# gligen/GLIGEN

Hardware: AMD Instinct MI355X
Metric: 512x512 images/sec @ 50 PLMS steps, box+text (CFG 7.5), UNet step ms (higher is better)
Workload: dtype bf16; 1 GPU; C2: box+text, 8 boxes (30 grounding tokens), 512x512, 50 PLMS steps, CFG 7.5, bf16 storage / fp32 accumulate; plms_steps=50, unet_evals_per_image=102, hipgraph=True, batches_in_flight=3

## Files before the change

gligen_amd/_lib.py:

```python
from __future__ import annotations

import ctypes as C
from pathlib import Path

_HERE = Path(__file__).resolve().parent
LIB_PATH = _HERE / "libgligen_amd.so"


class GligenAmdError(RuntimeError):
    pass


class UNetConfig(C.Structure):
    _fields_ = [
        ("in_channels", C.c_int), ("out_channels", C.c_int), ("model_channels", C.c_int),
        ("num_res_blocks", C.c_int), ("num_heads", C.c_int), ("context_dim", C.c_int),
        ("n_mult", C.c_int), ("channel_mult", C.c_int * 8),
        ("n_attn", C.c_int), ("attention_resolutions", C.c_int * 8),
        ("inpaint_mode", C.c_int), ("grounding_kind", C.c_int),
        ("gr_in_dim", C.c_int), ("gr_out_dim", C.c_int), ("max_persons", C.c_int), ("fuser_kind", C.c_int),
        ("extra_channels", C.c_int), ("tok_resize", C.c_int), ("tok_in_dim", C.c_int),
    ]


# ... 157 lines not shown
                                                C.POINTER(_P), C.POINTER(_P), _P, _P, _P]),
    "gl_op_class_conv_wgrad": (_I, [_P, _I, _P, _I, _I, _I, _I, _I, _P, _I, _P, _P, _P]),
}

TRAIN_INPUT_SYMBOLS = {
    "gl_train_step_inputs": (_I, [_P, C.POINTER(TrainStepInputsArgs), _P]),
}

TRAIN_FUSER_SYMBOLS = {
    "gl_op_block_train_fuser": (_I, [_P, _I, _P, C.POINTER(_P), _P, _P, _P, _P, _P, _P, _P, _P, C.POINTER(_P), _P]),
    "gl_op_grid_resize": (_I, [_P, _P, _I, _I, _I, _I, _P, _P]),
    "gl_op_grid_resize_backward": (_I, [_P, _P, _I, _I, _I, _I, _P, _P]),
}

_F = C.c_float
TRAIN_PRIM_SYMBOLS = {
    "gl_op_train_attention": (_I, [_P, _I, _I, _I, _I, _I] + [_P] * 9 + [_P]),
    "gl_op_train_linear": (_I, [_P, _I, _I, _I] + [_P] * 8 + [_P]),
    "gl_op_train_layernorm": (_I, [_P, _I, _I, _F, _P, _P, _P, _P, _I] + [_P] * 6 + [_P]),
    "gl_op_train_groupnorm": (_I, [_P, _I, _I, _I, _I, _F, _P, _P, _P, _P, _I] + [_P] * 4 + [_P]),
    "gl_op_train_geglu": (_I, [_P, _I, _I, _P, _P, _P, _P, _P]),
    "gl_op_train_dot": (_I, [_P, C.c_int64, _P, _P, _P, _F, _I, _P, _P]),
}

TRAINER_SYMBOLS = {
    "gl_op_adamw_ema_step": (_I, [_P, _P, _P, _P, _P, _P, C.c_int64, C.c_double, C.c_double, C.c_double, C.c_double, C.c_double, C.c_double, _I, _P]),
}

SAMPLER_SYMBOLS = {
    "gl_set_cfg_shared_prefix": (_I, [_I]),
}

class GemmPlanRecord(C.Structure):
    _fields_ = [("kernel", C.c_char * 96)] + [(n, C.c_int) for n in ("family", "M", "N", "K", "tm", "tn", "splits", "grid", "n_items", "box", "rm", "rz",
                                                                     "units_per_split", "xcd")]


class AttnProjLayout(C.Structure):
    _fields_ = [(n, C.c_int) for n in ("d", "dp", "dpv", "tq", "tk", "tq_pad", "tk_pad", "vt_perm32")]


GEMM_PLAN_SYMBOLS = {
    "gl_gemm_force_plan": (_I, [_I, _I, _I, _I]),
    "gl_gemm_force_knobs": (_I, [_I, _I, _I, _I, _I, _I]),
    "gl_gemm_force_clear": (_I, []),
    "gl_gemm_plan_log_clear": (_I, []),
    "gl_gemm_plan_log": (_I, [C.POINTER(GemmPlanRecord), _I, C.POINTER(_I), C.POINTER(_I)]),
    "gl_op_attention_project": (_I, [_P, _P, _P, _I, _I, _I, _I, _I, _I, _P, _P, _P, _P, _P, _P, C.POINTER(AttnProjLayout), _P]),
}

ATTENTION_CORE_SYMBOLS = {
    "gl_op_attention_core": (_I, [_P, _P, _P, _P, C.POINTER(AttnProjLayout), _I, _I, _I, _I, _P, _I, _I, _I, _P]),
}
ATTN_CORE_KERNELS = {"auto": 0, "attn_kernel": 1, "attn2_kernel_w4": 2, "attn2_kernel_w8": 3, "attn3_kernel": 4}
GL_ERR_UNSUPPORTED = 5

FUSER_KINDS = {"gatedSA": 0, "gatedSA2": 1, "gatedCA": 2}


def fuser_kind(fuser_type) -> int:
    try:
        return FUSER_KINDS[fuser_type or "gatedSA"]
    except KeyError:
        raise ValueError(f"fuser_type {fuser_type!r}: one of {sorted(FUSER_KINDS)}") from None


_lib = None


def load() -> C.CDLL:
    global _lib
    if _lib is not None:
        return _lib
    if not LIB_PATH.exists():
        raise GligenAmdError(
            f"{LIB_PATH} not found: build it with `python -m gligen_amd.build` "
            "(gligen_amd has no fallback path without its HIP library)")
    import torch
    lib = C.CDLL(str(LIB_PATH))
    for name, (res, args) in {**SYMBOLS, **IMAGE_SYMBOLS, **MAP_SYMBOLS, **TRAIN_MAP_SYMBOLS, **TRAIN_INPUT_SYMBOLS, **TRAIN_FUSER_SYMBOLS, **TRAIN_PRIM_SYMBOLS,
                              **TRAINER_SYMBOLS, **SAMPLER_SYMBOLS, **GEMM_PLAN_SYMBOLS, **ATTENTION_CORE_SYMBOLS}.items():
        fn = getattr(lib, name)
        fn.restype = res
        fn.argtypes = args
    _lib = lib
    return lib


def check(rc: int) -> None:
    if rc != 0:
        msg = load().gl_last_error()
        raise GligenAmdError(f"libgligen_amd error {rc}: {msg.decode() if msg else '?'}")
```

gligen_amd/csrc/capi.hip:

```cpp
#include "classmap.h"
#include "engine_impl.h"
#include "image.h"
#include "train.h"
#include "train_fusers.h"
#include "../../include/gligen_amd_train_maps.h"
#include "../../include/gligen_amd_train_inputs.h"
#include "../../include/gligen_amd_train_fusers.h"
#include "../../include/gligen_amd_train_prims.h"
#include "../../include/gligen_amd_trainer.h"
#include "../../include/gligen_amd_sampler.h"
#include "../../include/gligen_amd_gemm_plans.h"
#include "../../include/gligen_amd_attention_core.h"
#include "gemm_plan.h"

#include <cstdlib>

#include <cmath>

using namespace gl;

struct gl_ctx {
    std::shared_ptr<Engine> holder;
    Engine* eng;
    ImageStage image_stage;
};

#define GL_API_BEGIN try {
#define GL_API_END                                       \
    }                                                    \
    catch (const gl::GlError& e) {                       \
        return gl::set_error(e.code, "%s", e.what());    \
    }                                                    \
    catch (const std::exception& e) {                    \
        return gl::set_error(GL_ERR_STATE, "%s", e.what()); \
    }                                                    \
    return GL_OK;

struct DeviceGuard {
    int prev = -1;
    bool ok = true;
    explicit DeviceGuard(int dev) {
        if (hipGetDevice(&prev) != hipSuccess) prev = -1;
        if (prev != dev) ok = hipSetDevice(dev) == hipSuccess;
        else prev = -1;
    }
    ~DeviceGuard() {
        if (prev >= 0) (void)hipSetDevice(prev);
    }
};
#define NEED(ctx)                                                         \
    if (!(ctx) || !(ctx)->eng) return gl::set_error(GL_ERR_ARG, "null context"); \
    DeviceGuard device_guard_((ctx)->eng->device());                      \
    if (!device_guard_.ok) return gl::set_error(GL_ERR_HIP, "hipSetDevice(%d) failed", (ctx)->eng->device());

static inline hipStream_t S(gl_stream s) { return reinterpret_cast<hipStream_t>(s); }
#define HIPCK_API(expr)                                                                           \
    do {                                                                                          \
        hipError_t _e = (expr);                                                                   \
        if (_e != hipSuccess) throw GlError(GL_ERR_HIP, std::string(#expr) + ": " + hipGetErrorString(_e)); \
    } while (0)

extern "C" {

const char* gl_last_error(void) { return gl::last_error(); }

// ... 330 lines not shown
                    gl_stream s) {
    NEED(ctx);
    if (!x || !timesteps || !eps_out || !recs || !n_recs || max_recs <= 0) return gl::set_error(GL_ERR_ARG, "null pointer");
    GL_API_BEGIN
    ctx->eng->profile_begin();
    std::vector<Engine::ProfRec> out;
    try {
        ctx->eng->unet_forward(Beff, h, w, x, xB, timesteps, inpaint_extra, extraB, eps_out, S(s));
    } catch (...) {
        (void)ctx->eng->profile_end(S(s));
        throw;
    }
    out = ctx->eng->profile_end(S(s));
    int n = 0;
    for (const auto& r : out) {
        if (n >= max_recs) break;
        gl_prof_rec& d = recs[n++];
        snprintf(d.name, sizeof d.name, "%s", r.name.c_str());
        d.calls = r.calls; d.ms = r.ms; d.flops = r.flops; d.bytes = r.bytes;
    }
    *n_recs = n;
    GL_API_END
}

int gl_to_uint8(const float* img, uint8_t* out, int B, int C, int HW, gl_stream s) {
    if (!img || !out) return gl::set_error(GL_ERR_ARG, "null pointer");
    hipPointerAttribute_t at;
    if (hipPointerGetAttributes(&at, img) != hipSuccess) {
        (void)hipGetLastError();
        return gl::set_error(GL_ERR_ARG, "gl_to_uint8: img is not a device pointer");
    }
    DeviceGuard guard(at.device);
    if (!guard.ok) return gl::set_error(GL_ERR_HIP, "hipSetDevice(%d) failed", at.device);
    return to_uint8_launch(img, out, B, C, HW, S(s));
}

int gl_arena_high_water(gl_ctx* ctx, size_t* bytes) {
    NEED(ctx);
    *bytes = ctx->eng->arena().high_water();
    return GL_OK;
}

int gl_launch_count(gl_ctx* ctx, int64_t* n) {
    NEED(ctx);
    *n = ctx->eng->n_launches;
    return GL_OK;
}

int gl_set_ff_rows_policy(int mode) { return gl::ff_rows_policy_set(mode); }

int gl_ff_rows_policy_report(char* buf, size_t cap) { return gl::ff_rows_policy_report(buf, cap); }

int gl_set_cfg_shared_prefix(int on) { return gl::cfg_shared_prefix_set(on); }

int gl_gemm_force_plan(int tm, int tn, int splits, int grid_cap) {
    bool tile = tm == 0 && tn == 0;
    for (int c = 0; c < kGemmTiles; ++c) tile |= kGemmTm[c] == tm && kGemmTn[c] == tn;
    if (!tile || splits < 0 || splits > 32 || grid_cap < 0)
        return gl::set_error(GL_ERR_ARG, "gl_gemm_force_plan: tile %dx%d / %d splits / cap %d (tiles 4x5 4x4 2x5 2x4 2x2 or 0x0, splits 0..32, cap >= 0)", tm, tn, splits, grid_cap);
    gemm_force_cfg(tm, tn, tm ? splits : 0);
    gemm_force_grid(grid_cap);
    return GL_OK;
}
int gl_gemm_force_knobs(int halo_splits, int wide_splits, int wide_xcd, int xcd_boxes, int halo, int wide) {
    if (halo_splits < 0 || wide_splits < 0 || wide_xcd < -1 || wide_xcd > 1 || xcd_boxes < 0 || xcd_boxes > 1 || halo < 0 || wide < 0 || wide > 2)
        return gl::set_error(GL_ERR_ARG, "gl_gemm_force_knobs: halo_splits %d, wide_splits %d, wide_xcd %d, xcd_boxes %d, halo %d, wide %d", halo_splits, wide_splits, wide_xcd, xcd_boxes, halo, wide);
    gemm_force_knobs(halo_splits, wide_splits, wide_xcd, xcd_boxes, halo, wide);
    return GL_OK;
}
int gl_gemm_force_clear(void) { gemm_force_clear(); return GL_OK; }
int gl_gemm_plan_log_clear(void) { gemm_plan_log_clear(); return GL_OK; }
int gl_gemm_plan_log(gl_gemm_plan_record* out, int max, int* n_written, int* n_launches) {
    if (!out || !n_written || !n_launches || max < 0) return gl::set_error(GL_ERR_ARG, "gl_gemm_plan_log: null pointer or negative max");
    GemmLogEntry e[kGemmLogSize];
    const int n = gemm_plan_log(e, std::min(max, (int)kGemmLogSize), n_launches);
    for (int i = 0; i < n; ++i) {
        const GemmPlan& p = e[i].plan;
        gl_gemm_plan_record& r = out[i];
        r = gl_gemm_plan_record{};
        snprintf(r.kernel, sizeof r.kernel, "%s", p.name);
        r.family = p.family; r.M = e[i].M; r.N = e[i].N; r.K = e[i].K;
        r.tm = p.tm; r.tn = p.tn; r.splits = p.splits; r.grid = p.grid;
        if (p.family == GEMM_HALO) { r.n_items = p.halo.n_items; r.units_per_split = p.halo.chunks_per_split; }
        else if (p.family == GEMM_WIDE) { r.n_items = p.wide.n_items; r.units_per_split = p.wide.kt_per_split; r.xcd = p.wide.xcd; }
        else {
            r.n_items = p.work.n_items; r.units_per_split = p.work.kt_per_split;
            if (p.family != GEMM_GLDS) { r.box = p.work.box; r.rm = p.work.rm; r.rz = p.work.rz; }
        }
    }
    *n_written = n;
    return GL_OK;
}

int gl_box_calibrate(gl_ctx* ctx, gl_box_calibration* out, gl_stream s) {
    NEED(ctx);
    if (!out) return gl::set_error(GL_ERR_ARG, "gl_box_calibrate: null out pointer");
    GL_API_BEGIN
    Arena& ar = ctx->eng->arena();
    const size_t mk = ar.mark();
    const size_t bytes = size_t(1) << 30;
    void* scratch = ar.alloc(bytes);
    HIPCK_API(hipMemsetAsync(scratch, 1, bytes, S(s)));
    float v[3] = {0.f, 0.f, 0.f};
    int rc = box_calibrate_launch(scratch, bytes, v, S(s));
    ar.release(mk);
    if (rc != GL_OK) throw GlError(rc, gl::last_error());
// ... 592 lines not shown
        bf16* w4 = ar.get<bf16>((size_t)16 * Cout * Cin);
        const int rp = pack_upconv_phases_launch(w_oihw, w4, Cout, Cin, Cout, S(s));
        if (rp != GL_OK) throw GlError(rp, gl::last_error());
        c.w4 = w4;
        ctx->eng->conv3x3(TRef{(const bf16*)x0, C0, (const bf16*)x1, C1}, B, H, W, c, 1, 1, 1, nullptr, 0, nullptr, S(s), (bf16*)y);
        return GL_OK;
    }
    bf16* wp = ar.get<bf16>((size_t)Cout * 9 * Cin);
    int r = pack_conv_weight_launch(w_oihw, wp, Cout, Cin, 3, 3, Cout, S(s));
    if (r != GL_OK) throw GlError(r, gl::last_error());
    const int Hup = H << ups, Wup = W << ups;
    const int Ho = stride == 1 ? Hup : (pad_lo ? (Hup + 2 - 3) / 2 + 1 : (Hup + 1 - 3) / 2 + 1);
    const int Wo = stride == 1 ? Wup : (pad_lo ? (Wup + 2 - 3) / 2 + 1 : (Wup + 1 - 3) / 2 + 1);
    AOperand A{};
    A.p0 = (const bf16*)x0; A.C0 = C0; A.ld0 = C0; A.p1 = (const bf16*)x1; A.C1 = C1; A.ld1 = C1;
    A.mode = A_CONV3; A.Hin = H; A.Win = W; A.Ho = Ho; A.Wo = Wo; A.stride = stride; A.ups = ups; A.pad_lo = pad_lo;
    Epilogue E;
    epilogue_defaults(E);
    E.out = y; E.ldo = Cout; E.bias = bias; E.res = (const bf16*)res; E.ldres = Cout; E.rows_per_b = Ho * Wo;
    r = gemm_launch(A, wp, B * Ho * Wo, Cout, 9 * Cin, E, ctx->eng->splitk_ws(), ctx->eng->splitk_ws_bytes(), S(s));
    if (r != GL_OK) throw GlError(r, gl::last_error());
    GL_API_END
}

int gl_op_gn_silu_conv3x3(gl_ctx* ctx, const void* x0, int C0, const void* x1, int C1, int B, int H, int W, const float* gamma, const float* beta,
                          float eps, const float* w_oihw, const float* bias, int Cout, const float* bias2, const void* res, void* y, int mode,
                          int* used_prologue, gl_stream s) {
    NEED(ctx);
    if (!x0 || !gamma || !beta || !w_oihw || !y || !used_prologue) return gl::set_error(GL_ERR_ARG, "gl_op_gn_silu_conv3x3: null pointer");
    GL_API_BEGIN
    Engine& eng = *ctx->eng;
    Arena& ar = eng.arena();
    ar.reset();
    const int Cin = C0 + C1;
    bf16* wp = ar.get<bf16>((size_t)Cout * 9 * Cin);
    int r = pack_conv_weight_launch(w_oihw, wp, Cout, Cin, 3, 3, Cout, S(s));
    if (r != GL_OK) throw GlError(r, gl::last_error());
    NormW n;
    n.g = gamma; n.b = beta; n.C = Cin;
    ConvW c;
    c.w = wp; c.b = bias; c.Cin = Cin; c.Cout = Cout;
    const bool saved = eng.gn_prologue_;
    if (mode >= 0) eng.gn_prologue_ = mode != 0;
    const int64_t n0 = eng.n_prologue_convs;
    try {
        eng.gn_silu_conv3x3(TRef{(const bf16*)x0, C0, (const bf16*)x1, C1}, B, H, W, n, eps, c, bias2, Cout, (const bf16*)res, (bf16*)y, S(s));
    } catch (...) {
        eng.gn_prologue_ = saved;
        throw;
    }
    eng.gn_prologue_ = saved;
    *used_prologue = eng.n_prologue_convs > n0 ? 1 : 0;
    if (mode == 1 && !*used_prologue) throw GlError(GL_ERR_UNSUPPORTED, "gl_op_gn_silu_conv3x3: this shape has no GroupNorm prologue (conv_halo_kernel, H W % 256 == 0)");
    GL_API_END
}

int gl_op_groupnorm(gl_ctx* ctx, const void* x0, int C0, const void* x1, int C1, int B, int HW,
                    const float* gamma, const float* beta, float eps, int silu, void* y, gl_stream s) {
    NEED(ctx);
    GL_API_BEGIN
    Arena& ar = ctx->eng->arena();
    ar.reset();
    GNParams P{};
    P.x0 = (const bf16*)x0; P.C0 = C0; P.x1 = (const bf16*)x1; P.C1 = C1; P.B = B; P.HW = HW; P.eps = eps;
    P.gamma = gamma; P.beta = beta; P.y = (bf16*)y; P.silu = silu;
    P.partial = reinterpret_cast<float*>(ar.alloc(gn_partial_bytes(B, HW)));
    int r = groupnorm_launch(P, S(s));
    if (r != GL_OK) throw GlError(r, gl::last_error());
    GL_API_END
}

int gl_op_layernorm(gl_ctx* ctx, const void* x, const void* x2, int B, int N1, int N2, int Tpad, int C,
                    const float* gamma, const float* beta, float eps, void* y, gl_stream s) {
    NEED(ctx);
    GL_API_BEGIN
    LNParams P{};
    P.x = (const bf16*)x; P.x2 = (const bf16*)x2; P.B = B; P.N1 = N1; P.N2 = N2; P.Tpad = Tpad; P.C = C; P.eps = eps;
    P.gamma = gamma; P.beta = beta; P.y = (bf16*)y;
    int r = layernorm_launch(P, S(s));
    if (r != GL_OK) throw GlError(r, gl::last_error());
    GL_API_END
}

static void attention_project(Engine& eng, const void* xq, const void* xkv, int B, int Nq, int Nk, int C, int Ck, int H, const float* wq,
                              const float* wk, const float* wv, bf16* q, bf16* k, bf16* vt, int Tq_pad, int Tk_pad, int dp, int dpv, int vt_layout,
                              hipStream_t s) {
    Arena& ar = eng.arena();
    const int d = C / H, Tq = round_up(Nq, 64), Tk = round_up(Nk, 64);
    bf16* wqb = ar.get<bf16>((size_t)C * C);
    bf16* wkb = ar.get<bf16>((size_t)C * Ck);
    bf16* wvb = ar.get<bf16>((size_t)C * Ck);
    bf16* xqp = ar.get<bf16>((size_t)B * Tq * C);
    bf16* xkp = ar.get<bf16>((size_t)B * Tk * Ck);
    auto ck = [&](int rc) { if (rc != GL_OK) throw GlError(rc, gl::last_error()); };
    ck(cast_f32_bf16_launch(wq, wqb, (int64_t)C * C, s));
    ck(cast_f32_bf16_launch(wk, wkb, (int64_t)C * Ck, s));
    ck(cast_f32_bf16_launch(wv, wvb, (int64_t)C * Ck, s));
    ck(pad_rows_bf16_launch((const bf16*)xq, xqp, B, Nq, Tq, C, s));
    ck(pad_rows_bf16_launch((const bf16*)xkv, xkp, B, Nk, Tk, Ck, s));
    const bool fused = xq == xkv && C == Ck && Nq == Nk && gemm_supports_qkv() && (2 * C) % 128 == 0 &&
                       !(dev_env("GL_QKV_FUSED") && atoi(dev_env("GL_QKV_FUSED")) == 0);
    if (fused) {
        bf16* wqkv = ar.get<bf16>((size_t)3 * C * C);
        ck(cast_f32_bf16_launch(wq, wqkv, (int64_t)C * C, s));
        ck(cast_f32_bf16_launch(wk, wqkv + (size_t)C * C, (int64_t)C * C, s));
        ck(cast_f32_bf16_launch(wv, wqkv + (size_t)2 * C * C, (int64_t)C * C, s));
// ... 159 lines not shown
```

gligen_amd/csrc/engine.h:

```cpp
#pragma once
#include <array>
#include <map>
#include <memory>
#include <stdexcept>
#include <string>
#include <unordered_map>
#include <unordered_set>
#include <vector>

#include "arena.h"
#include "attention.h"
#include "clip.h"
#include "common.h"
#include "convnext.h"
#include "ffn.h"
#include "gemm.h"
#include "misc.h"
#include "norm.h"
#include "train.h"
#include "../../include/gligen_amd.h"

namespace gl {

struct RawTensor {
// ... 31 lines not shown
    const void* chain_stream = nullptr;
    bool chain_post = false;
    const void* chain_q_stream = nullptr;
    const float* chain_q_bias = nullptr;
};
struct RowStats { float2* p = nullptr; int nb = 0, ld = 0; };
struct STW {
    int C = 0, d = 0, idx = 0;
    NormW gn;
    LinW proj_in, proj_out;
    NormW ln1, ln2, ln3, fn1, fn2;
    SelfAttnW a1, fa;
    CrossAttnW a2;
    FFW ff, fff;
    LinW flin;
    CrossAttnW fca;
};

enum LayerKind { L_CONV_IN, L_RES, L_ST, L_DOWN, L_UP };
struct Layer {
    LayerKind kind;
    int idx;
};
struct UNetBlock { std::vector<Layer> layers; };

struct VaeAttnW { NormW gn; LinW q, k, v, proj; };

struct CnxBlock { const float* dw_w = nullptr; const float* dw_b = nullptr; NormW ln; LinW pw1, pw2; };
struct CnxNet {
    bool present = false;
    int resize = 0, in_dim = 0, tokens = 0;
    const float* inconv_w = nullptr; const float* inconv_b = nullptr;
    LinW stem; NormW stem_ln;
    NormW ds_ln[3]; LinW ds[3];
    std::vector<CnxBlock> blocks[4];
    int dims[4] = {0, 0, 0, 0};
    const float* pos = nullptr; const float* null_feat = nullptr;
    LinW mlp[3];
};

struct AttnBufs {
    bf16* q = nullptr;
    bf16* k = nullptr;
    bf16* vt = nullptr;
    int Tq_pad = 0, Tk_pad = 0;
};

struct TRef { const bf16* p0 = nullptr; int C0 = 0; const bf16* p1 = nullptr; int C1 = 0; int C() const { return C0 + C1; } };

int ff_rows_policy_set(int mode);
int ff_rows_policy_report(char* buf, size_t cap);
int cfg_shared_prefix_set(int on);
bool cfg_shared_prefix();
AttnParams attn_params(const bf16* q, const bf16* k, const bf16* vt, bf16* o, int H, int d, int Nq, int Nk, int Tq_pad, int Tk_pad, int vt_layout);

class Engine {
   public:
    explicit Engine(int device);
    ~Engine();
    static std::shared_ptr<Engine> fork(const std::shared_ptr<Engine>& parent, size_t arena_bytes);
    size_t weight_bytes() const { return persist_bytes_; }
    size_t arena_bytes() const { return arena_.committed(); }
    bool is_fork() const { return (bool)parent_; }

    void upload(const std::string& key, const void* src, int ndim, const int64_t* shape, bool is_device);
    void configure_unet(const gl_unet_config& c);
    void configure_vae(const gl_vae_config& c);
    void configure_clip_text(const gl_clip_text_config& c);
    void configure_clip_vision(const gl_clip_vision_config& c);
    void finalize();
    bool finalized() const { return finalized_; }

    void set_cond(int Beff, const float* context, int n_ctx, const gl_grounding& g, hipStream_t s);
    void set_fuser_scale(float v, hipStream_t s);
    void set_fuser_scales(const float* scales_host, int n, hipStream_t s);
    int n_fusers() const { return (int)unet_.st.size(); }
    void grounding_tokens(float* out, hipStream_t s);
    void spatial_tokens(int B, const float* image, int C, int H, int W, const float* mask, float* out, hipStream_t s);
    void spatial_tokens_classes(int B, const uint8_t* cls, int H, int W, const float* mask, float* out, hipStream_t s);
    int spatial_token_count() const { return unet_.cnx.tokens; }
    void restore_first_conv(const float* w, const float* b, hipStream_t s);
    void unet_forward(int Beff, int h, int w, const float* x, int xB, const int64_t* t, const float* extra,
                      int extraB, float* eps, hipStream_t s, const float* emb_row = nullptr);
    void vae_decode(int B, int h, int w, const float* z, float* out, hipStream_t s);
    void vae_encode(int B, int H, int W, const float* img, const float* noise, float* z, hipStream_t s);
    bool has_vae_encoder() const { return vae_.enc.present; }
    void clip_text_encode(const int32_t* ids, const int32_t* eos_index, int S, int T, float* last_hidden, float* pooled, hipStream_t s);
    void clip_vision_encode(const float* pixel_values, int S, float* last_hidden, float* pooled, float* image_embeds, hipStream_t s);
    int clip_vision_tokens() const { const int g = clipv_.cfg.patch ? clipv_.cfg.image_size / clipv_.cfg.patch : 0; return g * g + 1; }
    void sample_plms(const gl_plms_args& a, hipStream_t s);
    void sampler_timing(float* avg_ms, float* first_ms, int* n);

    Arena& arena() { return arena_; }
    float* splitk_ws() { return ws_; }
    size_t splitk_ws_bytes() const { return ws_bytes_; }
    void* persist(size_t bytes, bool zero);
    void init_workspace();
    AttnBufs& attn_bufs(int B, int H, int d, int Tq, int Tk, int dpv_layout = 0, int slot = 0);
    void attn_regime_counters(int enable, unsigned* out);
    unsigned* attn_counters() const { return attn_counting_ ? attn_ctr_ : nullptr; }

    bf16* gn_silu_conv3x3(const TRef& x, int B, int H, int W, const NormW& n, float eps, const ConvW& c, const float* bias2, int bias2_ld,
                          const bf16* res, bf16* out, hipStream_t s);
    bf16* conv3x3(const TRef& x, int B, int Hin, int Win, const ConvW& c, int stride, int ups, int pad_lo,
                  const float* bias2, int bias2_ld, const bf16* res, hipStream_t s, bf16* out = nullptr);
    static bool upconv_phase_form(int Cin, int Cout);
    bool gn_prologue_ = dev_env("GL_GN_PROLOGUE") && atoi(dev_env("GL_GN_PROLOGUE")) == 1;
    int64_t n_prologue_convs = 0;
    int device() const { return device_; }
    int64_t n_launches = 0;
    static constexpr int kTrainEvents = 64;
    hipEvent_t* train_events();
    bool train_events_recorded = false;
    TrainWeightCache* train_cache = nullptr;

    struct ProfRec { std::string name; int calls = 0; double ms = 0, flops = 0, bytes = 0; };
    void profile_begin();
    std::vector<ProfRec> profile_end(hipStream_t s);

   private:
    struct ProfEvt { std::string name; double flops, bytes; hipEvent_t e0, e1; };
    bool profiling_ = false;
    std::vector<ProfEvt> prof_;
    std::vector<hipEvent_t> prof_pool_;
    struct ProfScope {
        Engine* e; hipStream_t s; size_t idx;
        ProfScope(Engine* eng, hipStream_t st, const std::string& name, double flops, double bytes);
        ~ProfScope();
        void rename(const std::string& n) { if (e->profiling_) e->prof_[idx].name = n; }
    };
    friend struct ProfScope;
    const RawTensor& raw(const std::string& key) const;
    bool has(const std::string& key) const { return raw_.count(key) != 0; }
    const float* F(const std::string& key) const { return raw(key).p; }
    const float* FK(const std::string& key) { keep_raw_.insert(key); return raw(key).p; }
    std::unordered_set<std::string> keep_raw_;
    NormW norm(const std::string& prefix);
    LinW linear(const std::string& prefix, bool bias = true);
    ConvW conv3(const std::string& prefix, int Npad = 0, bool up2x = false);
    ConvW conv3_small(const std::string& prefix, int Cout);
    LinW conv1(const std::string& prefix);
    const bf16* cast_rows(const std::vector<std::string>& weight_keys);
    FFW ffw(const std::string& prefix, int C, const NormW* fold = nullptr, const std::string& pre_key = "", const std::string& post_key = "",
            const float* post_q_w = nullptr, const float* post_q_b = nullptr);
    struct FoldTmp { float* w = nullptr; float* b = nullptr; int N = 0, K = 0; };
    FoldTmp fold_ln(const std::string& weight_key, const float* bias, const NormW& n);
    std::vector<void*> fold_tmps_;
    ResW resw(const std::string& prefix, int Cin, int Cout, bool unet);

    void gemm(const AOperand& A, const bf16* W, int M, int N, int K, const Epilogue& E, hipStream_t s);
    bf16* linear_rows(const bf16* x, int M, const LinW& L, int act, const bf16* res, const float* gate, hipStream_t s, RowStats* stats = nullptr);
    bf16* layernorm_plain(const bf16* x, int B, int N, int C, bool pad64, hipStream_t s);
    bf16* groupnorm(const TRef& x, int B, int HW, const NormW& n, float eps, bool silu, hipStream_t s);
    bf16* layernorm(const bf16* x, int B, int N, int C, const NormW& n, bool pad64, hipStream_t s);
    bf16* conv3x3_small(const ConvW& c, Im2colParams P, int reps, hipStream_t s);
    void gn_silu_conv3x3_nchw(const bf16* x, int C, int B, int H, int W, const NormW& n, float eps, const ConvW& c, int n_real, float* out, hipStream_t s);
    bf16* resblock(const ResW& r, const TRef& x, int B, int H, int W, const float* embout, int emb_ld, float eps, hipStream_t s, bf16* out = nullptr);
    void replicate(const bf16* src, bf16* dst, size_t n, int reps, hipStream_t s);
    void attention(const bf16* q, const bf16* k, const bf16* vt, bf16* o, int B, int H, int d, int Nq, int Nk, int Tq_pad, int Tk_pad, int vt_layout,
                   hipStream_t s);
    void spatial_tokens_tail(int B, const float* img, const float* mask, float* out, hipStream_t s);

    Engine(const Engine&) = default;
    Engine& operator=(const Engine&) = delete;
    std::shared_ptr<Engine> parent_;
    size_t persist_bytes_ = 0;
    int device_;
    bool finalized_ = false;
    std::unordered_map<std::string, RawTensor> raw_;
    std::vector<void*> owned_;
    Arena arena_;
    float* ws_ = nullptr;
    size_t ws_bytes_ = 0;
    typedef std::array<int, 7> AttnKey;
    std::map<AttnKey, AttnBufs> attn_bufs_;
    unsigned* attn_ctr_ = nullptr;
    bool attn_counting_ = false;
    std::vector<hipEvent_t> train_events_;

    struct Unet {
        bool present = false;
        gl_unet_config cfg{};
        LinW te0, te2;
        LinW embcat;
        ConvW conv_in_small;
        std::vector<ResW> res;
        std::vector<STW> st;
        std::vector<ConvW> updown;
        std::vector<UNetBlock> in_blocks, out_blocks;
        UNetBlock mid_block;
        NormW out_norm;
        ConvW out_conv;
        const float* const* alpha_ptrs = nullptr;
        int gkind = 0;
        LinW pn[2][3];
        const float* pn_null_feat[2] = {nullptr, nullptr};
        const float* pn_null_pos = nullptr;
        const float* kp_table = nullptr;
        CnxNet cnx;
    } unet_;
    bool ln_fold_ = false;
    bool ff_rows_ = true;
    int ff_chain_ = 2;
    int qkv_rows_ = 1;
    bool fuser_hoist_ = true;
    void build_unet();
    float* gates_ = nullptr;
    float* fuser_scale_ = nullptr;
    bool fuser_off_ = false;
    struct Cond {
        int Beff = 0, Ng = 0, ctx_T = 0, ctx_Tpad = 0, obj_Tpad = 0;
        bf16* tokens = nullptr;
        int obj_stride = 0;
        std::vector<bf16*> objs;
        std::vector<bf16*> obj_k;
        std::vector<bf16*> obj_vt;
        std::vector<bf16*> ctx_k;
        std::vector<bf16*> ctx_vt;
        std::vector<void*> allocs;
    } cond_;
    void fuser_kv_fill(const STW& t, int B, int HW, hipStream_t s);
    void ensure_fuser_kv(const STW& t, int B, int HW, hipStream_t s);
    struct FuserKV { uint64_t epoch = 0; int B = 0, HW = 0; };
    std::vector<FuserKV> fuser_kv_;
    uint64_t cond_epoch_ = 0;

    bf16* transformer(const STW& t, const bf16* x, int B, int Bp, int H, int W, hipStream_t s);
    bf16* feedforward(const FFW& f, const bf16* ln, int M, const bf16* res, const float* gate, hipStream_t s, const RowStats* in_stats = nullptr,
                      RowStats* out_stats = nullptr, bool raw_rows = false, bool use_rows = false);
    bf16* fuser_ff_tail(const STW& t, const bf16* o, const bf16* t1, int B, int HW, bool rows, hipStream_t s, RowStats* st3, bool* q_done = nullptr);
    AttnBufs& to_q_heads(const LinW& q, const bf16* ln, int B, int Tp, int C, int d, int Tk_pad, const RowStats* st, const float* csum, hipStream_t s);
    void cross_q_gemm(const STW& t, const bf16* rows, const RowStats& st, int B, int HW, hipStream_t s);
    bf16* concat_layernorm(const STW& t, const bf16* x, int B, int HW, int Tf, hipStream_t s);
    void block_ff_tail(const STW& t, const bf16* o, const bf16* t3, const bf16* x, bf16* out, int B, int HW, bool rows, hipStream_t s);
    bf16* ff_behind(const FFW& f, const NormW& nw, const bf16* rows_in, RowStats& st_in, int B, int HW, const float* gate, bool rows, hipStream_t s,
                    RowStats* out_stats);
    bool can_fold(const RowStats& st, int M, int C, int Nc, int mode, int act, bool aligned);
    struct ChainQ { bf16* q; int DP, T, Tpad; };
    bf16* feedforward_chain(const FFW& f, const bf16* x, int M, const LinW& pre, const bf16* pre_res, const float* pre_gate, const float* gate,
                            const LinW* post, const bf16* post_res, bf16* out, hipStream_t s, RowStats* out_stats, const ChainQ* cq = nullptr);
    void self_attention(const SelfAttnW& a, const bf16* ln, int B, int T, int Nq, int Nk, int C, int d, bf16* o, hipStream_t s,
                        const RowStats* in_stats = nullptr, int Tbuf = 0, int slot = 0, bool projected = false);
    bool qkv_rows_ok(const SelfAttnW& a, int B, int T, int Nk, int C, int d) const;
    void qkv_project_gemm(const SelfAttnW& a, const bf16* ln, int B, int T, int Nk, int C, int d, hipStream_t s, const RowStats* in_stats, int Tbuf, int slot);
    void qkv_rows_project(const SelfAttnW& a, const bf16* x, int B, int T, int Nk, int C, int d, const LinW& pre, const bf16* pre_res, bf16* mid,
                          RowStats* mid_stats, int Tbuf, int slot, hipStream_t s, int Bin = 0);
    float* emb_rows(const int64_t* t_dev, int R, float* out, hipStream_t s);
    void emb_table_build(const int64_t* t_host, int R, hipStream_t s);
    float* emb_table_ = nullptr;
    float* emb_cur_ = nullptr;
    int64_t* emb_t_dev_ = nullptr;
    int emb_table_cap_ = 0;
    std::vector<int64_t> emb_t_cache_;

    bool ff_rows_for(const STW& t, int which, int B, int HW, hipStream_t s);
    bool qkv_rows_for(const STW& t, int which, int B, int HW, int Nk, hipStream_t s);
    template <class Run>
    bool timed_form(uint64_t key, int M, int C, int n_zero, const char* name, int form, hipStream_t s, Run&& run);

    void build_convnext(const std::string& PN);

    struct VaeLevel { std::vector<ResW> blocks; bool has_resample = false; ConvW resample; };
    struct VaeHalf {
        bool present = false;
        ConvW in_small;
        ResW mid1, mid2;
        VaeAttnW attn;
        std::vector<VaeLevel> levels;
        NormW norm_out;
        ConvW conv_out;
        const float* quant_w = nullptr;
        const float* quant_b = nullptr;
    };
    struct Vae { gl_vae_config cfg{}; VaeHalf dec, enc; } vae_;
    void build_vae();
    void build_vae_encoder();
    void build_vae_mid(VaeHalf& h, const std::string& prefix, int C);
    bf16* vae_attn(const VaeAttnW& a, const bf16* x, int B, int HW, hipStream_t s);

    struct ClipLayerW { NormW ln1, ln2; LinW qkv, out, fc1, fc2; };
// ... 53 lines not shown
```

gligen_amd/csrc/engine.hip:

```cpp
#include "engine_impl.h"

#include <algorithm>
#include <cmath>
#include <cstdarg>
#include <cstring>

namespace gl {

static thread_local char g_err[2048] = "";
int set_error(int code, const char* fmt, ...) {
    va_list ap;
    va_start(ap, fmt);
    vsnprintf(g_err, sizeof(g_err), fmt, ap);
    va_end(ap);
    return code;
}
const char* last_error() { return g_err; }

void Arena::init(size_t bytes) {
    off_ = hw_ = 0;
    HIPCK(hipGetDevice(&dev_));
    int vmm = 0;
    const char* sw = dev_env("GL_ARENA_VMM");
    if (!(sw && atoi(sw) == 0) && hipDeviceGetAttribute(&vmm, hipDeviceAttributeVirtualMemoryManagementSupported, dev_) == hipSuccess && vmm) {
// ... 455 lines not shown
        ProfScope ps(this, s, sym, 4.0 * B * H * (double)Nq * Nk * d, 0.0);
        CK(attn_launch(P, B, s));
        if (FILE* f = launch_log_file()) {
            fprintf(f, "%s|%d|%d|%d|2|%.0f\n", sym, Nq, Nk, d, 2.0 * B * H * d * (2.0 * Nq + 2.0 * Nk));
            fflush(f);
        }
    }
    ++n_launches;
}

void Engine::gemm(const AOperand& A, const bf16* W, int M, int N, int K, const Epilogue& E, hipStream_t s) {
    ProfScope ps(this, s, "gemm", 2.0 * M * N * K, 0.0);
    CK(gemm_launch(A, W, M, N, K, E, ws_, ws_bytes_, s));
    if (profiling_) {
        static const bool by_shape = dev_env("GL_PROF_SHAPES") != nullptr;
        std::string nm = gemm_last_kernel_name();
        if (by_shape) nm += fmt(" M%d N%d K%d", M, N, K);
        ps.rename(nm);
    }
    FILE* launch_log = launch_log_file();
    if (launch_log) {
        const double a_rows = A.mode != A_ROWS ? (double)(M / (A.Ho * A.Wo)) * A.Hin * A.Win : (double)M;
        const double out_b = E.mode == EPI_NCHW_F32 ? 4.0 * M * E.n_real : (E.act == ACT_GEGLU ? 1.0 : 2.0) * M * (double)N * (E.out_f32 ? 2 : 1);
        const double bytes = a_rows * (A.C0 + A.C1) * 2 + (double)N * K * 2 + out_b + (E.res ? 2.0 * M * N : 0.0);
        fprintf(launch_log, "%s|%d|%d|%d|%d|%.0f\n", gemm_last_kernel_name(), M, N, K, A.mode, bytes);
        fflush(launch_log);
    }
    {
        int tm, tn, sp;
        gemm_last_cfg(&tm, &tn, &sp);
        n_launches += sp > 1 ? 2 : 1;
    }
}

bf16* Engine::linear_rows(const bf16* x, int M, const LinW& L, int act, const bf16* res, const float* gate, hipStream_t s, RowStats* stats) {
    bf16* out = arena_.get<bf16>((size_t)M * L.N);
    Epilogue E = e_rows_res(out, L.N, L.b, res);
    E.act = act;
    E.gate = gate;
    if (stats) {
        *stats = RowStats{};
        if (ln_fold_ && L.N % 64 == 0) {
            stats->ld = L.N / 32;
            stats->p = arena_.get<float2>((size_t)M * stats->ld);
            E.stats_out = stats->p;
            E.stats_ld = stats->ld;
        }
    }
    gemm(a_rows(x, L.K), L.w, M, L.N, L.K, E, s);
    if (stats && stats->p) stats->nb = gemm_last_stats_nb();
    return out;
}

bf16* Engine::groupnorm(const TRef& x, int B, int HW, const NormW& n, float eps, bool silu, hipStream_t s) {
    const int C = x.C();
    if (n.C != C) throw GlError(GL_ERR_ARG, fmt("groupnorm: %d channels given to a norm with %d", C, n.C));
    bf16* y = arena_.get<bf16>((size_t)B * HW * C);
    GNParams P{};
    P.x0 = x.p0; P.C0 = x.C0; P.x1 = x.p1; P.C1 = x.C1;
    P.B = B; P.HW = HW; P.eps = eps; P.gamma = n.g; P.beta = n.b; P.y = y; P.silu = silu ? 1 : 0;
    P.partial = reinterpret_cast<float*>(arena_.alloc(gn_partial_bytes(B, HW)));
    ProfScope ps(this, s, HW <= 256 ? "gn_small_kernel" : "gn_stats_kernel + gn_apply_kernel", 0.0, 2.0 * B * HW * (double)C * 2);
    CK(groupnorm_launch(P, s));
    n_launches += HW <= 256 ? 1 : 2;
    return y;
}

bf16* Engine::gn_silu_conv3x3(const TRef& x, int B, int H, int W, const NormW& n, float eps, const ConvW& c, const float* bias2, int bias2_ld,
                              const bf16* res, bf16* out, hipStream_t s) {
    if (x.C() != c.Cin || n.C != c.Cin) throw GlError(GL_ERR_ARG, fmt("gn_silu_conv3x3: %d channels into a norm of %d and a conv of %d", x.C(), n.C, c.Cin));
    const int HW = H * W, M = B * HW;
    if (!out) out = arena_.get<bf16>((size_t)M * c.Cout);
    AOperand A = a_conv3(x, H, W, H, W, 1, 0, 1);
    Epilogue E = e_rows_res(out, c.Cout, c.b, res);
    E.bias2 = bias2; E.bias2_ld = bias2_ld; E.rows_per_b = HW;
    if (gn_prologue_ && gemm_gn_prologue_supported(A, M, c.Cout, 9 * c.Cin, E)) {
        GNParams P{};
        P.x0 = x.p0; P.C0 = x.C0; P.x1 = x.p1; P.C1 = x.C1;
        P.B = B; P.HW = HW; P.eps = eps; P.gamma = n.g; P.beta = n.b; P.silu = 1;
        P.partial = reinterpret_cast<float*>(arena_.alloc(gn_partial_bytes(B, HW)));
        P.coef = reinterpret_cast<float*>(arena_.alloc(gn_coef_bytes(B, c.Cin)));
        {
            const int nl = groupnorm_coef_launches(HW, x.C0, x.C1);
            ProfScope ps(this, s, nl == 1 ? "gn_small_coef_kernel" : "gn_stats_kernel + gn_coef_kernel", 0.0, 1.0 * B * HW * (double)c.Cin * 2);
            CK(groupnorm_coef_launch(P, s));
            n_launches += nl;
        }
        A.gn = P.coef;
        gemm(A, c.w, M, c.Cout, 9 * c.Cin, E, s);
        ++n_prologue_convs;
        return out;
    }
    bf16* a = groupnorm(x, B, HW, n, eps, true, s);
    A.p0 = a; A.C0 = c.Cin; A.ld0 = c.Cin; A.p1 = nullptr; A.C1 = 0; A.ld1 = 0;
    gemm(A, c.w, M, c.Cout, 9 * c.Cin, E, s);
    return out;
}

bf16* Engine::layernorm(const bf16* x, int B, int N, int C, const NormW& n, bool pad64, hipStream_t s) {
    const int Tp = pad64 ? round_up(N, 64) : N;
    bf16* y = arena_.get<bf16>((size_t)B * Tp * C);
    LNParams P{};
    P.x = x; P.x2 = nullptr; P.B = B; P.N1 = N; P.N2 = 0; P.Tpad = Tp; P.C = C; P.eps = 1e-5f;
    P.gamma = n.g; P.beta = n.b; P.y = y;
    ProfScope ps(this, s, "ln_kernel", 0.0, 2.0 * B * N * (double)C * 2);
    CK(layernorm_launch(P, s));
    ++n_launches;
    return y;
}

bf16* Engine::layernorm_plain(const bf16* x, int B, int N, int C, bool pad64, hipStream_t s) {
    NormW none;
    none.C = C;
    return layernorm(x, B, N, C, none, pad64, s);
}

bf16* Engine::conv3x3(const TRef& x, int B, int Hin, int Win, const ConvW& c, int stride, int ups, int pad_lo,
                      const float* bias2, int bias2_ld, const bf16* res, hipStream_t s, bf16* out) {
    if (x.C() != c.Cin) throw GlError(GL_ERR_ARG, fmt("conv3x3: input has %d channels, weight expects %d", x.C(), c.Cin));
    if (c.w4) {
        if (stride != 1 || ups != 1 || pad_lo != 1 || bias2 || res) throw GlError(GL_ERR_ARG, "conv3x3: phase-form weights serve the plain upsample conv only");
        const int Mi = 4 * Hin * Win;
        if (!out) out = arena_.get<bf16>((size_t)B * Mi * c.Cout);
        auto ok = [&](int b) { return gemm_upconv_phases_supported(a_conv2up(x, Hin, Win), b * Mi, c.Cout, 4 * c.Cin, e_rows(out, c.Cout, c.b)); };
        int Bc = B;
        while (Bc > 1 && !ok(Bc)) Bc = (Bc + 1) / 2;
        if (!ok(Bc)) throw GlError(GL_ERR_UNSUPPORTED, fmt("conv3x3: no phase form for a %d x %d x %d -> %d upsample conv", Hin, Win, c.Cin, c.Cout));
        for (int b0 = 0; b0 < B; b0 += Bc) {
            const size_t px = (size_t)b0 * Hin * Win;
            const TRef xb{x.p0 + px * x.C0, x.C0, x.p1 ? x.p1 + px * x.C1 : nullptr, x.C1};
            gemm(a_conv2up(xb, Hin, Win), c.w4, std::min(Bc, B - b0) * Mi, c.Cout, 4 * c.Cin, e_rows(out + (size_t)b0 * Mi * c.Cout, c.Cout, c.b), s);
        }
        return out;
    }
    const int Hup = Hin << ups, Wup = Win << ups;
    const int Ho = stride == 1 ? Hup : (pad_lo ? (Hup + 2 - 3) / 2 + 1 : (Hup + 1 - 3) / 2 + 1);
    const int Wo = stride == 1 ? Wup : (pad_lo ? (Wup + 2 - 3) / 2 + 1 : (Wup + 1 - 3) / 2 + 1);
    const int M = B * Ho * Wo;
    if (!out) out = arena_.get<bf16>((size_t)M * c.Cout);
    Epilogue E = e_rows_res(out, c.Cout, c.b, res);
    E.bias2 = bias2; E.bias2_ld = bias2_ld; E.rows_per_b = Ho * Wo;
    gemm(a_conv3(x, Hin, Win, Ho, Wo, stride, ups, pad_lo), c.w, M, c.Cout, 9 * c.Cin, E, s);
    return out;
}

void Engine::replicate(const bf16* src, bf16* dst, size_t n, int reps, hipStream_t s) {
    ProfScope ps(this, s, "replicate_kernel", 0.0, (1.0 + reps) * n * 2);
    CK(replicate_launch(src, dst, n * sizeof(bf16), reps, s));
    ++n_launches;
}

bf16* Engine::resblock(const ResW& r, const TRef& x, int B, int H, int W, const float* embout, int emb_ld, float eps, hipStream_t s, bf16* out) {
    const int HW = H * W, M = B * HW;
    if (!out) out = arena_.get<bf16>((size_t)M * r.Cout);
    const size_t mk = arena_.mark();
    bf16* h = gn_silu_conv3x3(x, B, H, W, r.n1, eps, r.c1, embout ? embout + r.emb_off : nullptr, emb_ld, nullptr, nullptr, s);
    const bf16* sk;
    if (r.has_skip) {
        bf16* skb = arena_.get<bf16>((size_t)M * r.Cout);
        AOperand A{};
        A.p0 = x.p0; A.C0 = x.C0; A.ld0 = x.C0; A.p1 = x.p1; A.C1 = x.C1; A.ld1 = x.C1; A.mode = A_ROWS;
        gemm(A, r.skip.w, M, r.Cout, r.Cin, e_rows(skb, r.Cout, r.skip.b), s);
        sk = skb;
    } else {
        if (x.p1) throw GlError(GL_ERR_STATE, "identity skip over a concatenated input");
        sk = x.p0;
    }
    gn_silu_conv3x3(TRef{h, r.Cout, nullptr, 0}, B, H, W, r.n2, eps, r.c2, nullptr, 0, sk, out, s);
    arena_.release(mk);
    return out;
}

bf16* Engine::conv3x3_small(const ConvW& c, Im2colParams P, int reps, hipStream_t s) {
    const size_t rows = (size_t)P.B * P.H * P.W;
    bf16* col = arena_.get<bf16>(reps * rows * c.Kpad);
    bf16* out = arena_.get<bf16>(reps * rows * c.Cout);
    P.Kpad = c.Kpad;
    for (int r = 0; r < reps; ++r) {
        P.out = col + r * rows * c.Kpad;
        CK(im2col_small_launch(P, s));
        ++n_launches;
    }
    gemm(a_rows(col, c.Kpad), c.w, (int)(reps * rows), c.Cout, c.Kpad, e_rows(out, c.Cout, c.b), s);
    return out;
}

void Engine::gn_silu_conv3x3_nchw(const bf16* x, int C, int B, int H, int W, const NormW& n, float eps, const ConvW& c, int n_real, float* out, hipStream_t s) {
    const int HW = H * W;
    bf16* a = groupnorm(TRef{x, C, nullptr, 0}, B, HW, n, eps, true, s);
    Epilogue E;
    epilogue_defaults(E);
    E.mode = EPI_NCHW_F32; E.out = out; E.bias = c.b; E.rows_per_b = HW; E.n_real = n_real;
    gemm(a_conv3(TRef{a, C, nullptr, 0}, H, W, H, W, 1, 0, 1), c.w, B * HW, c.Npad, 9 * C, E, s);
}

AttnBufs& Engine::attn_bufs(int B, int H, int d, int Tq, int Tk, int dpv_layout, int slot) {
    const int Tq_pad = round_up(Tq, 128), Tk_pad = round_up(Tk, 64);
    int dp, dpv;
    CK(attn_dims(d, &dp, &dpv));
    if (dpv_layout) dpv = dpv_layout;
    const AttnKey key{{B, H, d, Tq_pad, Tk_pad, dpv, slot}};
    auto it = attn_bufs_.find(key);
    if (it != attn_bufs_.end()) return it->second;
    AttnBufs b;
    b.Tq_pad = Tq_pad;
    b.Tk_pad = Tk_pad;
    b.q = reinterpret_cast<bf16*>(persist((size_t)B * H * Tq_pad * dp * sizeof(bf16), true));
    b.k = reinterpret_cast<bf16*>(persist((size_t)B * H * Tk_pad * dp * sizeof(bf16), true));
    b.vt = reinterpret_cast<bf16*>(persist((size_t)B * H * dpv * Tk_pad * sizeof(bf16), true));
    CK(attn_vt_ones_launch(b.vt, B * H, d, Tk_pad, 0, dpv));
    CK(attn_k_init_launch(b.k, B * H, d, Tk_pad, 0));
    HIPCK(hipStreamSynchronize(0));
    return attn_bufs_.emplace(key, b).first->second;
}

}
```

gligen_amd/csrc/engine_impl.h:

```cpp
#pragma once
#include "engine.h"

namespace gl {

#define CK(expr)                                              \
    do {                                                      \
        int _r = (expr);                                      \
        if (_r != GL_OK) throw GlError(_r, gl::last_error()); \
    } while (0)
#define HIPCK(expr)                                                                             \
    do {                                                                                        \
        hipError_t _e = (expr);                                                                 \
        if (_e != hipSuccess)                                                                   \
            throw GlError(GL_ERR_HIP, std::string(#expr) + " -> " + hipGetErrorString(_e));     \
    } while (0)

FILE* launch_log_file();

unsigned ff_rows_policy_epoch();

void cfg_shared_prefix_note(int what);

struct PlanAsBatch {
    explicit PlanAsBatch(int scale) { gemm_set_plan_batch_scale(scale); }
    ~PlanAsBatch() { gemm_set_plan_batch_scale(1); }
};

inline AOperand a_rows(const bf16* x, int K) {
    AOperand A;
    aoperand_rows(A, x, K, K);
    return A;
}
inline AOperand a_conv3(const TRef& x, int Hin, int Win, int Ho, int Wo, int stride, int ups, int pad_lo) {
    AOperand A{};
    A.p0 = x.p0; A.C0 = x.C0; A.ld0 = x.C0;
    A.p1 = x.p1; A.C1 = x.C1; A.ld1 = x.C1;
    A.mode = A_CONV3;
    A.Hin = Hin; A.Win = Win; A.Ho = Ho; A.Wo = Wo; A.stride = stride; A.ups = ups; A.pad_lo = pad_lo;
    return A;
}
inline AOperand a_conv2up(const TRef& x, int Hin, int Win) {
    AOperand A = a_conv3(x, Hin, Win, 2 * Hin, 2 * Win, 1, 0, 1);
    A.mode = A_CONV2UP;
    return A;
}
inline Epilogue e_rows(void* out, int ldo, const float* bias = nullptr) {
    Epilogue E;
    epilogue_defaults(E);
    E.out = out; E.ldo = ldo; E.bias = bias;
    return E;
}
inline Epilogue e_rows_res(void* out, int ldo, const float* bias, const bf16* res) {
    Epilogue E = e_rows(out, ldo, bias);
    E.res = res; E.ldres = ldo;
    return E;
}
inline Epilogue e_heads(int mode, bf16* q, bf16* k, int C, int H, int d, int DP, int T, int Tpad_q, int Tpad_k) {
    Epilogue E;
    epilogue_defaults(E);
    E.mode = mode;
    E.q = q; E.k = k; E.C = C; E.H = H; E.d = d; E.DP = DP; E.T = T; E.Tpad_q = Tpad_q; E.Tpad_k = Tpad_k;
    return E;
}
inline void e_fold_ln(Epilogue& E, const RowStats& st, const float* csum, int C) {
    E.ln_stats = st.p; E.ln_nb = st.nb; E.ln_ld = st.ld; E.ln_csum = csum;
    E.ln_inv_c = 1.f / (float)C; E.ln_eps = 1e-5f;
}

}
```

gligen_amd/csrc/engine_policy.hip:

```cpp
#include "engine_impl.h"
#include <algorithm>
#include <atomic>
#include <map>
#include <mutex>

namespace gl {

namespace ff_policy {
static std::mutex mu;
struct Entry { int rows; float us_rows, us_gemm; };
static std::map<uint64_t, Entry> table;
static std::atomic<int> mode{-1};
static std::atomic<unsigned> epoch{1};
static uint64_t key(int dev, int which, int form, int C, int M) {
    return ((uint64_t)dev << 56) | ((uint64_t)which << 52) | ((uint64_t)form << 48) | ((uint64_t)C << 32) | (uint64_t)(unsigned)M;
}
static bool static_rule(int M) { return M / 128 >= 224; }
static int current_mode() {
    static const bool env_once = [] {
        if (const char* e = dev_env("GL_FF_POLICY")) mode.store(atoi(e));
        return true;
    }();
    (void)env_once;
    return mode.load();
}
}

int ff_rows_policy_set(int mode) {
    if (mode < -1 || mode > 2) return set_error(GL_ERR_ARG, "ff_rows policy %d (expected -1 timed, 0 never, 1 wherever supported, 2 static rule)", mode);
    if (ff_policy::mode.exchange(mode) != mode) ff_policy::epoch.fetch_add(1);
    return GL_OK;
}
unsigned ff_rows_policy_epoch() { return ff_policy::epoch.load(); }

namespace cfg_prefix {
static std::atomic<int> on{-1};
static int current() {
    int v = on.load();
    if (v < 0) {
        const char* e = dev_env("GL_CFG_SHARED_PREFIX");
        const int want = (e && atoi(e) == 0) ? 0 : 1;
        int expect = -1;
        on.compare_exchange_strong(expect, want);
        v = on.load();
    }
    return v;
}
static std::atomic<long long> count[3];
}
bool cfg_shared_prefix() { return cfg_prefix::current() != 0; }
void cfg_shared_prefix_note(int what) { cfg_prefix::count[what].fetch_add(1); }
int cfg_shared_prefix_set(int on) {
    if (on != 0 && on != 1) return set_error(GL_ERR_ARG, "cfg shared prefix %d (expected 0 or 1)", on);
    if (cfg_prefix::current() != on) {
        cfg_prefix::on.store(on);
        ff_policy::epoch.fetch_add(1);
    }
    return GL_OK;
}
int ff_rows_policy_report(char* buf, size_t cap) {
    if (!buf || !cap) return set_error(GL_ERR_ARG, "ff_rows_policy_report: no buffer");
    std::lock_guard<std::mutex> lk(ff_policy::mu);
    size_t n = (size_t)snprintf(buf, cap, "mode=%d", ff_policy::mode.load());
    for (const auto& kv : ff_policy::table) {
        if (n + 96 + 128 >= cap) break;
        const uint64_t k = kv.first;
        n += (size_t)snprintf(buf + n, cap - n, ";dev%d %s form%d C%d M%d -> %s (rows %.1f us, gemm %.1f us)", (int)(k >> 56),
                              ((k >> 52) & 15) == 1 ? "fuser.ff" : ((k >> 52) & 15) == 2 ? "ff" : ((k >> 52) & 15) == 3 ? "proj_in+attn1.qkv" : "attn1.to_out+fuser.qkv", (int)((k >> 48) & 15), (int)((k >> 32) & 0xffff), (int)(k & 0xffffffffu),
                              kv.second.rows ? "rows" : "gemm", kv.second.us_rows, kv.second.us_gemm);
    }
    if (n + 128 < cap)
        snprintf(buf + n, cap - n, ";cfg_shared_prefix=%d evals=%lld rows_at_prefix=%lld rows_periodic=%lld", cfg_prefix::current(),
                 cfg_prefix::count[0].load(), cfg_prefix::count[1].load(), cfg_prefix::count[2].load());
    return GL_OK;
}

template <class Run>
bool Engine::timed_form(uint64_t key, int M, int C, int n_zero, const char* name, int form, hipStream_t s, Run&& run) {
    const int mode = ff_policy::current_mode();
    if (mode == 0) return false;
    if (mode == 1) return true;
    if (mode == 2) return ff_policy::static_rule(M);
    std::unique_lock<std::mutex> lk(ff_policy::mu);
    auto it = ff_policy::table.find(key);
    if (it != ff_policy::table.end()) return it->second.rows != 0;
    hipStreamCaptureStatus cap = hipStreamCaptureStatusNone;
    (void)hipStreamIsCapturing(s, &cap);
    if (cap != hipStreamCaptureStatusNone) {
        const bool rows = ff_policy::static_rule(M);
        ff_policy::table[key] = ff_policy::Entry{rows ? 1 : 0, 0.f, 0.f};
        return rows;
    }

    HIPCK(hipDeviceSynchronize());
    struct Restore {
        Engine* e; size_t mk; int64_t launches; bool prof;
        ~Restore() { e->arena_.release(mk); e->n_launches = launches; e->profiling_ = prof; }
    } restore{this, arena_.mark(), n_launches, profiling_};
    profiling_ = false;
    bf16* z[4];
    for (bf16*& p : z) p = arena_.get<bf16>((size_t)M * C);
    for (int i = 0; i < n_zero; ++i) HIPCK(hipMemsetAsync(z[i], 0, (size_t)M * C * sizeof(bf16), s));
    auto once = [&](bool rows) {
        const size_t m2 = arena_.mark();
        run(rows, z);
        arena_.release(m2);
    };
    hipEvent_t ev[2];
    HIPCK(hipEventCreate(&ev[0]));
    HIPCK(hipEventCreate(&ev[1]));
    struct EvGuard { hipEvent_t* e; ~EvGuard() { (void)hipEventDestroy(e[0]); (void)hipEventDestroy(e[1]); } } guard{ev};
    float best[2] = {1e30f, 1e30f};
    constexpr int REPS = 4, ROUNDS = 3;
    for (int form_i = 0; form_i < 2; ++form_i) once(form_i == 1);
    for (int r = 0; r < ROUNDS; ++r)
        for (int form_i = 0; form_i < 2; ++form_i) {
            HIPCK(hipEventRecord(ev[0], s));
            for (int i = 0; i < REPS; ++i) once(form_i == 1);
            HIPCK(hipEventRecord(ev[1], s));
            HIPCK(hipEventSynchronize(ev[1]));
            float ms = 0.f;
            HIPCK(hipEventElapsedTime(&ms, ev[0], ev[1]));
            best[form_i] = std::min(best[form_i], ms * 1e3f / REPS);
// ... 50 lines not shown
```

gligen_amd/csrc/engine_unet.hip:

```cpp
#include "engine_impl.h"
#include <algorithm>
#include <cmath>

namespace gl {

void Engine::configure_unet(const gl_unet_config& c) {
    if (c.n_mult < 1 || c.n_mult > 8 || c.n_attn < 0 || c.n_attn > 8) throw GlError(GL_ERR_ARG, "bad unet config");
    if (c.model_channels % 64 != 0) throw GlError(GL_ERR_UNSUPPORTED, "model_channels must be a multiple of 64");
    if (c.fuser_kind < 0 || c.fuser_kind > 2) throw GlError(GL_ERR_ARG, "fuser_kind: 0 gatedSA, 1 gatedSA2, 2 gatedCA");
    if (c.extra_channels < 0 || c.extra_channels > 64) throw GlError(GL_ERR_ARG, "extra_channels out of range");
    if (c.extra_channels && c.inpaint_mode) throw GlError(GL_ERR_UNSUPPORTED, "inpaint_mode with a grounding downsampler is undefined in the reference");
    unet_.cfg = c;
    unet_.present = true;
}

void Engine::build_unet() {
    const gl_unet_config& c = unet_.cfg;
    const int mc = c.model_channels;
    const std::string U = "unet/";
    auto in_attn = [&](int ds) {
        for (int i = 0; i < c.n_attn; ++i)
            if (c.attention_resolutions[i] == ds) return true;
        return false;
    };
// ... 464 lines not shown
    Epilogue E = e_rows(hbuf, 4 * C, f.b1);
    E.act = ACT_GEGLU; E.geglu16 = f.geglu16;
    if (in_stats) {
        if (!f.folded) throw GlError(GL_ERR_STATE, "feedforward: row statistics given to an unfolded projection");
        e_fold_ln(E, *in_stats, f.csum1, C);
    }
    gemm(a_rows(ln, C), f.w1, M, 8 * C, C, E, s);
    return linear_rows(hbuf, M, f.w2, ACT_NONE, res, gate, s, out_stats);
}

AttnBufs& Engine::to_q_heads(const LinW& q, const bf16* ln, int B, int Tp, int C, int d, int Tk_pad, const RowStats* st, const float* csum, hipStream_t s) {
    const int heads = C / d;
    int dp, dpv;
    CK(attn_dims(d, &dp, &dpv));
    AttnBufs& bufs = attn_bufs(B, heads, d, Tp, Tk_pad);
    Epilogue E = e_heads(EPI_QK_HEADS, bufs.q, nullptr, C, heads, d, dp, Tp, bufs.Tq_pad, 0);
    E.bias = q.b;
    if (st) e_fold_ln(E, *st, csum, C);
    gemm(a_rows(ln, C), q.w, B * Tp, C, C, E, s);
    return bufs;
}

void Engine::cross_q_gemm(const STW& t, const bf16* rows, const RowStats& st, int B, int HW, hipStream_t s) {
    const int C = t.C, M = B * HW;
    const int Tp = round_up(HW, 64);
    const bool f3 = t.a2.folded && can_fold(st, M, C, C, EPI_QK_HEADS, ACT_NONE, Tp == HW);
    const bf16* ln = f3 ? rows : (t.a2.folded ? layernorm_plain(rows, B, HW, C, true, s) : layernorm(rows, B, HW, C, t.ln2, true, s));
    to_q_heads(t.a2.q, ln, B, Tp, C, t.d, cond_.ctx_Tpad, f3 ? &st : nullptr, t.a2.q_csum, s);
}

void Engine::ensure_fuser_kv(const STW& t, int B, int HW, hipStream_t s) {
    if (fuser_kv_.size() < unet_.st.size()) fuser_kv_.resize(unet_.st.size());
    const FuserKV& kv = fuser_kv_[t.idx];
    if (kv.epoch == cond_epoch_ && kv.B == B && kv.HW == HW) return;
    hipStreamCaptureStatus cap = hipStreamCaptureStatusNone;
    (void)hipStreamIsCapturing(s, &cap);
    if (cap != hipStreamCaptureStatusNone) throw GlError(GL_ERR_STATE, "fuser keys of this prompt / shape were not projected before the graph capture");
    fuser_kv_fill(t, B, HW, s);
    n_launches += 2;
}

bf16* Engine::concat_layernorm(const STW& t, const bf16* x, int B, int HW, int Tf, hipStream_t s) {
    const int Ng = cond_.Ng, C = t.C;
    bf16* lnc = arena_.get<bf16>((size_t)B * Tf * C);
    LNParams P{};
    P.x = x; P.x2 = cond_.objs[t.idx]; P.B = B; P.N1 = HW; P.N2 = Ng; P.Tpad = Tf; P.C = C; P.eps = 1e-5f;
    P.gamma = t.fa.folded ? nullptr : t.fn1.g; P.beta = t.fa.folded ? nullptr : t.fn1.b; P.y = lnc;
    ProfScope ps(this, s, "ln_kernel", 0.0, 2.0 * B * (HW + Ng) * (double)C * 2);
    CK(layernorm_launch(P, s));
    ++n_launches;
    return lnc;
}

bf16* Engine::transformer(const STW& t, const bf16* x, int B, int Bp, int H, int W, hipStream_t s) {
    const int HW = H * W, M = B * HW, C = t.C, d = t.d, heads = C / d;
    bf16* out = arena_.get<bf16>((size_t)M * C);
    const size_t mk = arena_.mark();
    if (cond_.Beff != B) throw GlError(GL_ERR_STATE, fmt("unet_forward batch %d != batch %d of the conditioning set by gl_unet_set_cond", B, cond_.Beff));
    if (Bp <= 0 || B % Bp != 0) throw GlError(GL_ERR_STATE, fmt("transformer: prefix batch %d does not divide batch %d", Bp, B));
    const bool shared = Bp < B;
    const int Mp = Bp * HW;

    bf16* n = groupnorm(TRef{x, C, nullptr, 0}, Bp, HW, t.gn, 1e-6f, false, s);
    const int Tp = round_up(HW, 64);
    const bool aligned = Tp == HW;
    auto normed = [&](const bf16* rows, const NormW& nw, bool folded, bool fuse, bool pad64) -> const bf16* {
        if (fuse) return rows;
        return folded ? layernorm_plain(rows, Bp, HW, C, pad64, s) : layernorm(rows, Bp, HW, C, nw, pad64, s);
    };
    RowStats st0, st1, st2, st3;
    const bool r2 = !fuser_off_ && ff_rows_for(t, 1, B, HW, s), r4 = ff_rows_for(t, 2, B, HW, s);
    bf16* t0;
    const bf16* ln = nullptr;
    bf16* o = arena_.get<bf16>((size_t)M * C);
    bool rq1;
    {
    PlanAsBatch plan_as(B / Bp);
    rq1 = aligned && qkv_rows_for(t, 0, Bp, HW, HW, s);
    if (rq1) {
        t0 = arena_.get<bf16>((size_t)Mp * C);
        qkv_rows_project(t.a1, n, Bp, HW, HW, C, d, t.proj_in, nullptr, t0, nullptr, 0, 0, s);
        self_attention(t.a1, nullptr, Bp, Tp, HW, HW, C, d, o, s, nullptr, 0, 0, true);
        if (shared) cfg_shared_prefix_note(1);
    } else {
        t0 = linear_rows(n, Mp, t.proj_in, ACT_NONE, nullptr, nullptr, s, &st0);
        const bool f1 = t.a1.folded && can_fold(st0, Mp, C, 3 * C, EPI_QKV_HEADS, ACT_NONE, aligned);
        ln = normed(t0, t.ln1, t.a1.folded, f1, true);
        self_attention(t.a1, ln, Bp, Tp, HW, HW, C, d, o, s, f1 ? &st0 : nullptr);
    }
    }
    const int Ng = cond_.Ng;
    const bool rq2 = !fuser_off_ && unet_.cfg.fuser_kind == 0 && fuser_hoist_ && aligned && cond_.Ng > 0 && qkv_rows_for(t, 1, B, HW, HW + Ng, s);
    if (shared && !rq2) {
        replicate(o, o + (size_t)Mp * C, (size_t)Mp * C, B / Bp - 1, s);
        bf16* t0b = arena_.get<bf16>((size_t)M * C);
        replicate(t0, t0b, (size_t)Mp * C, B / Bp, s);
        t0 = t0b;
    }
    bf16* t1 = rq2 ? arena_.get<bf16>((size_t)M * C) : linear_rows(o, M, t.a1.out, ACT_NONE, t0, nullptr, s, &st1);

    bf16* t3;
    bool q_done = false;
    if (fuser_off_) {
        t3 = t1;
        st3 = st1;
    } else if (unet_.cfg.fuser_kind == 0) {
        const int Tf = round_up(HW + Ng, 64);
        if (rq2) {
            ensure_fuser_kv(t, B, HW, s);
            qkv_rows_project(t.fa, o, B, HW, HW + Ng, C, d, t.a1.out, t0, t1, nullptr, Tf, t.idx + 1, s, shared ? Bp : 0);
            if (shared) cfg_shared_prefix_note(2);
            self_attention(t.fa, nullptr, B, HW, HW, HW + Ng, C, d, o, s, nullptr, Tf, t.idx + 1, true);
        } else if (fuser_hoist_ && t.fa.fused && t.fa.folded && aligned) {
            ensure_fuser_kv(t, B, HW, s);
            const bool ff = can_fold(st1, M, C, 3 * C, EPI_QKV_HEADS, ACT_NONE, aligned);
            const bf16* rows = ff ? t1 : layernorm_plain(t1, B, HW, C, false, s);
// ... 214 lines not shown
    if ((int)emb_t_cache_.size() == R && std::equal(t_host, t_host + R, emb_t_cache_.begin())) return;
    if (R > emb_table_cap_) {
        const int cap = std::max(R, 64);
        emb_table_ = reinterpret_cast<float*>(persist((size_t)cap * unet_.embcat.N * sizeof(float), false));
        emb_t_dev_ = reinterpret_cast<int64_t*>(persist((size_t)cap * sizeof(int64_t), false));
        if (!emb_cur_) emb_cur_ = reinterpret_cast<float*>(persist((size_t)unet_.embcat.N * sizeof(float), true));
        emb_table_cap_ = cap;
    }
    HIPCK(hipMemcpyAsync(emb_t_dev_, t_host, (size_t)R * sizeof(int64_t), hipMemcpyHostToDevice, s));
    const size_t mk = arena_.mark();
    emb_rows(emb_t_dev_, R, emb_table_, s);
    arena_.release(mk);
    emb_t_cache_.assign(t_host, t_host + R);
}

void Engine::unet_forward(int Beff, int h, int w, const float* x, int xB, const int64_t* t, const float* extra,
                          int extraB, float* eps, hipStream_t s, const float* emb_row) {
    if (!unet_.present || !finalized_) throw GlError(GL_ERR_STATE, "unet not finalized");
    if (cond_.Beff != Beff) throw GlError(GL_ERR_STATE, fmt("unet_forward batch %d but conditioning was set for %d", Beff, cond_.Beff));
    const gl_unet_config& c = unet_.cfg;
    const int extra_C = c.inpaint_mode ? c.in_channels + 1 : c.extra_channels;
    if ((extra_C != 0) != (extra != nullptr))
        throw GlError(GL_ERR_ARG, "the extra first-conv input (inpainting_extra_input / downsampled grounding_extra_input) must be given iff the model has those channels");
    if (xB <= 0 || Beff % xB != 0) throw GlError(GL_ERR_ARG, "x batch must divide the effective batch");
    const int mc = c.model_channels;
    arena_.reset();

    const float* embout = emb_row;
    int emb_ld = 0;
    if (!emb_row) {
        embout = emb_rows(t, Beff, nullptr, s);
        emb_ld = unet_.embcat.N;
        ++n_launches;
    }
    CK(gates_launch(unet_.alpha_ptrs, fuser_scale_, gates_, 2 * (int)unet_.st.size(), s));
    ++n_launches;

    struct Act { bf16* p; int C, H, W; };
    std::vector<Act> hs;
    Act cur{nullptr, 0, h, w};

    int Bp = Beff;
    if (emb_row && Beff / xB > 1 && cfg_shared_prefix()) {
        bool has_st = false;
        for (const UNetBlock& b : unet_.in_blocks)
            for (const Layer& L : b.layers) has_st = has_st || L.kind == L_ST;
        if (has_st) {
            Bp = xB;
            cfg_shared_prefix_note(0);
        }
    }
    bool in_prefix = Bp < Beff;

    auto run_layer = [&](const Layer& L, const TRef& in, int Bl, bool full) {
        PlanAsBatch plan_as(L.kind == L_ST ? 1 : Beff / Bl);
        auto out_for = [&](int HWo, int Co) { return full ? arena_.get<bf16>((size_t)Beff * HWo * Co) : nullptr; };
        auto fill = [&](bf16* o, int HWo, int Co) {
            if (full) replicate(o, o + (size_t)Bl * HWo * Co, (size_t)Bl * HWo * Co, Beff / Bl - 1, s);
        };
        switch (L.kind) {
            case L_CONV_IN: {
                if (extra && extraB != xB) throw GlError(GL_ERR_ARG, "extra first-conv input batch must equal x batch");
                Im2colParams P{};
                P.x0 = x; P.C0 = c.in_channels;
                P.x1 = extra; P.C1 = extra_C;
                P.B = xB; P.H = cur.H; P.W = cur.W;
                cur.p = conv3x3_small(unet_.conv_in_small, P, Beff / xB, s);
                cur.C = mc;
                break;
            }
            case L_RES: {
                const ResW& r = unet_.res[L.idx];
                cur.p = resblock(r, in, Bl, cur.H, cur.W, embout, emb_ld, 1e-5f, s, out_for(cur.H * cur.W, r.Cout));
                cur.C = r.Cout;
                fill(cur.p, cur.H * cur.W, cur.C);
                break;
            }
            case L_ST: {
                if (in.p1) throw GlError(GL_ERR_STATE, "transformer over concatenated input");
                cur.p = transformer(unet_.st[L.idx], in.p0, Beff, Bl, cur.H, cur.W, s);
                break;
            }
            case L_DOWN: {
                const int Ho = (cur.H + 2 - 3) / 2 + 1, Wo = (cur.W + 2 - 3) / 2 + 1;
                cur.p = conv3x3(in, Bl, cur.H, cur.W, unet_.updown[L.idx], 2, 0, 1, nullptr, 0, nullptr, s, out_for(Ho * Wo, unet_.updown[L.idx].Cout));
                cur.H = Ho;
                cur.W = Wo;
                fill(cur.p, Ho * Wo, unet_.updown[L.idx].Cout);
                break;
            }
            case L_UP: {
                cur.p = conv3x3(in, Beff, cur.H, cur.W, unet_.updown[L.idx], 1, 1, 1, nullptr, 0, nullptr, s);
                cur.H *= 2;
                cur.W *= 2;
                break;
            }
        }
    };

    for (const UNetBlock& b : unet_.in_blocks) {
        for (size_t i = 0; i < b.layers.size(); ++i) {
            const Layer& L = b.layers[i];
            const bool pre = in_prefix && L.kind != L_CONV_IN;
            const bool last = i + 1 == b.layers.size();
            run_layer(L, TRef{cur.p, cur.C, nullptr, 0}, pre ? Bp : Beff, pre && L.kind != L_ST && (last || b.layers[i + 1].kind == L_ST));
            if (L.kind == L_ST) in_prefix = false;
        }
        hs.push_back(cur);
    }
    for (const Layer& L : unet_.mid_block.layers) run_layer(L, TRef{cur.p, cur.C, nullptr, 0}, Beff, false);
    for (const UNetBlock& b : unet_.out_blocks) {
        Act sk = hs.back();
        hs.pop_back();
        if (sk.H != cur.H || sk.W != cur.W) throw GlError(GL_ERR_ARG, "latent size must be divisible by the UNet's total stride");
        bool first = true;
        for (const Layer& L : b.layers) {
            if (first) run_layer(L, TRef{cur.p, cur.C, sk.p, sk.C}, Beff, false);
            else run_layer(L, TRef{cur.p, cur.C, nullptr, 0}, Beff, false);
            first = false;
        }
    }
    gn_silu_conv3x3_nchw(cur.p, cur.C, Beff, cur.H, cur.W, unet_.out_norm, 1e-5f, unet_.out_conv, c.out_channels, eps, s);
}

}
```

gligen_amd/csrc/gemm.h:

```cpp
#pragma once
#include "common.h"

namespace gl {

enum { A_ROWS = 0, A_CONV3 = 1, A_CONV2UP = 2 };

struct AOperand {
    const bf16* p0;
    const bf16* p1;
    int C0, C1;
    int ld0, ld1;
    int mode;
    int Hin, Win, Ho, Wo;
    int stride, ups, pad_lo;
    const float* gn = nullptr;
};

enum { EPI_ROWMAJOR = 0, EPI_QK_HEADS = 1, EPI_VT_HEADS = 2, EPI_NCHW_F32 = 3, EPI_QKV_HEADS = 4 };
enum { ACT_NONE = 0, ACT_SILU = 1, ACT_GEGLU = 2, ACT_GELU = 3, ACT_QUICK_GELU = 4 };

struct Epilogue {
    int mode;
    int act;
    void* out;
    int ldo;
    int out_f32;
    const float* bias;
    const float* bias2;
    int bias2_ld;
    int rows_per_b;
    unsigned rpb_magic;
    int rpb_shift;
    const bf16* res;
    int ldres;
    const float* gate;
    bf16* q;
    bf16* k;
    int q_tiled;
    int C, H, d, DP, T;
    int Tpad_q, Tpad_k;
    bf16* vt;
    int DPV;
    int tok_off;
    int vt_perm32;
    int n_real;
    int remap_in, remap_out, remap_off;
    int up_win;
    int geglu16;
    float2* stats_out;
    int stats_ld;
    const float2* ln_stats;
    int ln_nb, ln_ld;
    const float* ln_csum;
    float ln_inv_c, ln_eps;
};

__host__ __device__ inline size_t ktile_off(size_t bh, int tpad, int t, int dd, int DP) {
    return (bh * (size_t)tpad + (size_t)(t & ~63)) * DP + (size_t)(dd >> 3) * 512 + (size_t)(t & 63) * 8 + (dd & 7);
}

int gemm_launch(const AOperand& A, const bf16* W, int M, int N, int K, const Epilogue& E,
                float* ws, size_t ws_bytes, hipStream_t stream);

int gemm_launch_t(const bf16* Wrows, int Mw, const bf16* X, int Nx, int K, const Epilogue& E,
                  hipStream_t stream);

void epilogue_defaults(Epilogue& E);
bool gemm_supports_qkv();
void gemm_set_variant(int v);
int gemm_geglu_layout();
void gemm_force_cfg(int tm, int tn, int splits);
void gemm_force_grid(int blocks);
void gemm_set_autotune(int on);
void gemm_set_no_split(int on);
void gemm_set_plan_batch_scale(int scale);
void gemm_last_cfg(int* tm, int* tn, int* splits);
const char* gemm_last_kernel_name();
bool gemm_gn_prologue_supported(const AOperand& A, int M, int N, int K, const Epilogue& E);
bool gemm_upconv_phases_supported(const AOperand& A, int M, int N, int K, const Epilogue& E);
bool gemm_ln_fold_supported(const AOperand& A, int M, int N, int K, const Epilogue& E);
int gemm_last_stats_nb();
void aoperand_rows(AOperand& A, const bf16* p, int K, int ld);

}
```

gligen_amd/csrc/gemm.hip:

```cpp
#include "gemm_plan.h"

#include <algorithm>
#include <climits>
#include <cstdio>
#include <cstdlib>
#include <cstring>
#include <type_traits>

namespace gl {

void epilogue_defaults(Epilogue& E) {
    E = Epilogue{};
    E.mode = EPI_ROWMAJOR;
    E.act = ACT_NONE;
    E.rows_per_b = 1;
    E.rpb_magic = 1; E.rpb_shift = 0;
}

void aoperand_rows(AOperand& A, const bf16* p, int K, int ld) {
    A = AOperand{};
    A.p0 = p;
    A.C0 = K;
    A.ld0 = ld;
    A.mode = A_ROWS;
}

__device__ __forceinline__ int perm_tok4(int t0, int p32 = 0) {
    if (p32) {
        const int g = (t0 >> 2) & 7;
        return (t0 & ~31) | ((((g & 1) << 2) | (g >> 1)) << 2);
    }
    int g = (t0 >> 2) & 3;
    int gp = ((g & 1) << 1) | (g >> 1);
    return (t0 & ~15) | (gp << 2);
}

__device__ __forceinline__ void store_bf16x4(bf16* dst, const float v[4]) {
    U2BF4 o;
    o.e[0] = f2bf(v[0]);
    o.e[1] = f2bf(v[1]);
    o.e[2] = f2bf(v[2]);
    o.e[3] = f2bf(v[3]);
    *reinterpret_cast<uint2*>(dst) = o.u;
}

__device__ __forceinline__ int div_rpb(const Epilogue& E, int m) {
    return (int)((__umulhi((unsigned)m, E.rpb_magic) + (unsigned)m) >> E.rpb_shift);
}

__device__ __forceinline__ void epi_finish4(const Epilogue& E, int m, int n0, float v[4]) {
    if (E.bias) {
        float4 b = *reinterpret_cast<const float4*>(E.bias + n0);
        v[0] += b.x; v[1] += b.y; v[2] += b.z; v[3] += b.w;
// ... 1374 lines not shown
                gate[0] += b.x; gate[1] += b.y; gate[2] += b.z; gate[3] += b.w;
            }
            epi_geglu4(E, m, n0, val, gate);
        } else {
            const bool fast = E.mode == EPI_ROWMAJOR && !E.out_f32 && !E.remap_in && E.act != ACT_GELU && E.act != ACT_QUICK_GELU && !E.ln_stats;
            const float4 pb = *reinterpret_cast<const float4*>((fast && E.bias) ? E.bias + n0 : ws);
            const float4 pb2 = *reinterpret_cast<const float4*>((fast && E.bias2) ? E.bias2 + (size_t)div_rpb(E, m) * E.bias2_ld + n0 : ws);
            const uint2 pr = *reinterpret_cast<const uint2*>((fast && E.res) ? reinterpret_cast<const void*>(E.res + (size_t)m * E.ldres + n0)
                                                                              : reinterpret_cast<const void*>(ws));
            const float pg = *((fast && E.res && E.gate) ? E.gate : ws);
            float v[4] = {0, 0, 0, 0};
            const float* p0 = ws + (size_t)m * N + n0;
            const size_t zs = (size_t)M * N;
            for (int z = 0; z < splits; z += 4) {
                float4 a[4];
#pragma unroll
                for (int u = 0; u < 4; ++u) a[u] = *reinterpret_cast<const float4*>(p0 + (size_t)min(z + u, splits - 1) * zs);
#pragma unroll
                for (int u = 0; u < 4; ++u) {
                    const bool ok = z + u < splits;
                    v[0] += ok ? a[u].x : 0.f; v[1] += ok ? a[u].y : 0.f; v[2] += ok ? a[u].z : 0.f; v[3] += ok ? a[u].w : 0.f;
                }
            }
            if (E.ln_stats) {
                const float2 st = ln_row_stats(E, m);
                const float4 cs = *reinterpret_cast<const float4*>(E.ln_csum + n0);
                v[0] = st.y * (v[0] - st.x * cs.x); v[1] = st.y * (v[1] - st.x * cs.y);
                v[2] = st.y * (v[2] - st.x * cs.z); v[3] = st.y * (v[3] - st.x * cs.w);
            }
            if (fast) {
                if (E.bias) { v[0] += pb.x; v[1] += pb.y; v[2] += pb.z; v[3] += pb.w; }
                if (E.bias2) { v[0] += pb2.x; v[1] += pb2.y; v[2] += pb2.z; v[3] += pb2.w; }
                if (E.act == ACT_SILU) {
#pragma unroll
                    for (int i = 0; i < 4; ++i) v[i] = silu_f(v[i]);
                }
                if (E.res) {
                    U2BF4 r;
                    r.u = pr;
                    const float g = E.gate ? pg : 1.f;
#pragma unroll
                    for (int i = 0; i < 4; ++i) v[i] = bf2f(r.e[i]) + g * v[i];
                }
                int mo = m;
                if (E.up_win) {
                    const int mp = M >> 2, ph = m / mp, r = m - ph * mp, q = div_rpb(E, r);
                    mo = ((2 * q + (ph >> 1)) * E.up_win + (r - q * E.up_win)) * 2 + (ph & 1);
                }
                store_bf16x4(reinterpret_cast<bf16*>(E.out) + (size_t)mo * E.ldo + n0, v);
            } else {
                epi_finish4(E, m, n0, v);
            }
        }
    }
}

template <int TN, int NW, bool GN = false>
__global__ void __launch_bounds__(NW * 64, 1)
conv_halo_kernel(AOperand A, const bf16* __restrict__ W, int M, int N, int K, Epilogue E, float* __restrict__ ws, HaloDesc hd) {
    constexpr int NT = NW * 64;
    constexpr int RPP = NT / 8;
    constexpr int TM = 32 / NW;
    constexpr int BM = 256;
    constexpr int BN = TN * 32;
    constexpr int HROWS = 448;
    constexpr int HPASS = HROWS / RPP;
    constexpr int HPT = (HPASS + 6) / 7;
    constexpr int HBUF = HROWS * 128;
    constexpr int WSLOT = BN * 128;
    constexpr int WP = (BN + RPP - 1) / RPP;
    constexpr int WREM = BN % RPP;
    constexpr unsigned SENT = 0x80000000u;
    constexpr int COEF0 = 2 * HBUF + 2 * WSLOT;
    static_assert(HPASS * RPP == HROWS && HPT * 7 >= HPASS && WREM % 8 == 0, "loader geometry");
    static_assert(!GN || (HPT == 1 && HPASS == 7), "the prologue rewrites pass p of the next chunk during tap p + 1");

    extern __shared__ __attribute__((aligned(16))) unsigned char smem[];

    const int t = threadIdx.x;
    const int lane = t & 63;
    const int wave = __builtin_amdgcn_readfirstlane(t >> 6);
    const int wm = wave >> 1;
    const int wn = wave & 1;
    const int l15 = lane & 15;
    const int q = lane >> 4;
    const int r0 = t >> 3;
    const unsigned chb = (((t & 7) ^ ((r0 >> 1) & 7)) * 16);
    const unsigned chb_h = (((t & 7) ^ (r0 & 6)) * 16);
    const int Cin = A.C0 + A.C1;

    const int Wd = 1 << hd.lgW, Hd = 1 << hd.lgH;
    const int R = BM >> hd.lgW;
    const int lgHB = min(hd.lgH, 8 - hd.lgW);
    const int HB = 1 << lgHB;
    const int W2 = Wd + 2;
    const int blkrows = (HB + 2) * W2;
    const int NH = (R >> lgHB) * blkrows;

    const __amdgpu_buffer_rsrc_t ra0 = __builtin_amdgcn_make_buffer_rsrc((void*)A.p0, 0, 0x80000000u, 0x00020000);
    const __amdgpu_buffer_rsrc_t ra1 = __builtin_amdgcn_make_buffer_rsrc((void*)(A.p1 ? A.p1 : A.p0), 0, 0x80000000u, 0x00020000);
    const __amdgpu_buffer_rsrc_t rw = __builtin_amdgcn_make_buffer_rsrc((void*)W, 0, 0x80000000u, 0x00020000);

    const unsigned inv_w2 = ((1u << 22) + W2 - 1) / W2, inv_blk = ((1u << 22) + blkrows - 1) / blkrows;
    int hr00;
    {
        const int p = wm * TM * 16 + l15;
// ... 649 lines not shown
        } else {
            __builtin_amdgcn_s_waitcnt(0x0F70);
        }
        __builtin_amdgcn_s_barrier();
        asm volatile("" ::: "memory");
        if (NST == 3) { if (kt + 2 < kt_end) issue(kt + 2, ring_next(ring_next(stg))); }
        else if (kt + 1 < kt_end) issue(kt + 1, stg ^ 1);
        compute(stg, !first);
        stg_done = stg;
        stg = ring_next(stg);
        ++kt;
    };
    for (;;) {
        tile(std::true_type{});
        while (kt < kt_end) tile(std::false_type{});
        finish();
        const int done_m0 = m0, done_tn = c_tn, done_z = c_z;
        float done_s = ln_s, done_q = ln_q;
#pragma unroll
        for (int i = 0; i < LNV; ++i) { done_s += ln_v[i].x; done_q += ln_v[i].y; }
        item += gridDim.x;
        const bool more = item < wd.n_items;
        if (more) begin_item(item);
        {
            const int nm0 = m0, ntn = c_tn, nz = c_z;
            m0 = done_m0; c_tn = done_tn; c_z = done_z;
            const float2* lst = nullptr;
            if (E.ln_stats && wd.splits == 1) {
                float2* l = reinterpret_cast<float2*>(smem + stg_done * STAGE);
                __builtin_amdgcn_s_barrier();
                const int row = t >> 1, part = t & 1;
                float s = done_s, qq = done_q;
                s += __shfl_xor(s, 1, 64); qq += __shfl_xor(qq, 1, 64);
                if (part == 0) {
                    const float mean = s * E.ln_inv_c;
                    const float var = fmaxf(qq * E.ln_inv_c - mean * mean, 0.f);
                    l[row] = make_float2(mean, rsqrtf(var + E.ln_eps));
                }
                __syncthreads();
                lst = l;
            }
            epilogue(lst);
            m0 = nm0; c_tn = ntn; c_z = nz;
        }
        if (!more) break;
        zero_acc();
    }
}



static thread_local GemmPlan t_last = [] { GemmPlan p{}; strcpy(p.name, "gemm"); return p; }();
int gemm_last_stats_nb() { return t_last.stats_nb; }
const char* gemm_last_kernel_name() { return t_last.name; }
void gemm_last_cfg(int* tm, int* tn, int* splits) { *tm = t_last.tm; *tn = t_last.tn; *splits = t_last.splits; }
static thread_local GemmLogEntry t_log[kGemmLogSize];
static thread_local int t_log_n = 0;
void gemm_plan_log_clear() { t_log_n = 0; }
int gemm_plan_log(GemmLogEntry* out, int max, int* launches) {
    if (launches) *launches = t_log_n;
    const int n = std::max(0, std::min(std::min(t_log_n, kGemmLogSize), max));
    for (int i = 0; i < n; ++i) out[i] = t_log[(t_log_n - n + i) % kGemmLogSize];
    return n;
}

namespace {

struct Launch {
    const AOperand& A; const bf16* W; int M, N, K; const Epilogue& E; float* ws;
    hipStream_t stream;
    template <auto KFN, class... Tail> int run(dim3 grid, int block, size_t lds, const Tail&... tail) const {
        return launch_lds<KFN>(grid, dim3(block), lds, stream, A, W, M, N, K, E, ws, tail...);
    }
};

template <int WM, int WN, int TM, int TN>
int exec_glds(const Launch& l, const GemmPlan& p) {
    const dim3 grid(p.grid, 1, p.splits);
    const size_t lds = 2 * (WM * TM * 32 + WN * TN * 32) * 128;
    if (p.amode == A_ROWS) return l.run<gemm_glds_kernel<WM, WN, TM, TN, A_ROWS>>(grid, WM * WN * 64, lds, p.work.kt_per_split, p.work.tiles_n, p.grid);
    return l.run<gemm_glds_kernel<WM, WN, TM, TN, A_CONV3>>(grid, WM * WN * 64, lds, p.work.kt_per_split, p.work.tiles_n, p.grid);
}
template <int TM, int TN>
int exec_p(const Launch& l, const GemmPlan& p) {
    const size_t lds = 2 * (TM * 32 + TN * 32) * 128;
    if (p.amode == A_ROWS) return l.run<gemm_p_kernel<TM, TN, A_ROWS>>(p.grid, 256, lds, p.work);
    return l.run<gemm_p_kernel<TM, TN, A_CONV3>>(p.grid, 256, lds, p.work);
}
template <int TM, int TN>
int exec_u(const Launch& l, const GemmPlan& p) {
    const size_t lds = 2 * (TM * 32 + TN * 32) * 128;
    if (p.qkv) {
        if constexpr (TM == 4 && TN == 5) return set_error(GL_ERR_UNSUPPORTED, "gemm: no 128x160 tile for EPI_QKV_HEADS");
        else return l.run<gemm_u_kernel<2, TM, TN, A_ROWS, 2, true>>(p.grid, 256, lds, p.work);
    }
    if (p.amode == A_ROWS) return l.run<gemm_u_kernel<2, TM, TN, A_ROWS, 2>>(p.grid, 256, lds, p.work);
    if (p.amode == A_CONV2UP) return l.run<gemm_u_kernel<2, TM, TN, A_CONV2UP, 2>>(p.grid, 256, lds, p.work);
    return l.run<gemm_u_kernel<2, TM, TN, A_CONV3, 2>>(p.grid, 256, lds, p.work);
}
constexpr size_t halo_lds(int tn, bool gn) { return 2 * 7 * 64 * 128 + 2 * tn * 32 * 128 + (gn ? 2048 : 0); }
constexpr size_t wide_lds(int tn) { return GL_WIDE_NST * (256 + tn * 32) * 128; }

int execute(const GemmPlan& p, const AOperand& A, const bf16* W, int M, int N, int K, const Epilogue& E_in, float* ws, hipStream_t stream) {
    Epilogue E = E_in;
    if ((p.family == GEMM_P || p.family == GEMM_U) && !p.stats_nb) E.stats_out = nullptr;
    const Launch l{A, W, M, N, K, E, ws, stream};
    int rc = set_error(GL_ERR_UNSUPPORTED, "gemm: unknown tile candidate");
    switch (p.family * 1000 + p.gn * 100 + p.tm * 10 + p.tn) {
        case GEMM_HALO * 1000 + 185: rc = l.run<conv_halo_kernel<5, 8, true>>(p.grid, 512, halo_lds(5, true), p.halo); break;
        case GEMM_HALO * 1000 + 184: rc = l.run<conv_halo_kernel<4, 8, true>>(p.grid, 512, halo_lds(4, true), p.halo); break;
        case GEMM_HALO * 1000 + 85: rc = l.run<conv_halo_kernel<5, 8>>(p.grid, 512, halo_lds(5, false), p.halo); break;
        case GEMM_HALO * 1000 + 84: rc = l.run<conv_halo_kernel<4, 8>>(p.grid, 512, halo_lds(4, false), p.halo); break;
        case GEMM_WIDE * 1000 + 85: rc = l.run<gemm_wide_kernel<5>>(p.grid, 512, wide_lds(5), p.wide); break;
        case GEMM_WIDE * 1000 + 84: rc = l.run<gemm_wide_kernel<4>>(p.grid, 512, wide_lds(4), p.wide); break;
        case GEMM_U * 1000 + 45: rc = exec_u<4, 5>(l, p); break;
        case GEMM_U * 1000 + 44: rc = exec_u<4, 4>(l, p); break;
        case GEMM_U * 1000 + 25: rc = exec_u<2, 5>(l, p); break;
        case GEMM_U * 1000 + 24: rc = exec_u<2, 4>(l, p); break;
        case GEMM_U * 1000 + 22: rc = exec_u<2, 2>(l, p); break;
        case GEMM_P * 1000 + 45: rc = exec_p<4, 5>(l, p); break;
        case GEMM_P * 1000 + 44: rc = exec_p<4, 4>(l, p); break;
        case GEMM_P * 1000 + 25: rc = exec_p<2, 5>(l, p); break;
        case GEMM_P * 1000 + 24: rc = exec_p<2, 4>(l, p); break;
        case GEMM_GLDS * 1000 + 44: rc = exec_glds<2, 2, 2, 2>(l, p); break;
        case GEMM_GLDS * 1000 + 42: rc = exec_glds<2, 2, 2, 1>(l, p); break;
        case GEMM_GLDS * 1000 + 22: rc = exec_glds<2, 2, 1, 1>(l, p); break;
        case GEMM_GLDS * 1000 + 41: rc = exec_glds<4, 1, 1, 1>(l, p); break;
    }
    GL_TRY(rc);
    if (p.splits > 1) {
        int64_t total = (int64_t)M * (N / 4);
        int blocks = (int)fmin((double)cdiv64(total, 256), 4096.0);
        hipLaunchKernelGGL(splitk_reduce_kernel, dim3(blocks), dim3(256), 0, stream, ws, p.splits, M, N, E);
        GL_LAUNCH_CHECK();
    }
    return GL_OK;
}

int tune(const bf16* W, float* ws, hipStream_t stream, const GemmProblem& pb, bool use_u, const char* key, const GemmCand& model, GemmCand* win, bool* cache) {
    hipStreamCaptureStatus cap = hipStreamCaptureStatusNone;
    if (stream) (void)hipStreamIsCapturing(stream, &cap);
    if (cap != hipStreamCaptureStatusNone) return GL_OK;
    auto run = [&](const GemmCand& c, hipStream_t s) -> int {
        GemmPlan plan{};
        GL_TRY(gemm_plan_tile(pb, use_u, c, plan));
        return execute(plan, pb.A, W, pb.M, pb.N, pb.K, pb.E, ws, s);
    };
    GL_HIP(hipDeviceSynchronize());
    hipEvent_t ev[2];
    GL_HIP(hipEventCreate(&ev[0]));
    GL_HIP(hipEventCreate(&ev[1]));
    struct EvGuard { hipEvent_t* e; ~EvGuard() { (void)hipEventDestroy(e[0]); (void)hipEventDestroy(e[1]); } } ev_guard{ev};
    float win_ms = 1e30f;
    const int tune_reps = gemm_knobs().tune_reps, corun = gemm_knobs().corun;
    hipStream_t s2 = nullptr;
    hipEvent_t ev_fork = nullptr, ev_join = nullptr;
    struct CoGuard { hipStream_t& s; hipEvent_t &a, &b; ~CoGuard() { if (a) (void)hipEventDestroy(a); if (b) (void)hipEventDestroy(b); if (s) (void)hipStreamDestroy(s); } } co_guard{s2, ev_fork, ev_join};
    if (corun) {
        GL_HIP(hipStreamCreateWithFlags(&s2, hipStreamNonBlocking));
        GL_HIP(hipEventCreateWithFlags(&ev_fork, hipEventDisableTiming));
        GL_HIP(hipEventCreateWithFlags(&ev_join, hipEventDisableTiming));
    }
    for (const GemmCand& c : gemm_tune_candidates(pb, use_u)) {
        GL_TRY(run(c, stream));
        GL_HIP(hipEventRecord(ev[0], stream));
        if (corun) {
            GL_HIP(hipEventRecord(ev_fork, stream));
            GL_HIP(hipStreamWaitEvent(s2, ev_fork, 0));
            for (int r = 0; r < tune_reps; ++r) {
                GL_TRY(run(c, stream));
                GL_TRY(run(c, s2));
            }
            GL_HIP(hipEventRecord(ev_join, s2));
            GL_HIP(hipStreamWaitEvent(stream, ev_join, 0));
        } else
            for (int r = 0; r < tune_reps; ++r) GL_TRY(run(c, stream));
        GL_HIP(hipEventRecord(ev[1], stream));
        GL_HIP(hipEventSynchronize(ev[1]));
        float ms = 0.f;
        GL_HIP(hipEventElapsedTime(&ms, ev[0], ev[1]));
        if (ms < win_ms) { win_ms = ms; *win = c; }
    }
    *cache = true;
    if (gemm_knobs().tune_log)
        fprintf(stderr, "[gemm autotune] %s -> %dx%d / %d splits @%d (%.1f us; model said %dx%d / %d) cfg %d %d %d\n", key, kGemmTm[win->c] * 32,
                kGemmTn[win->c] * 32, win->sp, win->grid ? win->grid : 512, win_ms * 1e3f / tune_reps, kGemmTm[model.c] * 32, kGemmTn[model.c] * 32, model.sp,
                win->c, win->sp, win->grid);
    return GL_OK;
}

}

int gemm_launch(const AOperand& A, const bf16* W, int M, int N, int K, const Epilogue& E_in, float* ws,
                size_t ws_bytes, hipStream_t stream) {
    t_last.stats_nb = 0;
    Epilogue E = E_in;
    GemmPlan plan;
    GL_TRY(gemm_plan(A, M, N, K, E, ws != nullptr, ws_bytes, plan, [&](auto&&... a) { return tune(W, ws, stream, a...); }));
    t_last = plan;
    t_log[t_log_n % kGemmLogSize] = GemmLogEntry{plan, M, N, K};
    t_log_n = t_log_n == INT_MAX ? kGemmLogSize : t_log_n + 1;
    return execute(plan, A, W, M, N, K, E, ws, stream);
}

int gemm_launch_t(const bf16* Wrows, int Mw, const bf16* X, int Nx, int K, const Epilogue& E, hipStream_t stream) {
    AOperand A;
    aoperand_rows(A, Wrows, K, K);
    return gemm_launch(A, X, Mw, Nx, K, E, nullptr, 0, stream);
}

}
```

gligen_amd/csrc/gemm_plan.hip:

```cpp
#include "gemm_plan.h"

#include <algorithm>
#include <cmath>
#include <cstdio>
#include <mutex>
#include <string>
#include <unordered_map>

namespace gl {

static GemmKnobs read_knobs() {
    static const struct { const char* env; int GemmKnobs::*knob; } kInt[] = {
        {"GL_GEMM_VARIANT", &GemmKnobs::variant}, {"GL_GEMM_WIDE", &GemmKnobs::wide}, {"GL_GEMM_WIDE_SPLITS", &GemmKnobs::wide_splits},
        {"GL_CONV_HALO", &GemmKnobs::halo}, {"GL_CONV_HALO_SPLITS", &GemmKnobs::halo_splits}, {"GL_GEMM_XCD_BOXES", &GemmKnobs::xcd_boxes},
        {"GL_WIDE_XCD", &GemmKnobs::wide_xcd}, {"GL_GEMM_AUTOTUNE", &GemmKnobs::autotune}, {"GL_GEMM_TUNE_REPS", &GemmKnobs::tune_reps},
        {"GL_GEMM_TUNE_CORUN", &GemmKnobs::corun}};
    GemmKnobs k;
    for (const auto& e : kInt)
        if (const char* v = dev_env(e.env)) k.*e.knob = atoi(v);
    k.tune_reps = std::max(1, k.tune_reps);
    k.no_table = dev_env("GL_GEMM_NO_TABLE") != nullptr;
    k.tune_log = dev_env("GL_GEMM_TUNE_LOG") != nullptr;
    return k;
}
GemmKnobs& gemm_knobs() {
    static GemmKnobs k = read_knobs();
    return k;
}
void gemm_set_variant(int v) { gemm_knobs().variant = v < 0 ? read_knobs().variant : v; }
void gemm_set_autotune(int on) { gemm_knobs().autotune = on < 0 ? read_knobs().autotune : on; }
void gemm_force_cfg(int tm, int tn, int splits) { gemm_knobs().force_tm = tm; gemm_knobs().force_tn = tn; gemm_knobs().force_splits = splits; }
void gemm_force_grid(int g) { gemm_knobs().force_grid = g; }
void gemm_force_knobs(int halo_splits, int wide_splits, int wide_xcd, int xcd_boxes, int halo, int wide) {
    GemmKnobs& k = gemm_knobs();
    k.halo_splits = halo_splits; k.wide_splits = wide_splits; k.wide_xcd = wide_xcd; k.xcd_boxes = xcd_boxes; k.halo = halo; k.wide = wide;
}
void gemm_force_clear() {
    const GemmKnobs d = read_knobs();
    gemm_force_cfg(0, 0, 0);
    gemm_force_grid(0);
    gemm_force_knobs(d.halo_splits, d.wide_splits, d.wide_xcd, d.xcd_boxes, d.halo, d.wide);
}
static thread_local int t_no_split = 0;
void gemm_set_no_split(int on) { t_no_split = on; }
static thread_local int t_plan_scale = 1;
void gemm_set_plan_batch_scale(int scale) { t_plan_scale = scale > 1 ? scale : 1; }

int gemm_geglu_layout() { return gemm_knobs().variant >= 2 ? 1 : 0; }
bool gemm_supports_qkv() { return gemm_knobs().variant == 4; }

static size_t a_rows(const AOperand& A, int M) {
    return A.mode != A_ROWS && A.Ho * A.Wo > 0 ? (size_t)(M / (A.Ho * A.Wo)) * A.Hin * A.Win : (size_t)M;
}
static int row_tiles(const AOperand& A, int M, int bm) { return A.mode == A_CONV2UP ? 4 * cdiv(M / 4, bm) : cdiv(M, bm); }
static bool fits_buffer_offsets(const AOperand& A, int M, int N, int K) {
// ... 6 lines not shown
    return (1 << l) == v ? l : -1;
}
static bool halo_eligible(const AOperand& A, int M, int N, int K, const Epilogue& E) {
    if (A.mode != A_CONV3 || A.stride != 1 || A.ups || A.pad_lo != 1 || A.Ho != A.Hin || A.Wo != A.Win) return false;
    const int lgW = ilog2_exact(A.Win), lgH = ilog2_exact(A.Hin);
    if (lgW < 3 || lgW > 6 || lgH < 0 || M % 256) return false;
    const int R = 256 >> lgW, HB = std::min(A.Hin, R);
    if ((R / HB) * (HB + 2) * (A.Win + 2) > 448) return false;
    if (A.C0 % 64 || A.C1 % 64 || (N % 160 && N % 128)) return false;
    if (E.mode != EPI_ROWMAJOR || E.remap_in || (E.act != ACT_NONE && E.act != ACT_SILU) || (E.bias2 && E.res)) return false;
    if (E.bias2 && (E.rows_per_b != A.Hin * A.Win)) return false;
    return fits_buffer_offsets(A, M, N, K);
}
static bool wide_eligible(const AOperand& A, int M, int N, int K, const Epilogue& E) {
    if (A.mode != A_ROWS || M % 256 || (N % 160 && N % 128)) return false;
    if (A.C1 && A.C0 % 64) return false;
    if (E.mode != EPI_ROWMAJOR || E.remap_in || E.bias2) return false;
    if (E.act == ACT_GEGLU) { if (N % 128 || !E.geglu16 || E.res || E.out_f32) return false; }
    else if (E.act != ACT_NONE && E.act != ACT_SILU) return false;
    return fits_buffer_offsets(A, M, N, K);
}

static int gemm_route(const AOperand& A, int M, int N, int K, const Epilogue& E, bool honour_force = true) {
    const GemmKnobs& kn = gemm_knobs();
    if (A.mode == A_CONV2UP) return kn.variant == 4 && fits_buffer_offsets(A, M, N, K) ? GEMM_U : GEMM_P;
    if (kn.variant < 2 || (N < 128 && E.act != ACT_GEGLU)) return GEMM_GLDS;
    const bool use_u = kn.variant == 4 && fits_buffer_offsets(A, M, N, K) && !(E.bias2 && (E.res || A.mode == A_ROWS));
    if (!use_u) return GEMM_P;
    const bool forced = honour_force && kn.force_tm;
    if (kn.halo && !forced && N >= 128 && halo_eligible(A, M, N, K, E) && M >= kn.halo * 256) return GEMM_HALO;
    if (kn.wide && !forced && (kn.wide >= 2 || E.act == ACT_GEGLU) && wide_eligible(A, M, N, K, E)) return GEMM_WIDE;
    return GEMM_U;
}

bool gemm_gn_prologue_supported(const AOperand& A, int M, int N, int K, const Epilogue& E) {
    return K % 64 == 0 && gemm_route(A, M, N, K, E) == GEMM_HALO && (A.Hin * A.Win) % 256 == 0;
}

bool gemm_upconv_phases_supported(const AOperand& A, int M, int N, int K, const Epilogue& E) {
    if (A.mode != A_CONV2UP || M <= 0 || M != 4 * (M / (4 * A.Hin * A.Win)) * A.Hin * A.Win || A.Ho != 2 * A.Hin || A.Wo != 2 * A.Win) return false;
    if ((A.C0 + A.C1) % 64 || A.C0 % 64 || K != 4 * (A.C0 + A.C1) || N % 8 || A.gn) return false;
    if (E.mode != EPI_ROWMAJOR || E.act != ACT_NONE || E.out_f32 || E.bias2 || E.res || E.gate || E.remap_in || E.stats_out || E.ln_stats) return false;
    return gemm_route(A, M, N, K, E) == GEMM_U;
}

bool gemm_ln_fold_supported(const AOperand& A, int M, int N, int K, const Epilogue& E) {
    if (A.mode != A_ROWS || A.C1 || K % 64) return false;
    if (E.act == ACT_GEGLU) return E.mode == EPI_ROWMAJOR && gemm_route(A, M, N, K, E, false) == GEMM_WIDE;
    if (E.mode != EPI_QKV_HEADS && E.mode != EPI_QK_HEADS) return false;
    Epilogue Eh = E;
    Eh.bias2 = nullptr;
    return gemm_route(A, M, N, K, Eh, false) == GEMM_U;
}

static int gemm_validate(const AOperand& A, int M, int N, int K, Epilogue& E) {
    if (E.rows_per_b < 1) return set_error(GL_ERR_ARG, "gemm: rows_per_b=%d", E.rows_per_b);
    {
        E.up_win = A.mode == A_CONV2UP ? A.Win : 0;
        const unsigned d = E.up_win ? (unsigned)E.up_win : (unsigned)E.rows_per_b;
        int sh = 0;
        while ((1ull << sh) < d) ++sh;
        E.rpb_shift = sh;
        E.rpb_magic = (unsigned)((((1ull << sh) - d) << 32) / d + 1);
    }
    if (M <= 0 || N <= 0 || K <= 0) return set_error(GL_ERR_ARG, "gemm: empty problem M=%d N=%d K=%d", M, N, K);
    if (E.ln_stats && (!E.ln_csum || !E.bias || E.ln_nb < 1 || E.ln_ld < E.ln_nb || !gemm_ln_fold_supported(A, M, N, K, E)))
        return set_error(GL_ERR_UNSUPPORTED, "gemm: folded LayerNorm needs csum + folded bias + statistics, and an epilogue that applies them");
    if (K % 64 != 0) return set_error(GL_ERR_ARG, "gemm: K=%d must be a multiple of 64", K);
    if (N % 4 != 0) return set_error(GL_ERR_ARG, "gemm: N=%d must be a multiple of 4", N);
    if (A.gn && !gemm_gn_prologue_supported(A, M, N, K, E))
        return set_error(GL_ERR_UNSUPPORTED, "gemm: the GroupNorm prologue (AOperand::gn) exists in conv_halo_kernel only (3x3, stride 1, H W %% 256 == 0)");
    if (A.mode == A_CONV2UP) {
        if (!gemm_upconv_phases_supported(A, M, N, K, E))
            return set_error(GL_ERR_UNSUPPORTED, "conv3x3: no phase form of the upsample conv for this launch (gemm_u_kernel, bias-only bf16 epilogue, K = 4 Cin, N %% 8 == 0)");
    } else if (A.mode == A_CONV3) {
        if ((A.C0 + A.C1) % 64 != 0 || A.C0 % 64 != 0 || K != 9 * (A.C0 + A.C1))
            return set_error(GL_ERR_ARG, "conv3x3: channels (%d,%d) must be multiples of 64 and K=9*Cin (K=%d)", A.C0, A.C1, K);
    } else {
        if (K != A.C0 + A.C1 || (A.C1 && A.C0 % 64 != 0))
            return set_error(GL_ERR_ARG, "gemm: K=%d does not match operand channels (%d,%d)", K, A.C0, A.C1);
    }
    if (A.mode != A_ROWS && (E.gate || E.remap_in))
        return set_error(GL_ERR_UNSUPPORTED, "conv3x3: the gated residual and the row remap are row-GEMM epilogues");
    if ((E.act == ACT_GELU || E.act == ACT_QUICK_GELU) && (E.res || E.bias2 || A.mode != A_ROWS))
        return set_error(GL_ERR_UNSUPPORTED, "gemm: the GELU / quick-GELU epilogues have no residual / broadcast-bias form");
    if (E.act == ACT_GEGLU && (N % 32 != 0 || E.mode != EPI_ROWMAJOR))
        return set_error(GL_ERR_ARG, "gemm: GEGLU epilogue needs packed N %% 32 == 0 (N=%d)", N);
    if (E.act == ACT_GEGLU && E.geglu16 != gemm_geglu_layout())
        return set_error(GL_ERR_STATE, "gemm: GEGLU weights were packed for a different main-loop variant");
    if (E.mode == EPI_QKV_HEADS) {
        if (A.mode != A_ROWS || A.C1) return set_error(GL_ERR_ARG, "gemm: EPI_QKV_HEADS takes a single row-major activation operand");
        if (!gemm_supports_qkv() || !fits_buffer_offsets(A, M, N, K) || N != 3 * E.C || (2 * E.C) % 128 || !E.vt || !E.q || !E.k || E.T % 64 || M % E.T)
            return set_error(GL_ERR_UNSUPPORTED, "gemm: EPI_QKV_HEADS needs the v5 main loop, N = 3C with 2C %% 128 == 0, tokens per sample %% 64 == 0");
    }
    return GL_OK;
}

namespace {

struct Cfg { int bm, bn; float speed; };
const Cfg kCfgs[4] = {{128, 128, 1.0f}, {128, 64, 0.8f}, {64, 64, 0.55f}, {128, 32, 0.45f}};

const char* reduce_suffix(int splits) { return splits > 1 ? " + splitk_reduce_kernel" : ""; }
int split_units(const GemmProblem& pb, int want, int tiles, int units, int min_units, bool allowed, int& splits) {
    int sp = want;
    if (sp <= 0) {
// ... 257 lines not shown
```

gligen_amd/csrc/kbench.hip:

```cpp
#include <cstdio>
#include <cstdlib>
#include <chrono>
#include <cstring>
#include <functional>
#include <string>
#include <vector>

#include "attention.h"
#include "ffn.h"
#include "gemm.h"
#include "misc.h"
#include "norm.h"

using namespace gl;
#ifdef GL_FFN_ABLATE
namespace gl { void ff_rows_set_ablation(int abl); }
#endif

static hipStream_t cur_s = nullptr;

#define HC(expr)                                                                          \
    do {                                                                                  \
        hipError_t _e = (expr);                                                           \
        if (_e != hipSuccess) {                                                           \
// ... 454 lines not shown
            A.mode = A_CONV3; A.Hin = H; A.Win = W; A.Ho = H; A.Wo = W; A.stride = 1; A.ups = 0; A.pad_lo = 1;
            Epilogue E;
            epilogue_defaults(E);
            E.ldo = Cout; E.bias = bias; E.bias2 = gam; E.bias2_ld = Cout; E.rows_per_b = H * W;
            AOperand A1 = A, A2 = A;
            A1.p0 = y_norm; A1.C0 = Cin; A1.ld0 = Cin;
            A2.p0 = a0; A2.C0 = C0; A2.ld0 = C0; A2.p1 = C1 ? a1 : nullptr; A2.C1 = C1; A2.ld1 = C1; A2.gn = coef;
            Epilogue E1 = E, E2 = E;
            E1.out = out1; E2.out = out2;
            if (!gemm_gn_prologue_supported(A2, M, Cout, K, E2)) { printf("%-58s no GroupNorm prologue for this shape\n", line); continue; }
            auto two_pass = [=] { GC(groupnorm_launch(P, cur_s)); GC(gemm_launch(A1, w, M, Cout, K, E1, cur_s == s ? ws : ws2, ws_bytes, cur_s)); };
            auto gn_only = [=] { GC(groupnorm_launch(P, cur_s)); };
            auto conv_only = [=] { GC(gemm_launch(A1, w, M, Cout, K, E1, cur_s == s ? ws : ws2, ws_bytes, cur_s)); };
            auto coef_only = [=] { GC(groupnorm_coef_launch(P, cur_s)); };
            auto conv_pro = [=] { GC(gemm_launch(A2, w, M, Cout, K, E2, cur_s == s ? ws : ws2, ws_bytes, cur_s)); };
            relaunch = [=] { GC(groupnorm_coef_launch(P, cur_s)); GC(gemm_launch(A2, w, M, Cout, K, E2, cur_s == s ? ws : ws2, ws_bytes, cur_s)); };
            const float us2 = time_us(two_pass, reps, s);
            us = time_us(relaunch, reps, s);
            const float t_gn = time_us(gn_only, reps, s), t_cv = time_us(conv_only, reps, s), t_cf = time_us(coef_only, reps, s), t_cp = time_us(conv_pro, reps, s);
            float d, m;
            maxdiff(out1, out2, (size_t)M * Cout, s, &d, &m);
            const bool exact = H * W > 256;
            const bool ok = exact ? d == 0.f : d <= 0.01f * m;
            if (!ok) ++n_bad;
            printf("GNCONV %-44s two passes %.1f us (gn %.1f + conv %.1f) | prologue %.1f us (stats %.1f + conv %.1f)  maxdiff %g of %g %s\n", line, us2, t_gn, t_cv,
                   us, t_cf, t_cp, d, m, !ok ? "MISMATCH" : d == 0.f ? "bit-equal" : "within a bf16 step");
        } else if (!strcmp(kind, "attn")) {
            const int B = v[0], H = v[1], d = v[2], Nq = v[3], Nk = v[4];
            count = v[5]; c = 2;
            flop = 4.0 * B * H * d * (double)Nq * Nk;
            int dp, dpv;
            GC(attn_dims(d, &dp, &dpv));
            AttnParams P{};
            P.vt_layout = attn_vt_layout(d, Nk, &dpv);
            P.q = a0; P.k = a1; P.vt = a2;
            bf16* o = a2 + ((size_t)200 << 20);
            P.o = o;
            P.H = H; P.d = d; P.Nq = Nq; P.Nk = Nk; P.Tq_pad = round_up(Nq, 128); P.Tk_pad = round_up(Nk, 64);
            P.ldo = H * d; P.o_rows_per_b = Nq;
            P.scale_log2e = 1.4426950408889634f / sqrtf((float)d);
            GC(attn_vt_ones_launch(a2, B * H, d, P.Tk_pad, s, dpv));
            GC(attn_k_init_launch(a1, B * H, d, P.Tk_pad, s));
            relaunch = [=] { GC(attn_launch(P, B, cur_s)); };
            us = time_us(relaunch, reps, s);
        } else if (!strcmp(kind, "gn")) {
            const int B = v[0], HW = v[1], C0 = v[2], C1 = v[3], silu = v[4];
            count = v[5]; c = 3;
            bytes = 2.0 * B * HW * (double)(C0 + C1) * 2;
            GNParams P{};
            P.x0 = a0; P.C0 = C0; P.x1 = C1 ? a1 : nullptr; P.C1 = C1; P.B = B; P.HW = HW; P.eps = 1e-5f;
            P.gamma = gam; P.beta = bias; P.y = a2; P.silu = silu; P.partial = partial;
            relaunch = [=] { GC(groupnorm_launch(P, cur_s)); };
            us = time_us(relaunch, reps, s);
        } else if (!strcmp(kind, "ln")) {
            const int B = v[0], N1 = v[1], N2 = v[2], Tpad = v[3], C = v[4];
            count = v[5]; c = 4;
            bytes = 2.0 * B * (double)(N1 + N2) * C * 2;
            LNParams P{};
            P.x = a0; P.x2 = N2 ? a1 : nullptr; P.B = B; P.N1 = N1; P.N2 = N2; P.Tpad = Tpad; P.C = C; P.eps = 1e-5f;
            P.gamma = gam; P.beta = bias; P.y = a2;
            relaunch = [=] { GC(layernorm_launch(P, cur_s)); };
            us = time_us(relaunch, reps, s);
        } else {
            continue;
        }
        if (sweep && c <= 1) {
            static const int tms[7] = {4, 4, 2, 2, 8, 8, 2}, tns[7] = {5, 4, 5, 4, 5, 4, 2};
            static const int sps[8] = {1, 2, 3, 4, 6, 8, 12, 16};
            float best = 1e30f;
            int btm = 0, btn = 0, bsp = 0, bgrid = 0;
            std::string all;
            for (int gi = 0; gi < 3; ++gi)
                for (int ci = 0; ci < 7; ++ci)
                    for (int si = 0; si < 8; ++si) {
                        if (c == 0 && v[3] == 1 && (tns[ci] & 1)) continue;
                        if (tms[ci] >= 8 && gi) continue;
                        const int grid = gi == 0 ? 512 : gi == 1 ? 768 : 1024;
                        if (gi == 1 && (tms[ci] >= 8 || tms[ci] * 32 + tns[ci] * 32 > 192)) continue;
                        if (gi == 2 && tms[ci] * 32 + tns[ci] * 32 > 128) continue;
                        gemm_force_cfg(tms[ci], tns[ci], sps[si]);
                        gemm_force_grid(grid);
                        const int nk = gK / 64;
                        if (sps[si] > 1 && (nk / sps[si] < 2 || (size_t)sps[si] * gM * gN * 4 > ws_bytes)) continue;
                        if (gN < 128 && !(c == 0 && v[3] == 1)) continue;
                        if (c == 0 && v[3] == 3 && sps[si] > 1) continue;
                        int ctm2, ctn2, csp2;
                        relaunch();
                        gemm_last_cfg(&ctm2, &ctn2, &csp2);
                        if (csp2 != sps[si] || ctm2 != (tms[ci] > 8 ? tms[ci] - 8 : tms[ci]) || ctn2 != tns[ci]) continue;
                        float tus = time_us(relaunch, 5, s);
                        char buf[64];
                        snprintf(buf, sizeof buf, " %s%dx%d/%d@%d=%.1f", tms[ci] > 8 ? "D" : "", ctm2 * 32, tns[ci] * 32, csp2, grid, tus);
                        all += buf;
                        if (tus < best) { best = tus; btm = tms[ci]; btn = tns[ci]; bsp = csp2; bgrid = grid; }
                    }
            gemm_force_cfg(0, 0, 0);
            gemm_force_grid(0);
            if (best < 1e29f)
                printf("SWEEP %-52s auto %.1f us | best %.1f us %dx%d/%d@%d\n", line, us, best, btm * 32, btn * 32, bsp, bgrid);
            printf("      %s\n", all.c_str());
        }
        if (check && c <= 1 && !(c == 0 && (v[3] == 1 || v[3] == 4))) {
            gemm_set_variant(1);
            relaunch();
            HC(hipMemcpyAsync(r1, a1, CMP * 2, hipMemcpyDeviceToDevice, s));
            HC(hipMemcpyAsync(r2, a2, CMP * 2, hipMemcpyDeviceToDevice, s));
// ... 67 lines not shown
```

gligen_amd/csrc/norm.h:

```cpp
#pragma once
#include "common.h"

namespace gl {

struct GNParams {
    const bf16* x0;
    const bf16* x1;
    int C0, C1;
    int B, HW;
    float eps;
    const float* gamma;
    const float* beta;
    bf16* y;
    int silu;
    float* partial;
    float* coef;
};
int gn_nsplit(int HW);
size_t gn_partial_bytes(int B, int HW);
int groupnorm_launch(const GNParams& P, hipStream_t stream);
int groupnorm_coef_launch(const GNParams& P, hipStream_t stream);
int groupnorm_coef_launches(int HW, int C0, int C1);
inline size_t gn_coef_bytes(int B, int C) { return (size_t)B * C * 2 * sizeof(float); }

struct LNParams {
    const bf16* x;
    const bf16* x2;
    int B, N1, N2, Tpad, C;
    float eps;
    const float* gamma;
    const float* beta;
    bf16* y;
    int ldx, ldy;
};
int layernorm_launch(const LNParams& P, hipStream_t stream);

int softmax_rows_launch(const float* S, bf16* Pm, int rows, int cols, float scale, hipStream_t stream);

}
```

gligen_amd/csrc/norm.hip:

```cpp
#include "norm.h"

namespace gl {

constexpr int GN_UNR = 8;
static int gn_rows(int C8) { return C8 >= 256 ? 1 : 256 / C8; }
int gn_nsplit_c(int HW, int C8) { return max(1, min(64, cdiv(HW, gn_rows(C8) * GN_UNR))); }
int gn_nsplit(int HW) { return max(1, min(64, HW / 8)); }
size_t gn_partial_bytes(int B, int HW) { return (size_t)B * 64 * 32 * 2 * sizeof(float); }

__global__ void gn_stats_kernel(GNParams P, int nsplit, int C8, int R, int cpg) {
    extern __shared__ __attribute__((aligned(16))) unsigned char smem[];
    float4* tl = reinterpret_cast<float4*>(smem);
    const int t = threadIdx.x;
    const int cx = t % C8;
    const int ry = t / C8;
    const int b = blockIdx.y;
    const int c0 = cx * 8;
    const bool first = c0 < P.C0;
    const int ld = first ? P.C0 : P.C1;
    const bf16* base = (first ? P.x0 + c0 : P.x1 + (c0 - P.C0)) + (size_t)b * P.HW * ld;
    const int per = (P.HW + nsplit - 1) / nsplit;
    const int p0 = blockIdx.x * per;
    const int p1 = min(P.HW, p0 + per);
    const int g_lo = c0 / cpg;
    bool hi[4];
#pragma unroll
    for (int p = 0; p < 4; ++p) hi[p] = (c0 + 2 * p) / cpg != g_lo;

    float s_lo = 0.f, q_lo = 0.f, s_hi = 0.f, q_hi = 0.f;
    for (int p = p0 + ry; p < p1; p += R * GN_UNR) {
        U4BF8 v[GN_UNR];
#pragma unroll
        for (int u = 0; u < GN_UNR; ++u) v[u].u = *reinterpret_cast<const uint4*>(base + (size_t)min(p + u * R, p1 - 1) * ld);
#pragma unroll
        for (int u = 0; u < GN_UNR; ++u) {
            const bool ok = p + u * R < p1;
#pragma unroll
            for (int e = 0; e < 8; ++e) {
                const float f = ok ? bf2f(v[u].e[e]) : 0.f;
                if (hi[e >> 1]) { s_hi += f; q_hi += f * f; }
                else            { s_lo += f; q_lo += f * f; }
            }
        }
    }
    tl[t] = make_float4(s_lo, q_lo, s_hi, q_hi);
    __syncthreads();
    if (t < 32) {
        const int g = t;
        const int cx_lo = (g * cpg) / 8;
        const int cx_hi = ((g + 1) * cpg - 1) / 8;
        float s = 0.f, q = 0.f;
        for (int x = max(0, cx_lo - 1); x <= cx_hi; ++x) {
            const int gl_x = (x * 8) / cpg;
            for (int y = 0; y < R; ++y) {
                float4 v = tl[y * C8 + x];
                if (gl_x == g) { s += v.x; q += v.y; }
                if (gl_x + 1 == g) { s += v.z; q += v.w; }
            }
// ... 238 lines not shown
}

static int gn_check(const GNParams& P, int* cpg_out) {
    const int C = P.C0 + P.C1;
    if (C % 64 != 0 || (P.C1 && P.C0 % 8 != 0)) return set_error(GL_ERR_ARG, "groupnorm: C=%d (C0=%d) unsupported", C, P.C0);
    const int cpg = C / 32;
    if (cpg < 4 || (cpg & 1)) return set_error(GL_ERR_UNSUPPORTED, "groupnorm: %d channels per group (need an even number >= 4)", cpg);
    if (C / 8 > 1024) return set_error(GL_ERR_ARG, "groupnorm: C=%d too large", C);
    *cpg_out = cpg;
    return GL_OK;
}

int groupnorm_coef_launch(const GNParams& P, hipStream_t stream) {
    int cpg;
    GL_TRY(gn_check(P, &cpg));
    if (!P.coef) return set_error(GL_ERR_ARG, "groupnorm_coef: no coefficient buffer");
    const int C = P.C0 + P.C1, C8 = C / 8;
    if (P.HW <= 256 && (P.C0 & 3) == 0 && (cpg & 3) == 0) {
        if (P.HW * cpg >= 8192) hipLaunchKernelGGL(gn_small_coef_kernel<1024>, dim3(32, P.B), dim3(1024), 0, stream, P, cpg);
        else hipLaunchKernelGGL(gn_small_coef_kernel<256>, dim3(32, P.B), dim3(256), 0, stream, P, cpg);
        GL_LAUNCH_CHECK();
        return GL_OK;
    }
    const int R = gn_rows(C8);
    const int nsplit = gn_nsplit_c(P.HW, C8);
    const int T = C8 * R;
    hipLaunchKernelGGL(gn_stats_kernel, dim3(nsplit, P.B), dim3(T), T * sizeof(float4), stream, P, nsplit, C8, R, cpg);
    GL_LAUNCH_CHECK();
    hipLaunchKernelGGL(gn_coef_kernel, dim3(P.B), dim3(256), 0, stream, P, nsplit, cpg);
    GL_LAUNCH_CHECK();
    return GL_OK;
}
int groupnorm_coef_launches(int HW, int C0, int C1) {
    const int cpg = (C0 + C1) / 32;
    return (HW <= 256 && (C0 & 3) == 0 && (cpg & 3) == 0) ? 1 : 2;
}

int groupnorm_launch(const GNParams& P, hipStream_t stream) {
    const int C = P.C0 + P.C1;
    if (C % 64 != 0 || (P.C1 && P.C0 % 8 != 0)) return set_error(GL_ERR_ARG, "groupnorm: C=%d (C0=%d) unsupported", C, P.C0);
    const int cpg = C / 32;
    const int C8 = C / 8;
    if (cpg < 4 || (cpg & 1)) return set_error(GL_ERR_UNSUPPORTED, "groupnorm: %d channels per group (need an even number >= 4)", cpg);
    if (C8 > 1024) return set_error(GL_ERR_ARG, "groupnorm: C=%d too large", C);
    if (P.HW <= 256 && (P.C0 & 3) == 0 && (cpg & 3) == 0) {
        if (P.HW * cpg >= 8192) hipLaunchKernelGGL(gn_small_kernel<1024>, dim3(32, P.B), dim3(1024), 0, stream, P, cpg);
        else hipLaunchKernelGGL(gn_small_kernel<256>, dim3(32, P.B), dim3(256), 0, stream, P, cpg);
        GL_LAUNCH_CHECK();
        return GL_OK;
    }
    const int R = gn_rows(C8);
    const int nsplit = gn_nsplit_c(P.HW, C8);
    const int T = C8 * R;
    hipLaunchKernelGGL(gn_stats_kernel, dim3(nsplit, P.B), dim3(T), T * sizeof(float4), stream, P, nsplit, C8, R, cpg);
    GL_LAUNCH_CHECK();
    const int trips = cdiv(P.HW, R * GN_UNR);
    const int nblk = max(1, min(trips, max(1, 2048 / P.B)));
    const int per = cdiv(cdiv(P.HW, nblk), R) * R;
    hipLaunchKernelGGL(gn_apply_kernel, dim3(cdiv(P.HW, per), P.B), dim3(T), 0, stream, P, nsplit, C8, R, cpg, per);
    GL_LAUNCH_CHECK();
    return GL_OK;
}

__global__ void __launch_bounds__(256) ln_kernel(LNParams P) {
    const int lane = threadIdx.x & 63;
    const int wave = threadIdx.x >> 6;
    const int64_t r = (int64_t)blockIdx.x * 4 + wave;
    if (r >= (int64_t)P.B * P.Tpad) return;
    const int b = (int)(r / P.Tpad);
    const int t = (int)(r - (int64_t)b * P.Tpad);
    const int C8 = P.C >> 3;
    const int ldx = P.ldx ? P.ldx : P.C, ldy = P.ldy ? P.ldy : P.C;
    bf16* dst = P.y + r * ldy;
    for (int ch = C8 + lane; ch < (ldy >> 3); ch += 64) *reinterpret_cast<uint4*>(dst + ch * 8) = make_uint4(0, 0, 0, 0);
    const bf16* src;
    if (t < P.N1) src = P.x + ((size_t)b * P.N1 + t) * ldx;
    else if (t < P.N1 + P.N2) src = P.x2 + ((size_t)b * P.N2 + (t - P.N1)) * P.C;
    else {
        for (int ch = lane; ch < C8; ch += 64) *reinterpret_cast<uint4*>(dst + ch * 8) = make_uint4(0, 0, 0, 0);
        return;
    }
    float v[3][8];
    float s = 0.f;
#pragma unroll
    for (int i = 0; i < 3; ++i) {
        const int ch = lane + 64 * i;
        if (ch < C8) {
            U4BF8 u;
            u.u = *reinterpret_cast<const uint4*>(src + ch * 8);
#pragma unroll
            for (int e = 0; e < 8; ++e) { v[i][e] = bf2f(u.e[e]); s += v[i][e]; }
        } else {
#pragma unroll
            for (int e = 0; e < 8; ++e) v[i][e] = 0.f;
        }
    }
    const float mean = wave_sum(s) / P.C;
    float q = 0.f;
#pragma unroll
    for (int i = 0; i < 3; ++i) {
        const int ch = lane + 64 * i;
        if (ch < C8) {
#pragma unroll
            for (int e = 0; e < 8; ++e) { float d = v[i][e] - mean; q += d * d; }
        }
    }
    const float rstd = rsqrtf(wave_sum(q) / P.C + P.eps);
#pragma unroll
// ... 61 lines not shown
```

gligen_amd/engine.py:

```python
from __future__ import annotations

import ctypes as C
from typing import Dict, Mapping, Optional, Sequence

import numpy as np
import torch

from . import _lib
from ._lib import Grounding, PlmsArgs, UNetConfig, VaeConfig, check

GROUNDING_KINDS = {"text": 0, "text_image": 1, "keypoint": 2, "tokens": 3}


def _stream(device=None) -> C.c_void_p:
    return C.c_void_p(torch.cuda.current_stream(device).cuda_stream)


def _ptr(t: Optional[torch.Tensor]) -> C.c_void_p:
    return C.c_void_p(0 if t is None else t.data_ptr())


def _f32(t: torch.Tensor, device) -> torch.Tensor:
    return t.to(device=device, dtype=torch.float32).contiguous()

# ... 476 lines not shown
    def sampler_timing(self):
        a, f, n = C.c_float(), C.c_float(), C.c_int()
        check(self.lib.gl_sampler_timing(self._ctx, C.byref(a), C.byref(f), C.byref(n)))
        return float(a.value), float(f.value), int(n.value)

    def to_uint8(self, img: torch.Tensor) -> torch.Tensor:
        img = _f32(img, self.device)
        B, Cc, H, W = img.shape
        out = torch.empty((B, H, W, Cc), device=self.device, dtype=torch.uint8)
        check(self.lib.gl_to_uint8(_ptr(img), _ptr(out), int(B), int(Cc), int(H * W), _stream(self.device)))
        return out

    def arena_high_water(self) -> int:
        v = C.c_size_t()
        check(self.lib.gl_arena_high_water(self._ctx, C.byref(v)))
        return int(v.value)

    def launch_count(self) -> int:
        v = C.c_int64()
        check(self.lib.gl_launch_count(self._ctx, C.byref(v)))
        return int(v.value)

    def box_calibrate(self) -> dict:
        from ._lib import BoxCalibration
        c = BoxCalibration()
        check(self.lib.gl_box_calibrate(self._ctx, C.byref(c), _stream(self.device)))
        return {"hbm_copy_GBps": round(float(c.hbm_copy_gbs), 1), "lds_dma_TBps": round(float(c.lds_dma_tbs), 2),
                "mfma_bf16_TFLOPs": round(float(c.mfma_bf16_tflops), 1)}

    def mfma_calibrate(self, shape: int = 0, waves_per_simd: int = 2, n_acc: int = 4, zero_data: bool = False, target_ms: float = 25.0) -> dict:
        from ._lib import MfmaCalibration
        c = MfmaCalibration()
        check(self.lib.gl_mfma_calibrate(self._ctx, int(shape), int(waves_per_simd), int(n_acc), int(bool(zero_data)), float(target_ms), C.byref(c),
                                         _stream(self.device)))
        return {"shape": "32x32x16" if shape == 0 else "16x16x32", "waves_per_simd": int(waves_per_simd), "accumulators": int(n_acc),
                "data": "zeros" if zero_data else "random", "TFLOPs": round(float(c.tflops), 1), "sclk_MHz": round(float(c.sclk_mhz), 1),
                "ms": round(float(c.ms), 2), "cycles_per_mfma": round(float(c.cycles_per_mfma), 2),
                "frac_of_2.5PF": round(float(c.tflops) / 2500.0, 3)}

    def mfma_calibration_table(self, target_ms: float = 25.0) -> list:
        rows = []
        for shape in (0, 1):
            for wps in (1, 2):
                rows.append(self.mfma_calibrate(shape, wps, 8, False, target_ms))
        rows.append(self.mfma_calibrate(0, 2, 4, False, target_ms))
        rows.append(self.mfma_calibrate(0, 2, 8, True, target_ms))
        return rows

    def set_ff_rows_policy(self, mode: int) -> None:
        check(self.lib.gl_set_ff_rows_policy(int(mode)))

    def set_cfg_shared_prefix(self, on: bool) -> None:
        check(self.lib.gl_set_cfg_shared_prefix(int(bool(on))))

    def gemm_force_plan(self, tm=0, tn=0, splits=0, grid_cap=0) -> None:
        check(self.lib.gl_gemm_force_plan(int(tm), int(tn), int(splits), int(grid_cap)))

    def gemm_force_knobs(self, halo_splits, wide_splits, wide_xcd, xcd_boxes, halo, wide) -> None:
        check(self.lib.gl_gemm_force_knobs(int(halo_splits), int(wide_splits), int(wide_xcd), int(xcd_boxes), int(halo), int(wide)))

    def gemm_force_clear(self) -> None:
        check(self.lib.gl_gemm_force_clear())

    def gemm_plan_log_clear(self) -> None:
        check(self.lib.gl_gemm_plan_log_clear())

    def gemm_plan_log(self):
        from ._lib import GemmPlanRecord
        recs = (GemmPlanRecord * 32)()
        n, total = C.c_int(0), C.c_int(0)
        check(self.lib.gl_gemm_plan_log(recs, 32, C.byref(n), C.byref(total)))
        out = [{f: (getattr(r, f).decode() if f == "kernel" else getattr(r, f)) for f, _ in GemmPlanRecord._fields_} for r in recs[:n.value]]
        return out, total.value

    def ff_rows_policy_report(self) -> str:
        buf = C.create_string_buffer(4096)
        check(self.lib.gl_ff_rows_policy_report(buf, 4096))
        return buf.value.decode()

    def op_linear(self, x, w, bias=None, res=None, act=0, out_f32=False):
        M, K = x.shape
        N = w.shape[0]
        y = torch.empty((M, N), device=x.device, dtype=torch.float32 if out_f32 else torch.bfloat16)
        check(self.lib.gl_op_linear(self._ctx, _ptr(x), _ptr(w), _ptr(bias), _ptr(res), _ptr(y), M, N, K, act, int(out_f32), _stream(self.device)))
        return y

    def op_geglu(self, x, w_f32, b_f32):
        M, K = x.shape
        inner = w_f32.shape[0] // 2
        y = torch.empty((M, inner), device=x.device, dtype=torch.bfloat16)
        check(self.lib.gl_op_geglu(self._ctx, _ptr(x), _ptr(w_f32), _ptr(b_f32), _ptr(y), M, inner, K, _stream(self.device)))
        return y

    def op_ln_linear(self, a, w0, b0, res, gamma, beta, w1, b1, mode, inner_or_heads, T=0):
        M, K0 = a.shape
        Cc = w0.shape[0]
        x = torch.empty((M, Cc), device=a.device, dtype=torch.bfloat16)
        if mode == 0:
            y = torch.empty((M, inner_or_heads), device=a.device, dtype=torch.bfloat16)
        else:
            d = Cc // inner_or_heads
            dp = {40: 48, 80: 80, 160: 160}[d]
            y = torch.zeros((M // T * inner_or_heads, ((T + 127) // 128) * 128, dp), device=a.device, dtype=torch.bfloat16)
        used = C.c_int(-1)
        check(self.lib.gl_op_ln_linear(self._ctx, _ptr(a), M, K0, _ptr(w0), _ptr(b0), _ptr(res), Cc, _ptr(gamma), _ptr(beta), _ptr(w1),
                                       _ptr(b1), int(mode), int(inner_or_heads), int(T), _ptr(x), _ptr(y), C.byref(used), _stream(self.device)))
# ... 385 lines not shown
                                             1 if accumulate else 0, *[_ptr(o.get(n)) for n in ("a", "xhat", "rstd", "dx")], _stream(dev)))
        return o

    def op_train_geglu(self, u, dh=None, out=None):
        dev = self.device
        u = _f32(u, dev)
        dh = None if dh is None else _f32(dh, dev)
        R, I2 = u.shape
        if I2 % 2 or (dh is not None and dh.shape != (R, I2 // 2)):
            raise ValueError("op_train_geglu: u [R, 2 I], dh [R, I]")
        shapes = {"h": (R, I2 // 2)}
        if dh is not None:
            shapes.update(du=u.shape)
        o = self._prim_outs(shapes, out)
        check(self.lib.gl_op_train_geglu(self._ctx, int(R), int(I2 // 2), _ptr(u), _ptr(dh), _ptr(o.get("h")), _ptr(o.get("du")), _stream(dev)))
        return o

    def op_train_dot(self, a, b, mode, alpha=None, scale=1.0, out=None):
        dev = self.device
        a, b = _f32(a, dev).reshape(-1), _f32(b, dev).reshape(-1)
        alpha = None if alpha is None else _f32(alpha, dev)
        if a.shape != b.shape:
            raise ValueError("op_train_dot: a and b hold the same number of elements")
        o = self._prim_outs({"out": (1,)}, out, required=("out",))
        check(self.lib.gl_op_train_dot(self._ctx, int(a.numel()), _ptr(a), _ptr(b), _ptr(alpha), C.c_float(scale), int(mode), _ptr(o["out"]), _stream(dev)))
        return o

    def op_conv3x3(self, x0, w_oihw, bias, x1=None, stride=1, ups=0, pad_lo=1, res=None):
        B, H, W, C0 = x0.shape
        C1 = 0 if x1 is None else x1.shape[3]
        Cout = w_oihw.shape[0]
        Hup, Wup = H << ups, W << ups
        if stride == 1:
            Ho, Wo = Hup, Wup
        else:
            Ho = (Hup + (2 if pad_lo else 1) - 3) // 2 + 1
            Wo = (Wup + (2 if pad_lo else 1) - 3) // 2 + 1
        y = torch.empty((B, Ho, Wo, Cout), device=x0.device, dtype=torch.bfloat16)
        check(self.lib.gl_op_conv3x3(self._ctx, _ptr(x0), C0, _ptr(x1), C1, B, H, W, _ptr(w_oihw), _ptr(bias), Cout,
                                     stride, ups, pad_lo, _ptr(res), _ptr(y), _stream(self.device)))
        return y

    def op_gn_silu_conv3x3(self, x0, gamma, beta, eps, w_oihw, bias, x1=None, bias2=None, res=None, mode=-1):
        B, H, W, C0 = x0.shape
        C1 = 0 if x1 is None else x1.shape[3]
        Cout = w_oihw.shape[0]
        y = torch.empty((B, H, W, Cout), device=x0.device, dtype=torch.bfloat16)
        used = C.c_int(0)
        check(self.lib.gl_op_gn_silu_conv3x3(self._ctx, _ptr(x0), C0, _ptr(x1), C1, B, H, W, _ptr(gamma), _ptr(beta), C.c_float(eps),
                                             _ptr(w_oihw), _ptr(bias), Cout, _ptr(bias2), _ptr(res), _ptr(y), int(mode), C.byref(used),
                                             _stream(self.device)))
        return y, bool(used.value)

    def op_groupnorm(self, x0, gamma, beta, eps, silu, x1=None):
        B, HW, C0 = x0.shape
        C1 = 0 if x1 is None else x1.shape[2]
        y = torch.empty((B, HW, C0 + C1), device=x0.device, dtype=torch.bfloat16)
        check(self.lib.gl_op_groupnorm(self._ctx, _ptr(x0), C0, _ptr(x1), C1, B, HW, _ptr(gamma), _ptr(beta),
                                       C.c_float(eps), int(silu), _ptr(y), _stream(self.device)))
        return y

    def op_layernorm(self, x, gamma, beta, eps=1e-5, x2=None, Tpad=None):
        B, N1, Cc = x.shape
        N2 = 0 if x2 is None else x2.shape[1]
        Tpad = Tpad or (N1 + N2)
        y = torch.empty((B, Tpad, Cc), device=x.device, dtype=torch.bfloat16)
        check(self.lib.gl_op_layernorm(self._ctx, _ptr(x), _ptr(x2), B, N1, N2, Tpad, Cc, _ptr(gamma), _ptr(beta),
                                       C.c_float(eps), _ptr(y), _stream(self.device)))
        return y

    def op_ff_chain_q(self, x, pre_w, pre_b, pre_res, gamma, beta, w1, b1, w2, b2, gamma_q, beta_q, wq, pre_gate=None, gate=None):
        B, N, Cc = x.shape
        y = torch.empty_like(x)
        qbuf = torch.zeros((B * 8, N, 48), device=x.device, dtype=torch.bfloat16)
        check(self.lib.gl_op_ff_chain_q(self._ctx, _ptr(x), B, N, Cc, _ptr(pre_w), _ptr(pre_b), _ptr(pre_res), _ptr(pre_gate), _ptr(gamma), _ptr(beta),
                                        _ptr(w1), _ptr(b1), _ptr(w2), _ptr(b2), _ptr(gate), _ptr(gamma_q), _ptr(beta_q), _ptr(wq), _ptr(y), _ptr(qbuf),
                                        _stream(self.device)))
        return y, qbuf.view(B, 8, N, 48)[..., :40]

    def op_proj_attention(self, x, pre_w, pre_b, pre_res, gamma, beta, wq, wk, wv, heads, rows=True):
        B, N, Cc = x.shape
        mid = torch.empty_like(x)
        o = torch.empty_like(x)
        used = C.c_int(1 if rows else 0)
        check(self.lib.gl_op_proj_attention(self._ctx, _ptr(x), B, N, Cc, heads, _ptr(pre_w), _ptr(pre_b), _ptr(pre_res), _ptr(gamma), _ptr(beta),
                                            _ptr(wq), _ptr(wk), _ptr(wv), 0, _ptr(mid), _ptr(o), C.byref(used), _stream(self.device)))
        return mid, o, used.value

    def op_attention(self, xq, xkv, wq, wk, wv, heads):
        B, Nq, Cc = xq.shape
        _, Nk, Ck = xkv.shape
        o = torch.empty((B, Nq, Cc), device=xq.device, dtype=torch.bfloat16)
        check(self.lib.gl_op_attention(self._ctx, _ptr(xq), _ptr(xkv), B, Nq, Nk, Cc, Ck, heads, _ptr(wq), _ptr(wk), _ptr(wv),
                                       _ptr(o), _stream(self.device)))
        return o

    def op_attention_core(self, q, k, vt, layout, B, heads, Nq, Nk, o, ldo, o_rows_per_b, kernel="auto"):
        from ._lib import ATTN_CORE_KERNELS
        check(self.lib.gl_op_attention_core(self._ctx, _ptr(q), _ptr(k), _ptr(vt), C.byref(layout), B, heads, Nq, Nk, _ptr(o), ldo, o_rows_per_b,
                                            ATTN_CORE_KERNELS[kernel], _stream(self.device)))
        return o

    def attn_regime_counters(self, enable):
        lazy, reruns = C.c_uint(0), C.c_uint(0)
        check(self.lib.gl_attn_regime_counters(self._ctx, 1 if enable else 0, C.byref(lazy), C.byref(reruns)))
        return lazy.value, reruns.value
# ... 1 lines not shown
```

Measured before the change: 6.570 images/s.

## Fold GroupNorm statistics into split-K conv reduce epilogue and skip stats kernel

The split-K reduce epilogue of 3x3 conv GEMMs now also writes GroupNorm partial statistics. The following GroupNorm reuses them and launches only the apply kernel, skipping a separate stats pass that re-reads the activation. It is wired through resblocks (conv1 to norm2) and a new conv3x3_groupnorm op, and is on by default with an env and API switch to turn it off. It only applies to eligible shapes (HW>256, specific channel counts), and the reduce epilogue does a little extra work.

```diff
diff --git a/gligen_amd/_lib.py b/gligen_amd/_lib.py
--- a/gligen_amd/_lib.py
+++ b/gligen_amd/_lib.py
@@ -233,6 +233,11 @@
 ATTENTION_CORE_SYMBOLS = {
     "gl_op_attention_core": (_I, [_P, _P, _P, _P, C.POINTER(AttnProjLayout), _I, _I, _I, _I, _P, _I, _I, _I, _P]),
 }
+REDUCE_GN_SYMBOLS = {
+    "gl_set_reduce_gn_stats": (_I, [_I]),
+    "gl_reduce_gn_eligible": (_I, [_I] * 11),
+    "gl_op_conv3x3_groupnorm": (_I, [_P, _P, _I, _I, _I, _I, _P, _P, _I, _P, _P, _I, _I, _I, _P, _I, _P, _P, C.c_float, _I, _P, _P, _P]),
+}
 ATTN_CORE_KERNELS = {"auto": 0, "attn_kernel": 1, "attn2_kernel_w4": 2, "attn2_kernel_w8": 3, "attn3_kernel": 4}
 GL_ERR_UNSUPPORTED = 5
 
@@ -260,7 +265,7 @@
     import torch
     lib = C.CDLL(str(LIB_PATH))
     for name, (res, args) in {**SYMBOLS, **IMAGE_SYMBOLS, **MAP_SYMBOLS, **TRAIN_MAP_SYMBOLS, **TRAIN_INPUT_SYMBOLS, **TRAIN_FUSER_SYMBOLS, **TRAIN_PRIM_SYMBOLS,
-                              **TRAINER_SYMBOLS, **SAMPLER_SYMBOLS, **GEMM_PLAN_SYMBOLS, **ATTENTION_CORE_SYMBOLS}.items():
+                              **TRAINER_SYMBOLS, **SAMPLER_SYMBOLS, **GEMM_PLAN_SYMBOLS, **ATTENTION_CORE_SYMBOLS, **REDUCE_GN_SYMBOLS}.items():
         fn = getattr(lib, name)
         fn.restype = res
         fn.argtypes = args
diff --git a/gligen_amd/csrc/capi.hip b/gligen_amd/csrc/capi.hip
--- a/gligen_amd/csrc/capi.hip
+++ b/gligen_amd/csrc/capi.hip
@@ -11,6 +11,7 @@
 #include "../../include/gligen_amd_sampler.h"
 #include "../../include/gligen_amd_gemm_plans.h"
 #include "../../include/gligen_amd_attention_core.h"
+#include "../../include/gligen_amd_reduce_gn.h"
 #include "gemm_plan.h"
 
 #include <cstdlib>
@@ -447,6 +448,16 @@
 int gl_ff_rows_policy_report(char* buf, size_t cap) { return gl::ff_rows_policy_report(buf, cap); }
 
 int gl_set_cfg_shared_prefix(int on) { return gl::cfg_shared_prefix_set(on); }
+int gl_set_reduce_gn_stats(int on) { return gl::reduce_gn_stats_set(on); }
+int gl_reduce_gn_eligible(int B, int HW, int C, int ldo, int splits, int out_f32, int act, int row_remap, int up2x_phases, int ln_fold, int row_stats) {
+    gl::Epilogue E;
+    gl::epilogue_defaults(E);
+    static float dummy;
+    E.ldo = ldo; E.out_f32 = out_f32; E.act = act; E.rows_per_b = HW; E.remap_in = row_remap ? HW : 0; E.up_win = up2x_phases ? 1 : 0;
+    E.ln_stats = ln_fold ? reinterpret_cast<const float2*>(&dummy) : nullptr;
+    E.stats_out = row_stats ? reinterpret_cast<float2*>(&dummy) : nullptr;
+    return gl::gemm_reduce_gn_eligible(E, B * HW, C, splits) ? 1 : 0;
+}
 
 int gl_gemm_force_plan(int tm, int tn, int splits, int grid_cap) {
     bool tile = tm == 0 && tn == 0;
@@ -1145,6 +1156,33 @@
     eng.gn_prologue_ = saved;
     *used_prologue = eng.n_prologue_convs > n0 ? 1 : 0;
     if (mode == 1 && !*used_prologue) throw GlError(GL_ERR_UNSUPPORTED, "gl_op_gn_silu_conv3x3: this shape has no GroupNorm prologue (conv_halo_kernel, H W % 256 == 0)");
+    GL_API_END
+}
+
+int gl_op_conv3x3_groupnorm(gl_ctx* ctx, const void* x, int Cin, int B, int H, int W, const float* w_oihw, const float* bias, int Cout, const float* bias2,
+                            const void* res, int tm, int tn, int splits, const void* cat, int Ccat, const float* gamma, const float* beta, float eps, int silu,
+                            void* y, void* yn, gl_stream s) {
+    NEED(ctx);
+    if (!x || !w_oihw || !gamma || !beta || !y || !yn || (Ccat && !cat)) return gl::set_error(GL_ERR_ARG, "gl_op_conv3x3_groupnorm: null pointer");
+    if (splits < 0 || splits > 32) return gl::set_error(GL_ERR_ARG, "gl_op_conv3x3_groupnorm: %d splits (0 .. 32)", splits);
+    GL_API_BEGIN
+    Engine& eng = *ctx->eng;
+    Arena& ar = eng.arena();
+    ar.reset();
+    bf16* wp = ar.get<bf16>((size_t)Cout * 9 * Cin);
+    int r = pack_conv_weight_launch(w_oihw, wp, Cout, Cin, 3, 3, Cout, S(s));
+    if (r != GL_OK) throw GlError(r, gl::last_error());
+    ConvW c;
+    c.w = wp; c.b = bias; c.Cin = Cin; c.Cout = Cout;
+    NormW n;
+    n.g = gamma; n.b = beta; n.C = Cout + Ccat;
+    struct Restore {
+        gl::GemmKnobs saved = gl::gemm_knobs();
+        ~Restore() { gl::gemm_knobs() = saved; }
+    } restore;
+    if (splits && tm) gl::gemm_force_cfg(tm, tn, splits);
+    else if (splits) gl::gemm_knobs().halo_splits = splits;
+    eng.conv3x3_groupnorm((const bf16*)x, B, H, W, c, bias2, (const bf16*)res, (const bf16*)cat, Ccat, n, eps, silu != 0, (bf16*)y, (bf16*)yn, S(s));
     GL_API_END
 }
 
diff --git a/gligen_amd/csrc/engine.h b/gligen_amd/csrc/engine.h
--- a/gligen_amd/csrc/engine.h
+++ b/gligen_amd/csrc/engine.h
@@ -107,6 +107,8 @@
 int ff_rows_policy_report(char* buf, size_t cap);
 int cfg_shared_prefix_set(int on);
 bool cfg_shared_prefix();
+int reduce_gn_stats_set(int on);
+struct GnHandoff { const bf16* x = nullptr; int B = 0, HW = 0, C = 0, nsplit = 0; float* partial = nullptr; };
 AttnParams attn_params(const bf16* q, const bf16* k, const bf16* vt, bf16* o, int H, int d, int Nq, int Nk, int Tq_pad, int Tk_pad, int vt_layout);
 
 class Engine {
@@ -156,9 +158,11 @@
     unsigned* attn_counters() const { return attn_counting_ ? attn_ctr_ : nullptr; }
 
     bf16* gn_silu_conv3x3(const TRef& x, int B, int H, int W, const NormW& n, float eps, const ConvW& c, const float* bias2, int bias2_ld,
-                          const bf16* res, bf16* out, hipStream_t s);
+                          const bf16* res, bf16* out, hipStream_t s, const GnHandoff* x_stats = nullptr, GnHandoff* out_stats = nullptr);
     bf16* conv3x3(const TRef& x, int B, int Hin, int Win, const ConvW& c, int stride, int ups, int pad_lo,
-                  const float* bias2, int bias2_ld, const bf16* res, hipStream_t s, bf16* out = nullptr);
+                  const float* bias2, int bias2_ld, const bf16* res, hipStream_t s, bf16* out = nullptr, GnHandoff* out_stats = nullptr);
+    void conv3x3_groupnorm(const bf16* x, int B, int H, int W, const ConvW& c, const float* bias2, const bf16* res, const bf16* cat, int Ccat,
+                           const NormW& n, float eps, bool silu, bf16* y, bf16* yn, hipStream_t s);
     static bool upconv_phase_form(int Cin, int Cout);
     bool gn_prologue_ = dev_env("GL_GN_PROLOGUE") && atoi(dev_env("GL_GN_PROLOGUE")) == 1;
     int64_t n_prologue_convs = 0;
@@ -206,11 +210,13 @@
     void gemm(const AOperand& A, const bf16* W, int M, int N, int K, const Epilogue& E, hipStream_t s);
     bf16* linear_rows(const bf16* x, int M, const LinW& L, int act, const bf16* res, const float* gate, hipStream_t s, RowStats* stats = nullptr);
     bf16* layernorm_plain(const bf16* x, int B, int N, int C, bool pad64, hipStream_t s);
-    bf16* groupnorm(const TRef& x, int B, int HW, const NormW& n, float eps, bool silu, hipStream_t s);
+    bf16* groupnorm(const TRef& x, int B, int HW, const NormW& n, float eps, bool silu, hipStream_t s, const GnHandoff* x_stats = nullptr, bf16* y = nullptr);
+    GnHandoff* gn_handoff(GnHandoff& h, int B, int HW);
     bf16* layernorm(const bf16* x, int B, int N, int C, const NormW& n, bool pad64, hipStream_t s);
     bf16* conv3x3_small(const ConvW& c, Im2colParams P, int reps, hipStream_t s);
     void gn_silu_conv3x3_nchw(const bf16* x, int C, int B, int H, int W, const NormW& n, float eps, const ConvW& c, int n_real, float* out, hipStream_t s);
-    bf16* resblock(const ResW& r, const TRef& x, int B, int H, int W, const float* embout, int emb_ld, float eps, hipStream_t s, bf16* out = nullptr);
+    bf16* resblock(const ResW& r, const TRef& x, int B, int H, int W, const float* embout, int emb_ld, float eps, hipStream_t s, bf16* out = nullptr,
+                   GnHandoff* out_stats = nullptr);
     void replicate(const bf16* src, bf16* dst, size_t n, int reps, hipStream_t s);
     void attention(const bf16* q, const bf16* k, const bf16* vt, bf16* o, int B, int H, int d, int Nq, int Nk, int Tq_pad, int Tk_pad, int vt_layout,
                    hipStream_t s);
@@ -280,7 +286,7 @@
     std::vector<FuserKV> fuser_kv_;
     uint64_t cond_epoch_ = 0;
 
-    bf16* transformer(const STW& t, const bf16* x, int B, int Bp, int H, int W, hipStream_t s);
+    bf16* transformer(const STW& t, const bf16* x, int B, int Bp, int H, int W, hipStream_t s, const GnHandoff* x_stats = nullptr);
     bf16* feedforward(const FFW& f, const bf16* ln, int M, const bf16* res, const float* gate, hipStream_t s, const RowStats* in_stats = nullptr,
                       RowStats* out_stats = nullptr, bool raw_rows = false, bool use_rows = false);
     bf16* fuser_ff_tail(const STW& t, const bf16* o, const bf16* t1, int B, int HW, bool rows, hipStream_t s, RowStats* st3, bool* q_done = nullptr);
diff --git a/gligen_amd/csrc/engine.hip b/gligen_amd/csrc/engine.hip
--- a/gligen_amd/csrc/engine.hip
+++ b/gligen_amd/csrc/engine.hip
@@ -531,28 +531,53 @@
     return out;
 }
 
-bf16* Engine::groupnorm(const TRef& x, int B, int HW, const NormW& n, float eps, bool silu, hipStream_t s) {
+GnHandoff* Engine::gn_handoff(GnHandoff& h, int B, int HW) {
+    h = GnHandoff{};
+    if (!gemm_reduce_gn_stats() || HW <= 256) return nullptr;
+    h.partial = reinterpret_cast<float*>(arena_.alloc(gn_partial_bytes(B, HW)));
+    return &h;
+}
+
+static void gn_handoff_fill(GnHandoff* h, const bf16* out, int B, int HW, int C) {
+    if (!h) return;
+    float* partial = h->partial;
+    *h = GnHandoff{};
+    h->partial = partial;
+    if (!gemm_last_gn_stats()) return;
+    h->x = out; h->B = B; h->HW = HW; h->C = C; h->nsplit = gn_nsplit_c(HW, C / 8);
+}
+
+bf16* Engine::groupnorm(const TRef& x, int B, int HW, const NormW& n, float eps, bool silu, hipStream_t s, const GnHandoff* x_stats, bf16* y) {
     const int C = x.C();
     if (n.C != C) throw GlError(GL_ERR_ARG, fmt("groupnorm: %d channels given to a norm with %d", C, n.C));
-    bf16* y = arena_.get<bf16>((size_t)B * HW * C);
+    if (!y) y = arena_.get<bf16>((size_t)B * HW * C);
     GNParams P{};
     P.x0 = x.p0; P.C0 = x.C0; P.x1 = x.p1; P.C1 = x.C1;
     P.B = B; P.HW = HW; P.eps = eps; P.gamma = n.g; P.beta = n.b; P.y = y; P.silu = silu ? 1 : 0;
-    P.partial = reinterpret_cast<float*>(arena_.alloc(gn_partial_bytes(B, HW)));
-    ProfScope ps(this, s, HW <= 256 ? "gn_small_kernel" : "gn_stats_kernel + gn_apply_kernel", 0.0, 2.0 * B * HW * (double)C * 2);
+    const bool taken = x_stats && x_stats->x && x_stats->partial && x_stats->x == x.p0 && !x.p1 && x_stats->B == B && x_stats->HW == HW && x_stats->C == C &&
+                       HW > 256 && x_stats->nsplit == gn_nsplit_c(HW, C / 8);
+    if (taken) {
+        P.partial = x_stats->partial;
+        P.stats_done = 1;
+        reduce_gn_stats_note();
+    } else {
+        P.partial = reinterpret_cast<float*>(arena_.alloc(gn_partial_bytes(B, HW)));
+    }
+    ProfScope ps(this, s, HW <= 256 ? "gn_small_kernel" : taken ? "gn_apply_kernel" : "gn_stats_kernel + gn_apply_kernel", 0.0, (taken ? 1.5 : 2.0) * B * HW * (double)C * 2);
     CK(groupnorm_launch(P, s));
-    n_launches += HW <= 256 ? 1 : 2;
+    n_launches += HW <= 256 || taken ? 1 : 2;
     return y;
 }
 
 bf16* Engine::gn_silu_conv3x3(const TRef& x, int B, int H, int W, const NormW& n, float eps, const ConvW& c, const float* bias2, int bias2_ld,
-                              const bf16* res, bf16* out, hipStream_t s) {
+                              const bf16* res, bf16* out, hipStream_t s, const GnHandoff* x_stats, GnHandoff* out_stats) {
     if (x.C() != c.Cin || n.C != c.Cin) throw GlError(GL_ERR_ARG, fmt("gn_silu_conv3x3: %d channels into a norm of %d and a conv of %d", x.C(), n.C, c.Cin));
     const int HW = H * W, M = B * HW;
     if (!out) out = arena_.get<bf16>((size_t)M * c.Cout);
     AOperand A = a_conv3(x, H, W, H, W, 1, 0, 1);
     Epilogue E = e_rows_res(out, c.Cout, c.b, res);
     E.bias2 = bias2; E.bias2_ld = bias2_ld; E.rows_per_b = HW;
+    E.gn_partial = out_stats ? out_stats->partial : nullptr;
     if (gn_prologue_ && gemm_gn_prologue_supported(A, M, c.Cout, 9 * c.Cin, E)) {
         GNParams P{};
         P.x0 = x.p0; P.C0 = x.C0; P.x1 = x.p1; P.C1 = x.C1;
@@ -567,12 +592,14 @@
         }
         A.gn = P.coef;
         gemm(A, c.w, M, c.Cout, 9 * c.Cin, E, s);
+        gn_handoff_fill(out_stats, out, B, HW, c.Cout);
         ++n_prologue_convs;
         return out;
     }
-    bf16* a = groupnorm(x, B, HW, n, eps, true, s);
+    bf16* a = groupnorm(x, B, HW, n, eps, true, s, x_stats);
     A.p0 = a; A.C0 = c.Cin; A.ld0 = c.Cin; A.p1 = nullptr; A.C1 = 0; A.ld1 = 0;
     gemm(A, c.w, M, c.Cout, 9 * c.Cin, E, s);
+    gn_handoff_fill(out_stats, out, B, HW, c.Cout);
     return out;
 }
 
@@ -595,7 +622,8 @@
 }
 
 bf16* Engine::conv3x3(const TRef& x, int B, int Hin, int Win, const ConvW& c, int stride, int ups, int pad_lo,
-                      const float* bias2, int bias2_ld, const bf16* res, hipStream_t s, bf16* out) {
+                      const float* bias2, int bias2_ld, const bf16* res, hipStream_t s, bf16* out, GnHandoff* out_stats) {
+    if (out_stats) out_stats->x = nullptr;
     if (x.C() != c.Cin) throw GlError(GL_ERR_ARG, fmt("conv3x3: input has %d channels, weight expects %d", x.C(), c.Cin));
     if (c.w4) {
         if (stride != 1 || ups != 1 || pad_lo != 1 || bias2 || res) throw GlError(GL_ERR_ARG, "conv3x3: phase-form weights serve the plain upsample conv only");
@@ -619,8 +647,17 @@
     if (!out) out = arena_.get<bf16>((size_t)M * c.Cout);
     Epilogue E = e_rows_res(out, c.Cout, c.b, res);
     E.bias2 = bias2; E.bias2_ld = bias2_ld; E.rows_per_b = Ho * Wo;
+    E.gn_partial = out_stats ? out_stats->partial : nullptr;
     gemm(a_conv3(x, Hin, Win, Ho, Wo, stride, ups, pad_lo), c.w, M, c.Cout, 9 * c.Cin, E, s);
+    gn_handoff_fill(out_stats, out, B, Ho * Wo, c.Cout);
     return out;
+}
+
+void Engine::conv3x3_groupnorm(const bf16* x, int B, int H, int W, const ConvW& c, const float* bias2, const bf16* res, const bf16* cat, int Ccat,
+                               const NormW& n, float eps, bool silu, bf16* y, bf16* yn, hipStream_t s) {
+    GnHandoff h;
+    conv3x3(TRef{x, c.Cin, nullptr, 0}, B, H, W, c, 1, 0, 1, bias2, c.Cout, res, s, y, gn_handoff(h, B, H * W));
+    groupnorm(TRef{y, c.Cout, cat, Ccat}, B, H * W, n, eps, silu, s, &h, yn);
 }
 
 void Engine::replicate(const bf16* src, bf16* dst, size_t n, int reps, hipStream_t s) {
@@ -629,11 +666,13 @@
     ++n_launches;
 }
 
-bf16* Engine::resblock(const ResW& r, const TRef& x, int B, int H, int W, const float* embout, int emb_ld, float eps, hipStream_t s, bf16* out) {
+bf16* Engine::resblock(const ResW& r, const TRef& x, int B, int H, int W, const float* embout, int emb_ld, float eps, hipStream_t s, bf16* out,
+                       GnHandoff* out_stats) {
     const int HW = H * W, M = B * HW;
     if (!out) out = arena_.get<bf16>((size_t)M * r.Cout);
     const size_t mk = arena_.mark();
-    bf16* h = gn_silu_conv3x3(x, B, H, W, r.n1, eps, r.c1, embout ? embout + r.emb_off : nullptr, emb_ld, nullptr, nullptr, s);
+    GnHandoff hs;
+    bf16* h = gn_silu_conv3x3(x, B, H, W, r.n1, eps, r.c1, embout ? embout + r.emb_off : nullptr, emb_ld, nullptr, nullptr, s, nullptr, gn_handoff(hs, B, HW));
     const bf16* sk;
     if (r.has_skip) {
         bf16* skb = arena_.get<bf16>((size_t)M * r.Cout);
@@ -645,7 +684,7 @@
         if (x.p1) throw GlError(GL_ERR_STATE, "identity skip over a concatenated input");
         sk = x.p0;
     }
-    gn_silu_conv3x3(TRef{h, r.Cout, nullptr, 0}, B, H, W, r.n2, eps, r.c2, nullptr, 0, sk, out, s);
+    gn_silu_conv3x3(TRef{h, r.Cout, nullptr, 0}, B, H, W, r.n2, eps, r.c2, nullptr, 0, sk, out, s, &hs, out_stats);
     arena_.release(mk);
     return out;
 }
diff --git a/gligen_amd/csrc/engine_impl.h b/gligen_amd/csrc/engine_impl.h
--- a/gligen_amd/csrc/engine_impl.h
+++ b/gligen_amd/csrc/engine_impl.h
@@ -20,6 +20,7 @@
 unsigned ff_rows_policy_epoch();
 
 void cfg_shared_prefix_note(int what);
+void reduce_gn_stats_note();
 
 struct PlanAsBatch {
     explicit PlanAsBatch(int scale) { gemm_set_plan_batch_scale(scale); }
diff --git a/gligen_amd/csrc/engine_policy.hip b/gligen_amd/csrc/engine_policy.hip
--- a/gligen_amd/csrc/engine_policy.hip
+++ b/gligen_amd/csrc/engine_policy.hip
@@ -58,17 +58,29 @@
     }
     return GL_OK;
 }
+static std::atomic<long long> reduce_gn_taken{0};
+void reduce_gn_stats_note() { reduce_gn_taken.fetch_add(1); }
+int reduce_gn_stats_set(int on) {
+    if (on != 0 && on != 1) return set_error(GL_ERR_ARG, "reduce GroupNorm statistics %d (expected 0 or 1)", on);
+    if (gemm_reduce_gn_stats() != on) {
+        gemm_set_reduce_gn_stats(on);
+        ff_policy::epoch.fetch_add(1);
+    }
+    return GL_OK;
+}
 int ff_rows_policy_report(char* buf, size_t cap) {
     if (!buf || !cap) return set_error(GL_ERR_ARG, "ff_rows_policy_report: no buffer");
     std::lock_guard<std::mutex> lk(ff_policy::mu);
     size_t n = (size_t)snprintf(buf, cap, "mode=%d", ff_policy::mode.load());
     for (const auto& kv : ff_policy::table) {
-        if (n + 96 + 128 >= cap) break;
+        if (n + 96 + 64 + 128 >= cap) break;
         const uint64_t k = kv.first;
         n += (size_t)snprintf(buf + n, cap - n, ";dev%d %s form%d C%d M%d -> %s (rows %.1f us, gemm %.1f us)", (int)(k >> 56),
                               ((k >> 52) & 15) == 1 ? "fuser.ff" : ((k >> 52) & 15) == 2 ? "ff" : ((k >> 52) & 15) == 3 ? "proj_in+attn1.qkv" : "attn1.to_out+fuser.qkv", (int)((k >> 48) & 15), (int)((k >> 32) & 0xffff), (int)(k & 0xffffffffu),
                               kv.second.rows ? "rows" : "gemm", kv.second.us_rows, kv.second.us_gemm);
     }
+    if (n + 64 + 128 < cap)
+        n += (size_t)snprintf(buf + n, cap - n, ";reduce_gn_stats=%d taken=%lld", gemm_reduce_gn_stats(), reduce_gn_taken.load());
     if (n + 128 < cap)
         snprintf(buf + n, cap - n, ";cfg_shared_prefix=%d evals=%lld rows_at_prefix=%lld rows_periodic=%lld", cfg_prefix::current(),
                  cfg_prefix::count[0].load(), cfg_prefix::count[1].load(), cfg_prefix::count[2].load());
diff --git a/gligen_amd/csrc/engine_unet.hip b/gligen_amd/csrc/engine_unet.hip
--- a/gligen_amd/csrc/engine_unet.hip
+++ b/gligen_amd/csrc/engine_unet.hip
@@ -540,7 +540,7 @@
     return lnc;
 }
 
-bf16* Engine::transformer(const STW& t, const bf16* x, int B, int Bp, int H, int W, hipStream_t s) {
+bf16* Engine::transformer(const STW& t, const bf16* x, int B, int Bp, int H, int W, hipStream_t s, const GnHandoff* x_stats) {
     const int HW = H * W, M = B * HW, C = t.C, d = t.d, heads = C / d;
     bf16* out = arena_.get<bf16>((size_t)M * C);
     const size_t mk = arena_.mark();
@@ -549,7 +549,7 @@
     const bool shared = Bp < B;
     const int Mp = Bp * HW;
 
-    bf16* n = groupnorm(TRef{x, C, nullptr, 0}, Bp, HW, t.gn, 1e-6f, false, s);
+    bf16* n = groupnorm(TRef{x, C, nullptr, 0}, Bp, HW, t.gn, 1e-6f, false, s, x_stats);
     const int Tp = round_up(HW, 64);
     const bool aligned = Tp == HW;
     auto normed = [&](const bf16* rows, const NormW& nw, bool folded, bool fuse, bool pad64) -> const bf16* {
@@ -870,7 +870,10 @@
     }
     bool in_prefix = Bp < Beff;
 
-    auto run_layer = [&](const Layer& L, const TRef& in, int Bl, bool full) {
+    GnHandoff gn_next;
+    auto run_layer = [&](const Layer& L, const TRef& in, int Bl, bool full, bool st_next) {
+        const GnHandoff gn_in = gn_next;
+        gn_next = GnHandoff{};
         PlanAsBatch plan_as(L.kind == L_ST ? 1 : Beff / Bl);
         auto out_for = [&](int HWo, int Co) { return full ? arena_.get<bf16>((size_t)Beff * HWo * Co) : nullptr; };
         auto fill = [&](bf16* o, int HWo, int Co) {
@@ -889,14 +892,15 @@
             }
             case L_RES: {
                 const ResW& r = unet_.res[L.idx];
-                cur.p = resblock(r, in, Bl, cur.H, cur.W, embout, emb_ld, 1e-5f, s, out_for(cur.H * cur.W, r.Cout));
+                bf16* out = out_for(cur.H * cur.W, r.Cout);
+                cur.p = resblock(r, in, Bl, cur.H, cur.W, embout, emb_ld, 1e-5f, s, out, st_next ? gn_handoff(gn_next, Bl, cur.H * cur.W) : nullptr);
                 cur.C = r.Cout;
                 fill(cur.p, cur.H * cur.W, cur.C);
                 break;
             }
             case L_ST: {
                 if (in.p1) throw GlError(GL_ERR_STATE, "transformer over concatenated input");
-                cur.p = transformer(unet_.st[L.idx], in.p0, Beff, Bl, cur.H, cur.W, s);
+                cur.p = transformer(unet_.st[L.idx], in.p0, Beff, Bl, cur.H, cur.W, s, &gn_in);
                 break;
             }
             case L_DOWN: {
@@ -916,26 +920,27 @@
         }
     };
 
+    auto st_behind = [](const std::vector<Layer>& ls, size_t i) { return i + 1 < ls.size() && ls[i + 1].kind == L_ST; };
     for (const UNetBlock& b : unet_.in_blocks) {
         for (size_t i = 0; i < b.layers.size(); ++i) {
             const Layer& L = b.layers[i];
             const bool pre = in_prefix && L.kind != L_CONV_IN;
             const bool last = i + 1 == b.layers.size();
-            run_layer(L, TRef{cur.p, cur.C, nullptr, 0}, pre ? Bp : Beff, pre && L.kind != L_ST && (last || b.layers[i + 1].kind == L_ST));
+            run_layer(L, TRef{cur.p, cur.C, nullptr, 0}, pre ? Bp : Beff, pre && L.kind != L_ST && (last || b.layers[i + 1].kind == L_ST), st_behind(b.layers, i));
             if (L.kind == L_ST) in_prefix = false;
         }
         hs.push_back(cur);
     }
-    for (const Layer& L : unet_.mid_block.layers) run_layer(L, TRef{cur.p, cur.C, nullptr, 0}, Beff, false);
+    for (size_t i = 0; i < unet_.mid_block.layers.size(); ++i)
+        run_layer(unet_.mid_block.layers[i], TRef{cur.p, cur.C, nullptr, 0}, Beff, false, st_behind(unet_.mid_block.layers, i));
     for (const UNetBlock& b : unet_.out_blocks) {
         Act sk = hs.back();
         hs.pop_back();
         if (sk.H != cur.H || sk.W != cur.W) throw GlError(GL_ERR_ARG, "latent size must be divisible by the UNet's total stride");
-        bool first = true;
-        for (const Layer& L : b.layers) {
-            if (first) run_layer(L, TRef{cur.p, cur.C, sk.p, sk.C}, Beff, false);
-            else run_layer(L, TRef{cur.p, cur.C, nullptr, 0}, Beff, false);
-            first = false;
+        for (size_t i = 0; i < b.layers.size(); ++i) {
+            const Layer& L = b.layers[i];
+            if (i == 0) run_layer(L, TRef{cur.p, cur.C, sk.p, sk.C}, Beff, false, st_behind(b.layers, i));
+            else run_layer(L, TRef{cur.p, cur.C, nullptr, 0}, Beff, false, st_behind(b.layers, i));
         }
     }
     gn_silu_conv3x3_nchw(cur.p, cur.C, Beff, cur.H, cur.W, unet_.out_norm, 1e-5f, unet_.out_conv, c.out_channels, eps, s);
diff --git a/gligen_amd/csrc/gemm.h b/gligen_amd/csrc/gemm.h
--- a/gligen_amd/csrc/gemm.h
+++ b/gligen_amd/csrc/gemm.h
@@ -53,6 +53,7 @@
     int ln_nb, ln_ld;
     const float* ln_csum;
     float ln_inv_c, ln_eps;
+    float* gn_partial;
 };
 
 __host__ __device__ inline size_t ktile_off(size_t bh, int tpad, int t, int dd, int DP) {
@@ -79,6 +80,11 @@
 bool gemm_gn_prologue_supported(const AOperand& A, int M, int N, int K, const Epilogue& E);
 bool gemm_upconv_phases_supported(const AOperand& A, int M, int N, int K, const Epilogue& E);
 bool gemm_ln_fold_supported(const AOperand& A, int M, int N, int K, const Epilogue& E);
+bool gemm_reduce_gn_eligible(const Epilogue& E, int M, int N, int splits);
+void gemm_set_reduce_gn_stats(int on);
+int gemm_reduce_gn_stats();
+int splitk_reduce_launch(const float* ws, int splits, int M, int N, const Epilogue& E, hipStream_t stream);
+bool gemm_last_gn_stats();
 int gemm_last_stats_nb();
 void aoperand_rows(AOperand& A, const bf16* p, int K, int ld);
 
diff --git a/gligen_amd/csrc/gemm.hip b/gligen_amd/csrc/gemm.hip
--- a/gligen_amd/csrc/gemm.hip
+++ b/gligen_amd/csrc/gemm.hip
@@ -1,4 +1,5 @@
 #include "gemm_plan.h"
+#include "norm.h"
 
 #include <algorithm>
 #include <climits>
@@ -1479,6 +1480,120 @@
                 epi_finish4(E, m, n0, v);
             }
         }
+    }
+}
+
+template <int ZU, int UB, bool EXACT>
+__global__ void __launch_bounds__(256)
+splitk_reduce_gn_kernel(const float* __restrict__ ws, int splits, int M, int N, Epilogue E, int HW, int nsplit, int C8, int R, int cpg) {
+    __shared__ float4 tl[256];
+    const int t = threadIdx.x;
+    const int cx = t % C8;
+    const int ry = t / C8;
+    const int b = blockIdx.y;
+    const int c0 = cx * 8;
+    const int per = (HW + nsplit - 1) / nsplit;
+    const int p0 = blockIdx.x * per;
+    const int p1 = min(HW, p0 + per);
+    const int g_lo = c0 / cpg;
+    bool hi[4];
+#pragma unroll
+    for (int p = 0; p < 4; ++p) hi[p] = (c0 + 2 * p) / cpg != g_lo;
+    const size_t zs = (size_t)M * N;
+    const float* wsb = ws + (size_t)b * HW * N + c0;
+    const bf16* resb = E.res ? E.res + (size_t)b * HW * E.ldres + c0 : nullptr;
+    bf16* outb = reinterpret_cast<bf16*>(E.out) + (size_t)b * HW * E.ldo + c0;
+
+    float s_lo = 0.f, q_lo = 0.f, s_hi = 0.f, q_hi = 0.f;
+    for (int p = p0 + ry; p < p1; p += R * GN_UNR) {
+        float4 pb[2], pb2[2];
+#pragma unroll
+        for (int h = 0; h < 2; ++h) {
+            pb[h] = *reinterpret_cast<const float4*>(E.bias ? E.bias + c0 + 4 * h : ws);
+            pb2[h] = *reinterpret_cast<const float4*>(E.bias2 ? E.bias2 + (size_t)b * E.bias2_ld + c0 + 4 * h : ws);
+        }
+        const float pg = *((E.res && E.gate) ? E.gate : ws);
+        const bool has_b = E.bias != nullptr, has_b2 = E.bias2 != nullptr, has_res = E.res != nullptr;
+        const float g = E.gate ? pg : 1.f;
+        U4BF8 pr[GN_UNR];
+#pragma unroll
+        for (int u = 0; u < GN_UNR; ++u) {
+            const size_t px = (size_t)min(p + u * R, p1 - 1);
+            pr[u].u = *reinterpret_cast<const uint4*>(E.res ? reinterpret_cast<const void*>(resb + px * E.ldres) : reinterpret_cast<const void*>(ws));
+        }
+        float v[GN_UNR][8];
+#pragma unroll
+        for (int u = 0; u < GN_UNR; ++u)
+#pragma unroll
+            for (int e = 0; e < 8; ++e) v[u][e] = 0.f;
+#pragma unroll
+        for (int u0 = 0; u0 < GN_UNR; u0 += UB)
+            for (int z = 0; z < (EXACT ? ZU : splits); z += ZU) {
+                float4 a[UB][ZU][2];
+#pragma unroll
+                for (int u = 0; u < UB; ++u) {
+                    const float* src = wsb + (size_t)min(p + (u0 + u) * R, p1 - 1) * N;
+#pragma unroll
+                    for (int k = 0; k < ZU; ++k) {
+                        const float* sz = src + (size_t)min(z + k, splits - 1) * zs;
+                        a[u][k][0] = *reinterpret_cast<const float4*>(sz);
+                        a[u][k][1] = *reinterpret_cast<const float4*>(sz + 4);
+                    }
+                }
+#pragma unroll
+                for (int u = 0; u < UB; ++u)
+#pragma unroll
+                    for (int k = 0; k < ZU; ++k) {
+                        const bool ok = EXACT || z + k < splits;
+                        float* w = v[u0 + u];
+#pragma unroll
+                        for (int h = 0; h < 2; ++h) {
+                            w[4 * h + 0] += ok ? a[u][k][h].x : 0.f; w[4 * h + 1] += ok ? a[u][k][h].y : 0.f;
+                            w[4 * h + 2] += ok ? a[u][k][h].z : 0.f; w[4 * h + 3] += ok ? a[u][k][h].w : 0.f;
+                        }
+                    }
+            }
+#pragma unroll
+        for (int u = 0; u < GN_UNR; ++u) {
+            U4BF8 o;
+#pragma unroll
+            for (int h = 0; h < 2; ++h) {
+                float* w = &v[u][4 * h];
+                w[0] += has_b ? pb[h].x : 0.f; w[1] += has_b ? pb[h].y : 0.f; w[2] += has_b ? pb[h].z : 0.f; w[3] += has_b ? pb[h].w : 0.f;
+                w[0] += has_b2 ? pb2[h].x : 0.f; w[1] += has_b2 ? pb2[h].y : 0.f; w[2] += has_b2 ? pb2[h].z : 0.f; w[3] += has_b2 ? pb2[h].w : 0.f;
+            }
+#pragma unroll
+            for (int e = 0; e < 8; ++e) v[u][e] = has_res ? bf2f(pr[u].e[e]) + g * v[u][e] : v[u][e];
+#pragma unroll
+            for (int e = 0; e < 8; ++e) o.e[e] = f2bf(v[u][e]);
+            const bool ok = p + u * R < p1;
+            if (ok) *reinterpret_cast<uint4*>(outb + (size_t)(p + u * R) * E.ldo) = o.u;
+#pragma unroll
+            for (int e = 0; e < 8; ++e) {
+                const float f = ok ? bf2f(o.e[e]) : 0.f;
+                if (hi[e >> 1]) { s_hi += f; q_hi += f * f; }
+                else            { s_lo += f; q_lo += f * f; }
+            }
+        }
+    }
+    tl[t] = make_float4(s_lo, q_lo, s_hi, q_hi);
+    __syncthreads();
+    if (t < 32) {
+        const int g = t;
+        const int cx_lo = (g * cpg) / 8;
+        const int cx_hi = ((g + 1) * cpg - 1) / 8;
+        float s = 0.f, q = 0.f;
+        for (int x = max(0, cx_lo - 1); x <= cx_hi; ++x) {
+            const int gl_x = (x * 8) / cpg;
+            for (int y = 0; y < R; ++y) {
+                float4 w = tl[y * C8 + x];
+                if (gl_x == g) { s += w.x; q += w.y; }
+                if (gl_x + 1 == g) { s += w.z; q += w.w; }
+            }
+        }
+        float* dst = E.gn_partial + (((size_t)b * nsplit + blockIdx.x) * 32 + g) * 2;
+        dst[0] = s;
+        dst[1] = q;
     }
 }
 
@@ -2234,6 +2349,8 @@
 
 static thread_local GemmPlan t_last = [] { GemmPlan p{}; strcpy(p.name, "gemm"); return p; }();
 int gemm_last_stats_nb() { return t_last.stats_nb; }
+static thread_local bool t_last_gn_stats = false;
+bool gemm_last_gn_stats() { return t_last_gn_stats; }
 const char* gemm_last_kernel_name() { return t_last.name; }
 void gemm_last_cfg(int* tm, int* tn, int* splits) { *tm = t_last.tm; *tn = t_last.tn; *splits = t_last.splits; }
 static thread_local GemmLogEntry t_log[kGemmLogSize];
@@ -2282,6 +2399,26 @@
 }
 constexpr size_t halo_lds(int tn, bool gn) { return 2 * 7 * 64 * 128 + 2 * tn * 32 * 128 + (gn ? 2048 : 0); }
 constexpr size_t wide_lds(int tn) { return GL_WIDE_NST * (256 + tn * 32) * 128; }
+
+}
+
+int splitk_reduce_launch(const float* ws, int splits, int M, int N, const Epilogue& E, hipStream_t stream) {
+    if (E.gn_partial) {
+        if (!gemm_reduce_gn_eligible(E, M, N, splits)) return set_error(GL_ERR_UNSUPPORTED, "split-K reduce: no GroupNorm statistics for this epilogue (M=%d N=%d, %d splits)", M, N, splits);
+        const int HW = E.rows_per_b, C8 = N / 8, R = gn_rows(C8), nsplit = gn_nsplit_c(HW, C8);
+        const dim3 grid(nsplit, M / HW), block(C8 * R);
+        if (splits == 2) hipLaunchKernelGGL(HIP_KERNEL_NAME(splitk_reduce_gn_kernel<2, GN_UNR, true>), grid, block, 0, stream, ws, splits, M, N, E, HW, nsplit, C8, R, N / 32);
+        else hipLaunchKernelGGL(HIP_KERNEL_NAME(splitk_reduce_gn_kernel<4, 4, false>), grid, block, 0, stream, ws, splits, M, N, E, HW, nsplit, C8, R, N / 32);
+    } else {
+        int64_t total = (int64_t)M * (N / 4);
+        int blocks = (int)fmin((double)cdiv64(total, 256), 4096.0);
+        hipLaunchKernelGGL(splitk_reduce_kernel, dim3(blocks), dim3(256), 0, stream, ws, splits, M, N, E);
+    }
+    GL_LAUNCH_CHECK();
+    return GL_OK;
+}
+
+namespace {
 
 int execute(const GemmPlan& p, const AOperand& A, const bf16* W, int M, int N, int K, const Epilogue& E_in, float* ws, hipStream_t stream) {
     Epilogue E = E_in;
@@ -2310,12 +2447,7 @@
         case GEMM_GLDS * 1000 + 41: rc = exec_glds<4, 1, 1, 1>(l, p); break;
     }
     GL_TRY(rc);
-    if (p.splits > 1) {
-        int64_t total = (int64_t)M * (N / 4);
-        int blocks = (int)fmin((double)cdiv64(total, 256), 4096.0);
-        hipLaunchKernelGGL(splitk_reduce_kernel, dim3(blocks), dim3(256), 0, stream, ws, p.splits, M, N, E);
-        GL_LAUNCH_CHECK();
-    }
+    if (p.splits > 1) GL_TRY(splitk_reduce_launch(ws, p.splits, M, N, E, stream));
     return GL_OK;
 }
 
@@ -2323,10 +2455,12 @@
     hipStreamCaptureStatus cap = hipStreamCaptureStatusNone;
     if (stream) (void)hipStreamIsCapturing(stream, &cap);
     if (cap != hipStreamCaptureStatusNone) return GL_OK;
+    Epilogue Et = pb.E;
+    Et.gn_partial = nullptr;
     auto run = [&](const GemmCand& c, hipStream_t s) -> int {
         GemmPlan plan{};
         GL_TRY(gemm_plan_tile(pb, use_u, c, plan));
-        return execute(plan, pb.A, W, pb.M, pb.N, pb.K, pb.E, ws, s);
+        return execute(plan, pb.A, W, pb.M, pb.N, pb.K, Et, ws, s);
     };
     GL_HIP(hipDeviceSynchronize());
     hipEvent_t ev[2];
@@ -2376,12 +2510,15 @@
 int gemm_launch(const AOperand& A, const bf16* W, int M, int N, int K, const Epilogue& E_in, float* ws,
                 size_t ws_bytes, hipStream_t stream) {
     t_last.stats_nb = 0;
+    t_last_gn_stats = false;
     Epilogue E = E_in;
     GemmPlan plan;
     GL_TRY(gemm_plan(A, M, N, K, E, ws != nullptr, ws_bytes, plan, [&](auto&&... a) { return tune(W, ws, stream, a...); }));
     t_last = plan;
     t_log[t_log_n % kGemmLogSize] = GemmLogEntry{plan, M, N, K};
     t_log_n = t_log_n == INT_MAX ? kGemmLogSize : t_log_n + 1;
+    if (E.gn_partial && !(gemm_reduce_gn_stats() && gemm_reduce_gn_eligible(E, M, N, plan.splits))) E.gn_partial = nullptr;
+    t_last_gn_stats = E.gn_partial != nullptr;
     return execute(plan, A, W, M, N, K, E, ws, stream);
 }
 
diff --git a/gligen_amd/csrc/gemm_plan.hip b/gligen_amd/csrc/gemm_plan.hip
--- a/gligen_amd/csrc/gemm_plan.hip
+++ b/gligen_amd/csrc/gemm_plan.hip
@@ -1,6 +1,7 @@
 #include "gemm_plan.h"
 
 #include <algorithm>
+#include <atomic>
 #include <cmath>
 #include <cstdio>
 #include <mutex>
@@ -113,6 +114,32 @@
     Eh.bias2 = nullptr;
     return gemm_route(A, M, N, K, Eh, false) == GEMM_U;
 }
+
+bool gemm_reduce_gn_eligible(const Epilogue& E, int M, int N, int splits) {
+    if (splits <= 1 || M <= 0 || N <= 0) return false;
+    if (E.mode != EPI_ROWMAJOR || E.out_f32 || E.act != ACT_NONE) return false;
+    if (E.remap_in || E.up_win || E.ln_stats || E.stats_out) return false;
+    if (E.ldo != N || (E.res && E.ldres < N)) return false;
+    const int HW = E.rows_per_b;
+    if (HW <= 256 || M % HW != 0) return false;
+    const int cpg = N / 32;
+    return N % 64 == 0 && cpg >= 4 && (cpg & 1) == 0 && N / 8 <= 256;
+}
+
+namespace {
+std::atomic<int> g_reduce_gn{-1};
+}
+int gemm_reduce_gn_stats() {
+    int v = g_reduce_gn.load();
+    if (v < 0) {
+        const char* e = dev_env("GL_REDUCE_GN_STATS");
+        int expect = -1;
+        g_reduce_gn.compare_exchange_strong(expect, (e && atoi(e) == 0) ? 0 : 1);
+        v = g_reduce_gn.load();
+    }
+    return v;
+}
+void gemm_set_reduce_gn_stats(int on) { g_reduce_gn.store(on ? 1 : 0); }
 
 static int gemm_validate(const AOperand& A, int M, int N, int K, Epilogue& E) {
     if (E.rows_per_b < 1) return set_error(GL_ERR_ARG, "gemm: rows_per_b=%d", E.rows_per_b);
diff --git a/gligen_amd/csrc/kbench.hip b/gligen_amd/csrc/kbench.hip
--- a/gligen_amd/csrc/kbench.hip
+++ b/gligen_amd/csrc/kbench.hip
@@ -530,6 +530,45 @@
             P.gamma = gam; P.beta = bias; P.y = a2; P.silu = silu; P.partial = partial;
             relaunch = [=] { GC(groupnorm_launch(P, cur_s)); };
             us = time_us(relaunch, reps, s);
+        } else if (!strcmp(kind, "reducegn")) {
+            const int B = v[0], HW = v[1], C = v[2], splits = v[3], res = v[4];
+            count = v[5]; c = 3;
+            bytes = (double)B * HW * C * (4.0 * splits + 2 + (res ? 2 : 0));
+            Epilogue E;
+            epilogue_defaults(E);
+            E.out = a0; E.ldo = C; E.bias = bias; E.res = res ? a1 : nullptr; E.ldres = C; E.rows_per_b = HW;
+            Epilogue Eg = E;
+            if ((size_t)splits * B * HW * C * sizeof(float) > ws_bytes || (size_t)B * HW * C > ACT) { fprintf(stderr, "reducegn: shape too large\n"); continue; }
+            hipLaunchKernelGGL(fill_f32_kernel, dim3(2048), dim3(256), 0, s, ws, (size_t)splits * B * HW * C, 7u, 1.f);
+            Eg.gn_partial = partial;
+            GNParams P{};
+            P.x0 = a0; P.C0 = C; P.B = B; P.HW = HW; P.eps = 1e-5f; P.gamma = gam; P.beta = bias; P.y = a2; P.silu = 1; P.partial = partial;
+            GNParams Pd = P;
+            Pd.stats_done = 1;
+            const int M = B * HW;
+            auto pair = [=] { GC(splitk_reduce_launch(ws, splits, M, C, E, cur_s)); GC(groupnorm_launch(P, cur_s)); };
+            auto fused = [=] { GC(splitk_reduce_launch(ws, splits, M, C, Eg, cur_s)); GC(groupnorm_launch(Pd, cur_s)); };
+            auto r_plain = [=] { GC(splitk_reduce_launch(ws, splits, M, C, E, cur_s)); };
+            auto r_gn = [=] { GC(splitk_reduce_launch(ws, splits, M, C, Eg, cur_s)); };
+            auto gn_full = [=] { GC(groupnorm_launch(P, cur_s)); };
+            auto gn_apply = [=] { GC(groupnorm_launch(Pd, cur_s)); };
+            pair();
+            const unsigned long long o1 = checksum(a0, (size_t)M * C * 2, s), n1 = checksum(a2, (size_t)M * C * 2, s);
+            HC(hipMemsetAsync(a0, 0, (size_t)M * C * 2, s));
+            HC(hipMemsetAsync(a2, 0, (size_t)M * C * 2, s));
+            fused();
+            const unsigned long long o2 = checksum(a0, (size_t)M * C * 2, s), n2 = checksum(a2, (size_t)M * C * 2, s);
+            const bool same = o1 == o2 && n1 == n2;
+            if (!same) ++n_bad;
+            float t[6];
+            for (int round = 0; round < 3; ++round) {
+                const float r[6] = {time_us(pair, reps, s), time_us(fused, reps, s), time_us(r_plain, reps, s), time_us(r_gn, reps, s), time_us(gn_full, reps, s), time_us(gn_apply, reps, s)};
+                for (int i = 0; i < 6; ++i) t[i] = round ? std::min(t[i], r[i]) : r[i];
+            }
+            printf("REDUCEGN %-40s reduce + stats + apply %.2f us | fused reduce + apply %.2f us | reduce %.2f, fused reduce %.2f, stats + apply %.2f, apply %.2f "
+                   "-> reduce + stats %.2f against fused %.2f  %s\n", line, t[0], t[1], t[2], t[3], t[4], t[5], t[2] + t[4] - t[5], t[3], same ? "bit-equal" : "MISMATCH");
+            relaunch = fused;
+            us = t[1];
         } else if (!strcmp(kind, "ln")) {
             const int B = v[0], N1 = v[1], N2 = v[2], Tpad = v[3], C = v[4];
             count = v[5]; c = 4;
diff --git a/gligen_amd/csrc/norm.h b/gligen_amd/csrc/norm.h
--- a/gligen_amd/csrc/norm.h
+++ b/gligen_amd/csrc/norm.h
@@ -14,9 +14,13 @@
     bf16* y;
     int silu;
     float* partial;
+    int stats_done;
     float* coef;
 };
 int gn_nsplit(int HW);
+constexpr int GN_UNR = 8;
+int gn_rows(int C8);
+int gn_nsplit_c(int HW, int C8);
 size_t gn_partial_bytes(int B, int HW);
 int groupnorm_launch(const GNParams& P, hipStream_t stream);
 int groupnorm_coef_launch(const GNParams& P, hipStream_t stream);
diff --git a/gligen_amd/csrc/norm.hip b/gligen_amd/csrc/norm.hip
--- a/gligen_amd/csrc/norm.hip
+++ b/gligen_amd/csrc/norm.hip
@@ -2,8 +2,7 @@
 
 namespace gl {
 
-constexpr int GN_UNR = 8;
-static int gn_rows(int C8) { return C8 >= 256 ? 1 : 256 / C8; }
+int gn_rows(int C8) { return C8 >= 256 ? 1 : 256 / C8; }
 int gn_nsplit_c(int HW, int C8) { return max(1, min(64, cdiv(HW, gn_rows(C8) * GN_UNR))); }
 int gn_nsplit(int HW) { return max(1, min(64, HW / 8)); }
 size_t gn_partial_bytes(int B, int HW) { return (size_t)B * 64 * 32 * 2 * sizeof(float); }
@@ -348,8 +347,10 @@
     const int R = gn_rows(C8);
     const int nsplit = gn_nsplit_c(P.HW, C8);
     const int T = C8 * R;
-    hipLaunchKernelGGL(gn_stats_kernel, dim3(nsplit, P.B), dim3(T), T * sizeof(float4), stream, P, nsplit, C8, R, cpg);
-    GL_LAUNCH_CHECK();
+    if (!P.stats_done) {
+        hipLaunchKernelGGL(gn_stats_kernel, dim3(nsplit, P.B), dim3(T), T * sizeof(float4), stream, P, nsplit, C8, R, cpg);
+        GL_LAUNCH_CHECK();
+    }
     const int trips = cdiv(P.HW, R * GN_UNR);
     const int nblk = max(1, min(trips, max(1, 2048 / P.B)));
     const int per = cdiv(cdiv(P.HW, nblk), R) * R;
diff --git a/gligen_amd/engine.py b/gligen_amd/engine.py
--- a/gligen_amd/engine.py
+++ b/gligen_amd/engine.py
@@ -552,6 +552,9 @@
 
     def set_cfg_shared_prefix(self, on: bool) -> None:
         check(self.lib.gl_set_cfg_shared_prefix(int(bool(on))))
+
+    def set_reduce_gn_stats(self, on: bool) -> None:
+        check(self.lib.gl_set_reduce_gn_stats(int(bool(on))))
 
     def gemm_force_plan(self, tm=0, tn=0, splits=0, grid_cap=0) -> None:
         check(self.lib.gl_gemm_force_plan(int(tm), int(tn), int(splits), int(grid_cap)))
@@ -1043,6 +1046,19 @@
                                              _stream(self.device)))
         return y, bool(used.value)
 
+    def op_conv3x3_groupnorm(self, x, w_oihw, bias, gamma, beta, eps, silu, bias2=None, res=None, cat=None, tm=0, tn=0, splits=0, y=None, yn=None):
+        B, H, W, Cin = x.shape
+        Cout = w_oihw.shape[0]
+        Ccat = 0 if cat is None else cat.shape[-1]
+        if y is None:
+            y = torch.empty((B, H * W, Cout), device=x.device, dtype=torch.bfloat16)
+        if yn is None:
+            yn = torch.empty((B, H * W, Cout + Ccat), device=x.device, dtype=torch.bfloat16)
+        check(self.lib.gl_op_conv3x3_groupnorm(self._ctx, _ptr(x), Cin, B, H, W, _ptr(w_oihw), _ptr(bias), Cout, _ptr(bias2), _ptr(res), int(tm), int(tn),
+                                               int(splits), _ptr(cat), Ccat, _ptr(gamma), _ptr(beta), C.c_float(eps), int(silu), _ptr(y), _ptr(yn),
+                                               _stream(self.device)))
+        return y, yn
+
     def op_groupnorm(self, x0, gamma, beta, eps, silu, x1=None):
         B, HW, C0 = x0.shape
         C1 = 0 if x1 is None else x1.shape[2]
diff --git a/include/gligen_amd_reduce_gn.h b/include/gligen_amd_reduce_gn.h
--- /dev/null
+++ b/include/gligen_amd_reduce_gn.h
@@ -0,0 +1,19 @@
+#ifndef GLIGEN_AMD_REDUCE_GN_H
+#define GLIGEN_AMD_REDUCE_GN_H
+#include "gligen_amd.h"
+
+#ifdef __cplusplus
+extern "C" {
+#endif
+
+int gl_set_reduce_gn_stats(int on);
+int gl_reduce_gn_eligible(int B, int HW, int C, int ldo, int splits, int out_f32, int act, int row_remap, int up2x_phases, int ln_fold, int row_stats);
+
+int gl_op_conv3x3_groupnorm(gl_ctx* ctx, const void* x, int Cin, int B, int H, int W, const float* w_oihw, const float* bias, int Cout, const float* bias2,
+                            const void* res, int tm, int tn, int splits, const void* cat, int Ccat, const float* gamma, const float* beta, float eps, int silu,
+                            void* y, void* yn, gl_stream s);
+
+#ifdef __cplusplus
+}
+#endif
+#endif
```

After: 6.604 images/s (median of 6 runs). Within noise of the previous version (+0.5%).
